# rednote-hilab/dots.ocr

Hardware: AMD Instinct MI355X
Metric: pages/sec, dots.ocr 1.7B bf16, A4@200dpi page batch (preprocess + ViT + prefill + 1024-token greedy decode + detokenise) (higher is better)
Workload: dtype bf16; 1 GPU; a4: 8 pages/GPU of 1654x2339 px -> 19824 patches, 5200 prompt tokens/page, max_new_tokens=1024, EOS disabled; pages_per_gpu=8, parallelism=dp1, decode_rows_in_flight=64

## Files before the change

### dots_ocr_amd/csrc/attn_prefill.hip

```cpp
#include <algorithm>
#include <cstdlib>
#include <utility>

#include "common.h"
#include "kernels.h"

namespace {

constexpr int KT_BYTES = 64 * 256;
constexpr int VT_BYTES = 128 * 128;
constexpr int BUF_BYTES = KT_BYTES + VT_BYTES;
constexpr float RESCALE_THR = 6.0f;

template <bool CAUSAL, int NW, int MODE>
__global__ __launch_bounds__(NW * 64, 2) void flash_attn_kernel(
    const bf16_t* __restrict__ Q, const bf16_t* __restrict__ K, const bf16_t* __restrict__ VT,
    bf16_t* __restrict__ O, const QBlock* __restrict__ blocks, int n_items, int64_t T, int64_t Tpad, int Hq, int group,
    float scale_log2e) {
    constexpr bool PINGPONG = MODE == 1;
    static_assert(!PINGPONG || NW == 8, "ping-pong pairs wave w with wave w + 4 on the same SIMD");
    extern __shared__ __attribute__((aligned(16))) char smem[];

    const QBlock qb = blocks[xcd_remap(blockIdx.x, n_items)];
    const int h = qb.head;
// ... 502 lines not shown
        tile_body(j + 1, sB, sA);
    }

#ifdef F64_PROF
    if (blockIdx.x == 1000 && tid == 0)
        printf("F64_PROF tiles %d: gaps0-7 %llu, gaps8-63 %llu cycles per tile (s_memtime units)\n", n_tiles, prof[1] / n_tiles, prof[3] / n_tiles);
#endif
#pragma unroll
    for (int bk = 0; bk < 2; ++bk) {
        const float l_tot = l_run[bk] + __shfl_xor(l_run[bk], 32, 64);
        const float inv = 1.0f / l_tot;
        const int qrow = qb.q0 + w * 64 + bk * 32 + l31;
        if (qrow < n) {
            bf16_t* op = O + ((size_t)(qb.tok0 + qrow) * Hq + h) * 128;
#pragma unroll
            for (int dt = 0; dt < 4; ++dt)
#pragma unroll
                for (int rq = 0; rq < 4; ++rq) {
                    u32x2 pk = {pack_bf2(o[bk][dt][4 * rq] * inv, o[bk][dt][4 * rq + 1] * inv),
                                pack_bf2(o[bk][dt][4 * rq + 2] * inv, o[bk][dt][4 * rq + 3] * inv)};
                    *reinterpret_cast<u32x2*>(op + dt * 32 + 8 * rq + 4 * hi) = pk;
                }
        }
    }
}
#undef F64_QK_OPS
#undef F64_PV_OPS

}

XcdPlan make_xcd_plan(const QBlock* b, int n_blocks) {
    XcdPlan p;
    bool uniform = true;
    for (int i = 1; i < n_blocks && uniform; ++i) uniform = b[i].n == b[0].n;
    if (uniform || n_blocks < 8) {
        const int q = n_blocks / 8, r = n_blocks % 8;
        for (int x = 0, pos = 0; x < 8; ++x) { p.base[x] = pos; p.cnt[x] = q + (x < r ? 1 : 0); pos += p.cnt[x]; }
        return p;
    }
    auto cost = [&](int i) { return (int64_t)(((b[i].n + 63) / 64 + 1) & ~1); };
    int64_t total = 0;
    for (int i = 0; i < n_blocks; ++i) total += cost(i);
    int pos = 0;
    int64_t done = 0;
    for (int x = 0; x < 8; ++x) {
        const int64_t target = total * (x + 1) / 8;
        p.base[x] = pos;
        while (pos < n_blocks && (x == 7 || done + cost(pos) / 2 < target)) done += cost(pos++);
        p.cnt[x] = pos - p.base[x];
    }
    return p;
}

hipError_t launch_flash_attn(hipStream_t s, const bf16_t* q, const bf16_t* k, const bf16_t* vt, bf16_t* out,
                             const QBlock* blocks, int n_blocks, int64_t T, int64_t Tpad, int Hq, int Hkv,
                             int causal, float scale, const XcdPlan* plan) {
    if (n_blocks <= 0) return hipSuccess;
    if (Hq % Hkv != 0) return hipErrorInvalidValue;
    const float c = scale * 1.44269504088896340736f;
    dim3 grid(n_blocks);
    static const int mode = getenv("DOTS_OCR_ATTN_MODE") ? atoi(getenv("DOTS_OCR_ATTN_MODE")) : 2;
    auto go = [&](auto kern, int threads, int lds) -> hipError_t {
        if (lds > 64 * 1024) {
            hipError_t e = hipFuncSetAttribute(reinterpret_cast<const void*>(kern), hipFuncAttributeMaxDynamicSharedMemorySize, lds);
            if (e != hipSuccess) return e;
        }
        hipLaunchKernelGGL(kern, grid, dim3(threads), lds, s, q, k, vt, out, blocks, n_blocks, T, Tpad, Hq, Hq / Hkv, c);
        return hipGetLastError();
    };
    if (flash_rows_per_block() == 256) {
        static const bool causal64 = !(getenv("DOTS_OCR_PREFILL_F64") && atoi(getenv("DOTS_OCR_PREFILL_F64")) == 0);
        if (mode == 2 && (!causal || causal64)) {
            static uint32_t attr_done[2] = {0, 0};
            int dev = 0;
            hipError_t e = hipGetDevice(&dev);
            if (e != hipSuccess) return e;
            const uint32_t bit = 1u << (dev & 31);
            if (!(__atomic_load_n(&attr_done[causal ? 1 : 0], __ATOMIC_ACQUIRE) & bit)) {
                e = causal ? hipFuncSetAttribute(reinterpret_cast<const void*>(flash_attn64_kernel<true>), hipFuncAttributeMaxDynamicSharedMemorySize, RING_BYTES)
                           : hipFuncSetAttribute(reinterpret_cast<const void*>(flash_attn64_kernel<false>), hipFuncAttributeMaxDynamicSharedMemorySize, RING_BYTES);
                if (e != hipSuccess) return e;
                __atomic_fetch_or(&attr_done[causal ? 1 : 0], bit, __ATOMIC_RELEASE);
            }
            XcdPlan pl;
            if (plan) pl = *plan;
            else {
                const int qn = n_blocks / 8, rn = n_blocks % 8;
                for (int x = 0, pos = 0; x < 8; ++x) { pl.base[x] = pos; pl.cnt[x] = qn + (x < rn ? 1 : 0); pos += pl.cnt[x]; }
            }
            int mx = 0;
            for (int x = 0; x < 8; ++x) mx = std::max(mx, (int)pl.cnt[x]);
            if (causal) hipLaunchKernelGGL(flash_attn64_kernel<true>, dim3(8 * mx), dim3(256), RING_BYTES, s, q, k, vt, out, blocks, n_blocks, T, Tpad, Hq, Hq / Hkv, c, pl);
            else hipLaunchKernelGGL(flash_attn64_kernel<false>, dim3(8 * mx), dim3(256), RING_BYTES, s, q, k, vt, out, blocks, n_blocks, T, Tpad, Hq, Hq / Hkv, c, pl);
            return hipGetLastError();
        }
        if (mode >= 1) return causal ? go(flash_attn_kernel<true, 8, 1>, 512, 3 * BUF_BYTES) : go(flash_attn_kernel<false, 8, 1>, 512, 3 * BUF_BYTES);
        return causal ? go(flash_attn_kernel<true, 8, 0>, 512, 2 * BUF_BYTES) : go(flash_attn_kernel<false, 8, 0>, 512, 2 * BUF_BYTES);
    }
    return causal ? go(flash_attn_kernel<true, 4, 0>, 256, 2 * BUF_BYTES) : go(flash_attn_kernel<false, 4, 0>, 256, 2 * BUF_BYTES);
}

int flash_rows_per_block() {
    static const int rows = getenv("DOTS_OCR_ATTN_ROWS128") ? 128 : 256;
    return rows;
}
```

### dots_ocr_amd/csrc/elementwise.hip

```cpp
#include "common.h"
#include "kernels.h"

namespace {

constexpr int MAX_CHUNKS = 8;

template <bool LAYERNORM, int NCH>
__global__ __launch_bounds__(256) void norm_kernel(const bf16_t* __restrict__ x, const bf16_t* __restrict__ w,
                                                   const bf16_t* __restrict__ b, bf16_t* __restrict__ y,
                                                   int64_t rows, int dim, float eps) {
    const int l = threadIdx.x & 63;
    const int64_t row = (int64_t)blockIdx.x * 4 + (threadIdx.x >> 6);
    if (row >= rows) return;
    const bf16_t* xr = x + row * dim;
    constexpr int NC = NCH > 0 ? NCH : MAX_CHUNKS;
    u32x4 v[NC];
    float s = 0.f, s2 = 0.f;
    if constexpr (NCH > 0) {
#pragma unroll
        for (int c = 0; c < NC; ++c) v[c] = *reinterpret_cast<const u32x4*>(xr + c * 512 + l * 8);
    }
#pragma unroll
    for (int c = 0; c < NC; ++c) {
        const int off = c * 512 + l * 8;
// ... 104 lines not shown
            const int item = it * 256 + tid;
            const int tok = item >> 3, c = item & 7;
            if (tok >= tl.n) continue;
            const int64_t t = tl.tok0 + tok;
            const float2* tab = cs + t * 64 + c * 8;
            float2 cc[8];
#pragma unroll
            for (int e = 0; e < 8; ++e) cc[e] = tab[e];
            for (int hh = slot * ROPE_HPB; hh < h_end; ++hh) {
                bf16_t* dst = hh < Hq ? q + (size_t)hh * T * 128 : k + (size_t)(hh - Hq) * T * 128;
                const bf16_t* src = qkv + t * ld + hh * 128 + c * 8;
                u32x4 xl = *reinterpret_cast<const u32x4*>(src);
                u32x4 xh = *reinterpret_cast<const u32x4*>(src + 64);
                u32x4 ol, oh;
#pragma unroll
                for (int e = 0; e < 4; ++e) {
                    float2 c0 = cc[2 * e], c1 = cc[2 * e + 1];
                    float a0 = lo_bf(xl[e]), a1 = hi_bf(xl[e]), b0 = lo_bf(xh[e]), b1 = hi_bf(xh[e]);
                    ol[e] = pack_bf2(__builtin_fmaf(a0, c0.x, -(b0 * c0.y)), __builtin_fmaf(a1, c1.x, -(b1 * c1.y)));
                    oh[e] = pack_bf2(__builtin_fmaf(a0, c0.y, b0 * c0.x), __builtin_fmaf(b1, c1.x, a1 * c1.y));
                }
                bf16_t* d = dst + t * 128 + c * 8;
                *reinterpret_cast<u32x4*>(d) = ol;
                *reinterpret_cast<u32x4*>(d + 64) = oh;
            }
        }
    } else {
        const int h = slot - n_groups;
#pragma unroll
        for (int it = 0; it < 4; ++it) {
            const int item = it * 256 + tid;
            const int tok = item >> 4, c = item & 15;
            u32x4 v = {0, 0, 0, 0};
            if (tok < tl.n) v = *reinterpret_cast<const u32x4*>(qkv + (size_t)(tl.tok0 + tok) * ld + (Hq + Hkv + h) * 128 + c * 8);
            const int p = (tok & ~15) | (tok & 3) | (((tok >> 3) & 1) << 2) | (((tok >> 2) & 1) << 3);
            *reinterpret_cast<u32x4*>(&lds[p * 136 + c * 8]) = v;
        }
        __syncthreads();
#pragma unroll
        for (int it = 0; it < 4; ++it) {
            const int item = it * 256 + tid;
            const int d = item >> 3, pc = item & 7;
            u32x4 o;
#pragma unroll
            for (int e = 0; e < 4; ++e) {
                uint32_t a = lds[(pc * 8 + 2 * e) * 136 + d], b = lds[(pc * 8 + 2 * e + 1) * 136 + d];
                o[e] = a | (b << 16);
            }
            *reinterpret_cast<u32x4*>(vt + ((size_t)h * 128 + d) * Tpad + tl.pad0 + pc * 8) = o;
        }
    }
}

__global__ __launch_bounds__(256) void embed_gather_kernel(const int32_t* __restrict__ src, const bf16_t* __restrict__ embed,
                                                           const bf16_t* __restrict__ vision, bf16_t* __restrict__ x,
                                                           int64_t T, int dim) {
    const int l = threadIdx.x & 63;
    const int64_t t = (int64_t)blockIdx.x * 4 + (threadIdx.x >> 6);
    if (t >= T) return;
    const int sidx = src[t];
    const bf16_t* s = sidx >= 0 ? embed + (size_t)sidx * dim : vision + (size_t)(-sidx - 1) * dim;
    for (int off = l * 8; off < dim; off += 512)
        *reinterpret_cast<u32x4*>(x + t * dim + off) = *reinterpret_cast<const u32x4*>(s + off);
}

__global__ __launch_bounds__(256) void gather_rows_kernel(const bf16_t* __restrict__ x, const int32_t* __restrict__ rows,
                                                          const int32_t* __restrict__ dst, bf16_t* __restrict__ y, int n, int dim) {
    const int l = threadIdx.x & 63;
    const int r = blockIdx.x * 4 + (threadIdx.x >> 6);
    if (r >= n) return;
    const bf16_t* s = x + (size_t)rows[r] * dim;
    bf16_t* d = y + (size_t)(dst ? dst[r] : r) * dim;
    for (int off = l * 8; off < dim; off += 512) *reinterpret_cast<u32x4*>(d + off) = *reinterpret_cast<const u32x4*>(s + off);
}

}

hipError_t launch_rmsnorm(hipStream_t s, const bf16_t* x, const bf16_t* w, bf16_t* y, int64_t rows, int dim, float eps) {
    if (rows <= 0) return hipSuccess;
    if (dim % 8 != 0 || dim > MAX_CHUNKS * 512) return hipErrorInvalidValue;
    const dim3 grid((unsigned)((rows + 3) / 4));
    const bf16_t* nob = nullptr;
    if (dim == 1536) hipLaunchKernelGGL((norm_kernel<false, 3>), grid, dim3(256), 0, s, x, w, nob, y, rows, dim, eps);
    else if (dim == 1024) hipLaunchKernelGGL((norm_kernel<false, 2>), grid, dim3(256), 0, s, x, w, nob, y, rows, dim, eps);
    else if (dim == 512) hipLaunchKernelGGL((norm_kernel<false, 1>), grid, dim3(256), 0, s, x, w, nob, y, rows, dim, eps);
    else hipLaunchKernelGGL((norm_kernel<false, 0>), grid, dim3(256), 0, s, x, w, nob, y, rows, dim, eps);
    return hipGetLastError();
}

hipError_t launch_layernorm(hipStream_t s, const bf16_t* x, const bf16_t* w, const bf16_t* b, bf16_t* y,
                            int64_t rows, int dim, float eps) {
    if (rows <= 0) return hipSuccess;
    if (dim % 8 != 0 || dim > MAX_CHUNKS * 512) return hipErrorInvalidValue;
    const dim3 grid((unsigned)((rows + 3) / 4));
    if (dim == 1536) hipLaunchKernelGGL((norm_kernel<true, 3>), grid, dim3(256), 0, s, x, w, b, y, rows, dim, eps);
    else hipLaunchKernelGGL((norm_kernel<true, 0>), grid, dim3(256), 0, s, x, w, b, y, rows, dim, eps);
    return hipGetLastError();
}

hipError_t launch_patch_prep(hipStream_t s, const float* x, bf16_t* y, int64_t rows, int in_dim, int out_dim) {
    if (rows <= 0) return hipSuccess;
    if (in_dim % 4 != 0 || out_dim % 4 != 0 || out_dim < in_dim) return hipErrorInvalidValue;
    const int64_t n = rows * (out_dim / 4);
    hipLaunchKernelGGL(patch_prep_kernel, dim3((unsigned)((n + 255) / 256)), dim3(256), 0, s, x, y, rows, in_dim, out_dim);
    return hipGetLastError();
}

hipError_t launch_rope_table(hipStream_t s, const int32_t* pos, const float* inv_freq, float2* cs, int64_t T, int two_d) {
    if (T <= 0) return hipSuccess;
    hipLaunchKernelGGL(rope_table_kernel, dim3((unsigned)((T * 64 + 255) / 256)), dim3(256), 0, s, pos, inv_freq, cs, T, two_d);
    return hipGetLastError();
}

hipError_t launch_qkv_rope_split(hipStream_t s, const bf16_t* qkv, const float2* cs, const Tile64* tiles, int n_tiles,
                                 bf16_t* q, bf16_t* k, bf16_t* vt, int64_t T, int64_t Tpad, int Hq, int Hkv, bool v_only) {
    if (n_tiles <= 0) return hipSuccess;
    const int n_groups = (Hq + Hkv + ROPE_HPB - 1) / ROPE_HPB;
    if (v_only) hipLaunchKernelGGL(qkv_rope_split_kernel, dim3(n_tiles, Hkv), dim3(256), 0, s, qkv, cs, tiles, q, k, vt, T, Tpad, Hq, Hkv, n_groups);
    else hipLaunchKernelGGL(qkv_rope_split_kernel, dim3(n_tiles, n_groups + Hkv), dim3(256), 0, s, qkv, cs, tiles, q, k, vt, T, Tpad, Hq, Hkv, 0);
    return hipGetLastError();
}

hipError_t launch_embed_gather(hipStream_t s, const int32_t* src, const bf16_t* embed, const bf16_t* vision, bf16_t* x,
                               int64_t T, int dim) {
    if (T <= 0) return hipSuccess;
    hipLaunchKernelGGL(embed_gather_kernel, dim3((unsigned)((T + 3) / 4)), dim3(256), 0, s, src, embed, vision, x, T, dim);
    return hipGetLastError();
}

hipError_t launch_gather_rows(hipStream_t s, const bf16_t* x, const int32_t* rows, const int32_t* dst, bf16_t* y, int n, int dim) {
    if (n <= 0) return hipSuccess;
    hipLaunchKernelGGL(gather_rows_kernel, dim3((n + 3) / 4), dim3(256), 0, s, x, rows, dst, y, n, dim);
    return hipGetLastError();
}
```

### dots_ocr_amd/csrc/engine.h

```cpp
#pragma once
#include <hip/hip_runtime.h>
#include <hip/hip_fp16.h>

#include <algorithm>
#include <cmath>
#include <cstdarg>
#include <cstddef>
#include <cstdio>
#include <cstdlib>
#include <cstring>
#include <string>
#include <type_traits>
#include <unordered_map>
#include <vector>

#include "common.h"
#include "decode_layout.h"
#include "dots_ocr_hip.h"
#include "kernels.h"
#include "row_stage.h"

struct Tensor {
    bf16_t* p = nullptr;
    std::vector<int64_t> shape;
// ... 12 lines not shown
    uint8_t *qkv_8, *o_8, *w13_8, *down_8;
};

struct DotsEngine {
    DotsConfig cfg{};
    int device = 0;
    hipStream_t stream = nullptr;
    std::string err;
    std::vector<void*> allocs;
    bool finalized = false;

    std::unordered_map<std::string, Tensor> raw;

    bf16_t *patch_w = nullptr, *patch_b = nullptr, *patch_norm = nullptr;
    int patch_k = 0, patch_kpad = 0;
    std::vector<VLayer> vl;
    bf16_t *v_post_norm = nullptr, *m_ln_w = nullptr, *m_ln_b = nullptr, *m0_w = nullptr, *m0_b = nullptr, *m2_w = nullptr, *m2_b = nullptr;
    bf16_t *embed = nullptr, *final_norm = nullptr, *lm_head = nullptr;
    void* lm_head_d = nullptr;
    float *m0_s = nullptr, *m2_s = nullptr, *lm_head_s = nullptr;
    uint8_t *m0_8 = nullptr, *m2_8 = nullptr;
    uint8_t* act_q = nullptr;
    float* act_s = nullptr;
    uint8_t* act_q_v = nullptr;
    float* act_s_v = nullptr;
    hipStream_t s_vit = nullptr, s_dec = nullptr;
    int dec_cus = 128;
    hipEvent_t ev_vis_ready = nullptr, ev_xs = nullptr;
    bf16_t* vis_pref = nullptr;
    int64_t vis_pref_rows = 0;
    bool pref_pending = false;
    bool pref_deferred = false;
    const float* pref_pix = nullptr;
    int64_t pref_patches = 0;
    std::vector<int64_t> pref_grid;
    hipStream_t vs = nullptr;
    hipStream_t s_vit_full = nullptr;
    hipEvent_t ev_tw0 = nullptr, ev_tw_sw = nullptr, ev_dec_end = nullptr;
    int tail_fixed = 0;
    int tail_now = 0;
    int tail_head_blocks = 0;
    uint64_t tw_seq = 0, dec_end_seq = 0, dec_end_at_tw = 0;
    std::vector<LLayer> ll;
    float *v_inv_freq = nullptr, *lm_inv_freq = nullptr;

    int64_t P = 0, Ppad = 0;
    bf16_t *v_xa = nullptr, *v_x = nullptr, *v_xn = nullptr, *v_qkv = nullptr, *v_q = nullptr, *v_k = nullptr, *v_vt = nullptr,
           *v_att = nullptr, *v_act = nullptr, *v_mh = nullptr, *vis = nullptr;
    float* v_pix = nullptr;
    float2* v_cs = nullptr;
    int32_t* v_pos = nullptr;
    Tile64* v_tiles = nullptr;
    QBlock* v_qblocks = nullptr;
    int64_t vis_rows = 0;
    std::vector<int32_t> h_pos;
    std::vector<Tile64> h_tiles;
    std::vector<QBlock> h_qblocks;

    int64_t TP = 0, TPpad = 0;
    bf16_t *p_x = nullptr, *p_xn = nullptr, *p_qkv = nullptr, *p_q = nullptr, *p_k = nullptr, *p_vt = nullptr, *p_att = nullptr, *p_act = nullptr;
    float2* p_cs = nullptr;
    int32_t *p_pos = nullptr, *p_src = nullptr, *p_last = nullptr;
    Tile64* p_tiles = nullptr;
    QBlock* p_qblocks = nullptr;
    std::vector<int32_t> hp_pos, hp_src, hp_last, hp_table;
    std::vector<Tile64> hp_tiles;
    std::vector<QBlock> hp_qblocks;

    int max_pages = 0;
    int n_pool_pages = 0;
    int kv_capped = 0;
    std::vector<int32_t> free_pages;
    std::vector<int32_t> page_refs;
    std::vector<int> fresh_slots;
    int32_t* fk_dev = nullptr;
    std::vector<std::vector<int32_t>> slot_pages;
    bf16_t* pool = nullptr;
    size_t pool_layer_elems = 0;
    bool kv8 = false;
    float* kv_scales = nullptr;
    int32_t *block_table = nullptr, *ctx_len = nullptr, *cur_tokens = nullptr, *out_ids = nullptr, *out_lens = nullptr,
            *finished = nullptr, *eos_ids = nullptr, *am_idx = nullptr;
    float* am_val = nullptr;
    int n_eos = 0;
    float temperature = 0.f, top_p = 1.f;
    uint64_t seed = 0;
    RowStage stage;
    RowParams* d_rowp = nullptr;
    int32_t* d_row_own = nullptr;
    uint32_t* d_row_thr = nullptr;
    int32_t* pen_cnt = nullptr;
    uint32_t* pen_seen = nullptr;
    float* pen_logits = nullptr;
    RowRules* d_rules = nullptr;
    float* rule_img = nullptr;
    int32_t *rule_stage = nullptr, *rule_stage_host = nullptr;
    hipEvent_t rule_ev = nullptr;
    int32_t h_eos[16] = {0};
    int32_t* tok_off = nullptr;
    uint8_t* tok_bytes = nullptr;
    struct Guide { uint16_t* table = nullptr; uint8_t* accepting = nullptr; int n_states = 0, start = 0, rows = 0; };
    std::vector<Guide> guides;
    RowGuide* d_guides = nullptr;
    uint32_t* guide_mask = nullptr;
    int row_guide[DOTS_MAX_BATCH] = {0};
    RowNgram* d_ngram = nullptr;
    uint32_t* ngram_mask = nullptr;
    struct Stop { uint16_t* table = nullptr; uint16_t* match_len = nullptr; uint8_t* match_id = nullptr; int n_states = 0, rows = 0; };
    std::vector<Stop> stops;
// ... 79 lines not shown

static_assert(sizeof(RowParams) == sizeof(DotsSamplingParams) && offsetof(RowParams, seed) == offsetof(DotsSamplingParams, seed) &&
                  offsetof(RowParams, presence_penalty) == offsetof(DotsSamplingParams, presence_penalty),
              "RowParams (kernels.h) must mirror DotsSamplingParams");

#define CK(expr)                                                                                         \
    do {                                                                                                 \
        hipError_t e_ = (expr);                                                                          \
        if (e_ != hipSuccess) return e->fail(DOTS_E_HIP, "%s failed: %s (%s:%d)", #expr, hipGetErrorString(e_), __FILE__, __LINE__); \
    } while (0)

#define RET(x) do { int r_ = (x); if (r_ != DOTS_OK) return r_; } while (0)

struct Scratch {
    DotsEngine* e;
    std::vector<void*> ptrs;
    explicit Scratch(DotsEngine* e_) : e(e_) {}
    template <typename T>
    hipError_t get(T** p, size_t n) {
        hipError_t r = e->alloc(p, n);
        if (r == hipSuccess) ptrs.push_back(*p);
        return r;
    }
    ~Scratch() {
        hipStreamSynchronize(e->stream);
        for (void* p : ptrs) e->release(p);
    }
};

namespace engine {

inline int64_t round_up(int64_t a, int64_t b) { return (a + b - 1) / b * b; }

int alloc_workspaces(DotsEngine* e);
hipError_t upload_table_row(DotsEngine* e, int slot);
void release_pages(DotsEngine* e, int slot);
bool reserve_pages(DotsEngine* e, int slot, int tokens);
int admit_tokens(const DotsEngine* e, int prompt, int max_new);
StepState step_state(const DotsEngine* e, int advance, const int32_t* sel);
bool spec_draws(const DotsEngine* e);
SpecState spec_state(const DotsEngine* e);
hipError_t launch_row_stage(hipStream_t s, const float* logits, int V, int ld, int B, const RowSel& rs, float* am_val, int32_t* am_idx,
                            const StepState& st, const int32_t* ban_finished);
int select_tokens(DotsEngine* e, int advance);
int clear_row_feature(DotsEngine* e, int row, RowFeature f);
int hold_row_stop(DotsEngine* e, int row, int id, int min_tokens);
int check_row_params(DotsEngine* e, const DotsSamplingParams& p, RowParams* out);
int check_logit_rules(DotsEngine* e, const DotsLogitRules& r, int V, const int32_t* eos, int n_eos, RowRules* out);
int check_ngram_rule(DotsEngine* e, const DotsNgramRule& r, int V, int max_len, RowNgram* out);
int clear_lp_row(DotsEngine* e, int row);
int set_row_lp(DotsEngine* e, int row, int top_n);
void build_worklists(const std::vector<int>& lens, int Hq, std::vector<Tile64>& tiles, std::vector<QBlock>& qblocks, int64_t* Tpad_used,
                     const int* seq_ids = nullptr);
void drop_step_graphs(DotsEngine* e);
int chain_streams(DotsEngine* e, hipStream_t from, hipStream_t to);
int pick_decode_stream(DotsEngine* e, hipStream_t* cur);
int prefill(DotsEngine* e, const int32_t* ids, const int32_t* lens, int B, const int32_t* slots = nullptr, const int32_t* max_new = nullptr);
int decode_step_launches(DotsEngine* e, int n_splits, int part = 0);
int splits_for_ctx(int max_ctx);
int step_graph(DotsEngine* e, int rows, int n_splits, int out_cap, hipGraphExec_t* exec, int part = 0);

}
```

### dots_ocr_amd/csrc/engine.hip

```cpp
#include "engine.h"

namespace engine {
namespace {
thread_local std::string g_create_error;

int dense_on(DotsEngine* e, hipStream_t st, uint8_t* aq, float* as, const bf16_t* A, const bf16_t* W, const uint8_t* W8, const float* wscale,
             const bf16_t* bias, const bf16_t* R, void* C, int64_t M, int N, int K, int ldc, int epi) {
    if (!W8) {
        CK(launch_gemm(st, A, W, bias, R, C, M, N, K, K, ldc, epi, wscale));
        return DOTS_OK;
    }
    CK(launch_quant_act_fp8(st, A, aq, as, M, K, K));
    CK(launch_gemm_fp8(st, aq, as, W8, wscale, bias, R, C, M, N, K, ldc, epi));
    return DOTS_OK;
}
int dense(DotsEngine* e, const bf16_t* A, const bf16_t* W, const uint8_t* W8, const float* wscale, const bf16_t* bias, const bf16_t* R, void* C,
          int64_t M, int N, int K, int ldc, int epi) {
    return dense_on(e, e->stream, e->act_q, e->act_s, A, W, W8, wscale, bias, R, C, M, N, K, ldc, epi);
}
int vdense(DotsEngine* e, const bf16_t* A, const bf16_t* W, const uint8_t* W8, const float* wscale, const bf16_t* bias, const bf16_t* R, void* C,
           int64_t M, int N, int K, int ldc, int epi) {
    return dense_on(e, e->vs, e->act_q_v, e->act_s_v, A, W, W8, wscale, bias, R, C, M, N, K, ldc, epi);
}

int qkv_rope_on(DotsEngine* e, hipStream_t st, uint8_t* aq, float* as, const bf16_t* A, const bf16_t* W, const uint8_t* W8, const float* wscale, const bf16_t* bias,
                bf16_t* qkv, const float2* cs, const Tile64* tiles, int n_tiles, bf16_t* q, bf16_t* k, bf16_t* vt, int64_t T, int64_t Tpad, int K, int Hq, int Hkv) {
    const int N = (Hq + 2 * Hkv) * 128;
    if (!W8 && !wscale) {
        const hipError_t r = launch_gemm_qk_rope(st, A, W, bias, qkv, T, N, K, K, N, cs, q, k, Hq, Hkv);
        if (r == hipSuccess) {
            CK(launch_qkv_rope_split(st, qkv, cs, tiles, n_tiles, q, k, vt, T, Tpad, Hq, Hkv, true));
            return DOTS_OK;
        }
        if (r != hipErrorNotSupported) CK(r);
    }
    RET(dense_on(e, st, aq, as, A, W, W8, wscale, bias, nullptr, qkv, T, N, K, N, EPI_NONE));
    CK(launch_qkv_rope_split(st, qkv, cs, tiles, n_tiles, q, k, vt, T, Tpad, Hq, Hkv));
    return DOTS_OK;
}

const float* layer_kv_scales(const DotsEngine* e, int layer) {
    return e->kv8 ? e->kv_scales + (size_t)layer * e->cfg.num_kv_heads * 2 : nullptr;
}

hipError_t attn_event(DotsEngine* e, int idx) {
    while ((int)e->attn_ev.size() <= idx) {
        hipEvent_t ev;
        hipError_t r = hipEventCreate(&ev);
        if (r != hipSuccess) return r;
        e->attn_ev.push_back(ev);
    }
    return hipEventRecord(e->attn_ev[idx], e->vs);
}

int check_vision_request(DotsEngine* e, int64_t N, const int64_t* grid, int n_img) {
    const DotsConfig& c = e->cfg;
    const int m = c.v_merge;
    if (N > e->P) return e->fail(DOTS_E_CAPACITY, "total_patches %lld > max_patches %lld", (long long)N, (long long)e->P);
    if (c.v_temporal_patch != 1) return e->fail(DOTS_E_INVALID, "temporal_patch_size != 1 is not supported");
    int64_t off = 0, n_seq = 0;
    for (int i = 0; i < n_img; ++i) {
        const int64_t t = grid[i * 3], h = grid[i * 3 + 1], w = grid[i * 3 + 2];
        if (t < 1 || h < 1 || w < 1 || h % m || w % m) return e->fail(DOTS_E_INVALID, "grid_thw[%d] not divisible by merge size", i);
        if (t * h * w > N - off) return e->fail(DOTS_E_INVALID, "grid_thw does not match total_patches");
        off += t * h * w;
        n_seq += t;
    }
    if (off != N) return e->fail(DOTS_E_INVALID, "grid_thw covers %lld patches, total_patches is %lld", (long long)off, (long long)N);
    if (n_seq > 256) return e->fail(DOTS_E_CAPACITY, "more than 256 images per call");
    return DOTS_OK;
}

int vit_forward(DotsEngine* e, const float* pix_dev, int64_t N, const int64_t* grid, int n_img, void* out_dev, bf16_t* vis_out, int64_t* rows_out) {
    const DotsConfig& c = e->cfg;
    hipStream_t s = e->vs;
    const int E = c.v_embed_dim, Hh = c.v_heads, m = c.v_merge;
    RET(check_vision_request(e, N, grid, n_img));
    e->h_pos.resize((size_t)N * 2);
    std::vector<int> lens;
    int64_t off = 0;
    double attn_flops = 0;
    for (int i = 0; i < n_img; ++i) {
        const int64_t t = grid[i * 3], h = grid[i * 3 + 1], w = grid[i * 3 + 2];
        if (h % m || w % m || t < 1) return e->fail(DOTS_E_INVALID, "grid_thw[%d] not divisible by merge size", i);
        if (off + t * h * w > N) return e->fail(DOTS_E_INVALID, "grid_thw does not match total_patches");
        for (int64_t tt = 0; tt < t; ++tt) {
            for (int64_t gh = 0; gh < h / m; ++gh)
                for (int64_t gw = 0; gw < w / m; ++gw)
                    for (int mh = 0; mh < m; ++mh)
                        for (int mw = 0; mw < m; ++mw) {
                            e->h_pos[off * 2] = (int32_t)(gh * m + mh);
                            e->h_pos[off * 2 + 1] = (int32_t)(gw * m + mw);
                            ++off;
                        }
            lens.push_back((int)(h * w));
            attn_flops += 4.0 * (double)(h * w) * (double)(h * w) * E;
        }
    }
    if (off != N) return e->fail(DOTS_E_INVALID, "grid_thw covers %lld patches, total_patches is %lld", (long long)off, (long long)N);
    if (lens.size() > 256) return e->fail(DOTS_E_CAPACITY, "more than 256 images per call");
    int64_t Tpad = 0;
    build_worklists(lens, Hh, e->h_tiles, e->h_qblocks, &Tpad);
    CK(hipMemcpyAsync(e->v_pos, e->h_pos.data(), e->h_pos.size() * 4, hipMemcpyHostToDevice, s));
    CK(hipMemcpyAsync(e->v_tiles, e->h_tiles.data(), e->h_tiles.size() * sizeof(Tile64), hipMemcpyHostToDevice, s));
    CK(hipMemcpyAsync(e->v_qblocks, e->h_qblocks.data(), e->h_qblocks.size() * sizeof(QBlock), hipMemcpyHostToDevice, s));

    CK(hipEventRecord(e->ev[0], s));
    CK(launch_patch_prep(s, pix_dev, e->v_xa, N, e->patch_k, e->patch_kpad));
    CK(launch_gemm(s, e->v_xa, e->patch_w, e->patch_b, nullptr, e->v_xn, N, E, e->patch_kpad, e->patch_kpad, E, EPI_NONE));
    CK(launch_rmsnorm(s, e->v_xn, e->patch_norm, e->v_x, N, E, c.v_rms_eps));
    CK(launch_rope_table(s, e->v_pos, e->v_inv_freq, e->v_cs, N, 1));
    const float scale = 1.0f / sqrtf(128.0f);
    e->attn_pairs = 0;
    const XcdPlan xcd_plan = make_xcd_plan(e->h_qblocks.data(), (int)e->h_qblocks.size());
    hipStream_t const s_first = s;
    const bool prefetched = e->s_vit && s == e->s_vit && e->s_vit_full;
    const int switch_at = prefetched ? c.v_layers - std::max(0, std::min(e->tail_now, c.v_layers - 1)) : -1;
    if (prefetched) CK(hipEventRecord(e->ev_tw0, s));
    for (int i = 0; i < c.v_layers; ++i) {
        const VLayer& L = e->vl[i];
        if (i == switch_at) {
            CK(hipEventRecord(e->ev_tw_sw, s));
            e->tail_head_blocks = i;
            RET(chain_streams(e, s, e->s_vit_full));
            e->vs = s = e->s_vit_full;
        }
        CK(launch_rmsnorm(s, e->v_x, L.norm1, e->v_xn, N, E, c.v_rms_eps));
        RET(qkv_rope_on(e, s, e->act_q_v, e->act_s_v, e->v_xn, L.qkv_w, L.qkv_8, L.qkv_s, L.qkv_b, e->v_qkv, e->v_cs, e->v_tiles, (int)e->h_tiles.size(), e->v_q, e->v_k, e->v_vt,
                        N, Tpad, E, Hh, Hh));
        CK(attn_event(e, 2 * i));
        CK(launch_flash_attn(s, e->v_q, e->v_k, e->v_vt, e->v_att, e->v_qblocks, (int)e->h_qblocks.size(), N, Tpad, Hh, Hh, 0, scale, &xcd_plan));
        CK(attn_event(e, 2 * i + 1));
        e->attn_pairs = i + 1;
        RET(vdense(e, e->v_att, L.proj_w, L.proj_8, L.proj_s, L.proj_b, e->v_x, e->v_x, N, E, E, E, EPI_RESIDUAL));
        CK(launch_rmsnorm(s, e->v_x, L.norm2, e->v_xn, N, E, c.v_rms_eps));
        RET(vdense(e, e->v_xn, L.w13, L.w13_8, L.w13_s, L.b13, nullptr, e->v_act, N, 2 * c.v_intermediate, E, c.v_intermediate, EPI_SWIGLU));
        RET(vdense(e, e->v_act, L.w2, L.w2_8, L.w2_s, L.b2, e->v_x, e->v_x, N, E, c.v_intermediate, E, EPI_RESIDUAL));
        if (e->dbg_hidden && (size_t)(i + 1) * N * E <= e->dbg_cap) {
            CK(hipMemcpyAsync(e->dbg_hidden + (size_t)i * N * E, e->v_x, (size_t)N * E * 2, hipMemcpyDeviceToDevice, s));
            e->dbg_vit_rows = N;
        }
    }
    if (prefetched && switch_at == c.v_layers) {
        CK(hipEventRecord(e->ev_tw_sw, s));
        e->tail_head_blocks = c.v_layers;
    }
    const bf16_t* xin = e->v_x;
    if (c.v_post_norm) {
        CK(launch_rmsnorm(s, e->v_x, e->v_post_norm, e->v_xn, N, E, c.v_rms_eps));
        xin = e->v_xn;
    }
    CK(launch_layernorm(s, xin, e->m_ln_w, e->m_ln_b, e->v_att, N, E, c.v_ln_eps));
    const int g = m * m, Mg = E * g;
    const int64_t R = N / g;
    RET(vdense(e, e->v_att, e->m0_w, e->m0_8, e->m0_s, e->m0_b, nullptr, e->v_mh, R, Mg, Mg, Mg, EPI_GELU));
    RET(vdense(e, e->v_mh, e->m2_w, e->m2_8, e->m2_s, e->m2_b, nullptr, vis_out, R, c.hidden_size, Mg, c.hidden_size, EPI_NONE));
    if (s != s_first) {
        RET(chain_streams(e, s, s_first));
        e->vs = s = s_first;
    }
    CK(hipEventRecord(e->ev[1], s));
    *rows_out = R;
    if (out_dev) CK(hipMemcpyAsync(out_dev, vis_out, (size_t)R * c.hidden_size * 2, hipMemcpyDeviceToDevice, s));

    e->stats.vit_patches = N;
    e->stats.vit_attn_flops = attn_flops * c.v_layers;
    e->stats.vit_flops = e->stats.vit_attn_flops +
                         (double)c.v_layers * 2.0 * N * (4.0 * E * E + 3.0 * E * c.v_intermediate) +
                         2.0 * N * e->patch_k * E + 2.0 * (double)R * ((double)Mg * Mg + (double)Mg * c.hidden_size);
    return DOTS_OK;
}

int ensure_overlap_streams(DotsEngine* e) {
    if (e->s_vit) return DOTS_OK;
    if (const char* v = getenv("DOTS_OCR_OVERLAP_DEC_CUS")) e->dec_cus = std::max(32, std::min(224, atoi(v) / 8 * 8));
    uint32_t wd[8] = {0}, wv[8] = {0};
    static const bool by_xcd = getenv("DOTS_OCR_OVERLAP_BY_XCD") != nullptr;
    for (int b = 0; b < 256; ++b) ((by_xcd ? (b % 8) < e->dec_cus / 32 : b < e->dec_cus) ? wd : wv)[b / 32] |= 1u << (b % 32);
    if (hipExtStreamCreateWithCUMask(&e->s_dec, 8, wd) != hipSuccess || hipExtStreamCreateWithCUMask(&e->s_vit, 8, wv) != hipSuccess) {
        (void)hipGetLastError();
        if (e->s_dec) { hipStreamDestroy(e->s_dec); e->s_dec = nullptr; }
        fprintf(stderr, "[dots_ocr_hip] CU-masked streams are not available on this device: vision prefetch runs without CU partitioning\n");
// ... 40 lines not shown
    e->tail_now = pick_tower_tail(e);
    e->dec_end_at_tw = e->dec_end_seq;
    ++e->tw_seq;
    RET(chain_streams(e, e->stream, e->s_vit));
    e->vs = e->s_vit;
    int r = vit_forward(e, e->pref_pix, e->pref_patches, e->pref_grid.data(), (int)(e->pref_grid.size() / 3), nullptr, e->vis_pref, &e->vis_pref_rows);
    e->vs = e->stream;
    if (e->s_vit_full) {
        const int rc = chain_streams(e, e->s_vit_full, e->s_vit);
        if (r == DOTS_OK) r = rc;
    }
    CK(hipEventRecord(e->ev_vis_ready, e->s_vit));
    if (r != DOTS_OK) e->pref_pending = false;
    return r;
}

DotsEngine::StepKey step_key(const DotsEngine* e, int rows, int n_splits, int out_cap, int part) {
    DotsEngine::StepKey k;
    k.rows = rows; k.splits = n_splits; k.out_cap = out_cap; k.n_eos = e->n_eos; k.part = part;
    k.rowp = e->stage.staged_rows() > 0;
    k.lp = e->n_lp > 0;
    k.rules = e->stage.rows(ROW_RULES) > 0;
    k.guided = e->stage.rows(ROW_GUIDE) > 0;
    k.ngram = e->stage.rows(ROW_NGRAM) > 0;
    k.spec = e->slot_mode ? e->spec_k : 0;
    k.draw = spec_draws(e);
    return k;
}

double decode_step_bytes(const DotsConfig& c) {
    const double H = c.hidden_size, Nq = c.num_heads * 128.0, Nkv = c.num_kv_heads * 128.0, I = c.intermediate_size;
    const double lin = H * (Nq + 2 * Nkv) + Nq * H + 3 * H * I, chans = (Nq + 2 * Nkv) + H + 2 * I + H;
    const double small = 2.0 * ((c.attention_bias ? Nq + 2 * Nkv : 0) + 2 * H);
    if (c.fp8_weights) return c.num_layers * (lin + 4.0 * chans + small) + 2.0 * H + (double)c.vocab_size * (H + 4.0);
    return c.num_layers * (2.0 * lin + small) + 2.0 * H + 2.0 * (double)c.vocab_size * H;
}
}

void build_worklists(const std::vector<int>& lens, int Hq, std::vector<Tile64>& tiles, std::vector<QBlock>& qblocks, int64_t* Tpad_used,
                     const int* seq_ids) {
    tiles.clear();
    qblocks.clear();
    int tok0 = 0, pad0 = 0;
    for (size_t s = 0; s < lens.size(); ++s) {
        const int n = lens[s];
        const int seq = seq_ids ? seq_ids[s] : (int)s;
        for (int t = 0; t * 64 < n; ++t) tiles.push_back(Tile64{tok0 + t * 64, std::min(64, n - t * 64), pad0 + t * 64, seq, t, 0});
        for (int h = 0; h < Hq; ++h)
            for (int q = 0; q < n; q += flash_rows_per_block()) qblocks.push_back(QBlock{q, n, tok0, pad0, h, 0});
        tok0 += n;
        pad0 += (int)round_up(n, 64);
    }
    *Tpad_used = pad0;
}

void drop_step_graphs(DotsEngine* e) {
    for (auto& g : e->step_graphs) {
        hipGraphExecDestroy(g.exec);
        hipGraphDestroy(g.graph);
    }
    e->step_graphs.clear();
}

int chain_streams(DotsEngine* e, hipStream_t from, hipStream_t to) {
    if (from == to) return DOTS_OK;
    CK(hipEventRecord(e->ev_xs, from));
    CK(hipStreamWaitEvent(to, e->ev_xs, 0));
    return DOTS_OK;
}

int pick_decode_stream(DotsEngine* e, hipStream_t* cur) {
    hipStream_t want = e->stream;
    if (e->s_vit && e->pref_pending && !e->pref_deferred && hipEventQuery(e->ev_vis_ready) == hipErrorNotReady) {
        (void)hipGetLastError();
        want = e->s_dec;
    }
    if (want != *cur) {
        RET(chain_streams(e, *cur, want));
        *cur = want;
    }
    return DOTS_OK;
}

int prefill(DotsEngine* e, const int32_t* ids, const int32_t* lens, int B, const int32_t* slots, const int32_t* max_new) {
    const DotsConfig& c = e->cfg;
    hipStream_t s = e->stream;
    const int H = c.hidden_size, Hq = c.num_heads, Hkv = c.num_kv_heads, Nq = Hq * 128, Nkv = Hkv * 128, NQKV = Nq + 2 * Nkv;
    if (B < 1 || B > c.max_batch) return e->fail(DOTS_E_CAPACITY, "batch %d exceeds max_batch %d", B, c.max_batch);
    int64_t T = 0;
    std::vector<int> L(B), S(B);
    int rows = B;
    for (int b = 0; b < B; ++b) {
        if (lens[b] < 1 || lens[b] >= c.max_seq_len) return e->fail(DOTS_E_CAPACITY, "prompt %d length %d not in [1, max_seq_len)", b, lens[b]);
        L[b] = lens[b];
        T += lens[b];
        S[b] = slots ? slots[b] : b;
        if (slots) {
            if (S[b] < 0 || S[b] >= c.max_batch) return e->fail(DOTS_E_INVALID, "slot %d out of range [0, %d)", S[b], c.max_batch);
            if (e->spec_k && S[b] >= c.max_batch / (e->spec_k + 1))
                return e->fail(DOTS_E_CAPACITY, "slot %d is not usable while speculating: with %d drafts a slot takes %d rows of a step, so only slots [0, max_batch / (k + 1)) = [0, %d) are",
                               S[b], e->spec_k, e->spec_k + 1, c.max_batch / (e->spec_k + 1));
            if (e->slot_mode && e->slot_active[S[b]]) return e->fail(DOTS_E_STATE, "slot %d is occupied", S[b]);
            for (int a = 0; a < b; ++a)
                if (S[a] == S[b]) return e->fail(DOTS_E_INVALID, "slot %d listed twice", S[b]);
            if (max_new[b] < 1 || lens[b] + max_new[b] > c.max_seq_len)
                return e->fail(DOTS_E_CAPACITY, "slot %d: prompt (%d) + max_new_tokens (%d) exceeds max_seq_len %d", S[b], lens[b], max_new[b], c.max_seq_len);
            rows = std::max(rows, S[b] + 1);
        }
    }
    if (T > e->TP) return e->fail(DOTS_E_CAPACITY, "packed prompt tokens %lld > max_prefill_tokens %lld", (long long)T, (long long)e->TP);
    e->fresh_slots.clear();
    e->hp_pos.resize(T); e->hp_src.resize(T); e->hp_last.assign(DOTS_MAX_BATCH, 0);
    int64_t t = 0, vis_used = 0;
    for (int b = 0; b < B; ++b) {
        for (int i = 0; i < L[b]; ++i, ++t) {
            e->hp_pos[t] = i;
            const int id = ids[t];
            if (id == c.image_token_id) e->hp_src[t] = -(int32_t)(++vis_used);
            else if (id < 0 || id >= c.vocab_size) return e->fail(DOTS_E_INVALID, "token id %d out of range", id);
            else e->hp_src[t] = id;
        }
        e->hp_last[b] = (int32_t)(t - 1);
    }
    if (vis_used != (vis_used ? e->vis_rows : 0))
        return e->fail(DOTS_E_STATE, "prompt has %lld image tokens but the vision tower produced %lld rows", (long long)vis_used, (long long)e->vis_rows);
    int64_t Tpad = 0;
    build_worklists(L, Hq, e->hp_tiles, e->hp_qblocks, &Tpad, S.data());
    CK(hipMemcpyAsync(e->p_pos, e->hp_pos.data(), T * 4, hipMemcpyHostToDevice, s));
    CK(hipMemcpyAsync(e->p_src, e->hp_src.data(), T * 4, hipMemcpyHostToDevice, s));
    CK(hipMemcpyAsync(e->p_last, e->hp_last.data(), DOTS_MAX_BATCH * 4, hipMemcpyHostToDevice, s));
    CK(hipMemcpyAsync(e->p_tiles, e->hp_tiles.data(), e->hp_tiles.size() * sizeof(Tile64), hipMemcpyHostToDevice, s));
    CK(hipMemcpyAsync(e->p_qblocks, e->hp_qblocks.data(), e->hp_qblocks.size() * sizeof(QBlock), hipMemcpyHostToDevice, s));
    if (!slots || !e->slot_mode)
        for (int b = 0; b < (int)e->slot_pages.size(); ++b) release_pages(e, b);
    const bool whole_table = !slots || !e->slot_mode;
    {
        int need = 0;
        for (int b = 0; b < B; ++b) need += ((slots ? admit_tokens(e, L[b], max_new[b]) : std::min(L[b] + e->out_cap, c.max_seq_len)) + 63) / 64;
        if (need > (int)e->free_pages.size()) {
            const int have = (int)e->free_pages.size();
            if (whole_table) CK(hipMemcpyAsync(e->block_table, e->hp_table.data(), e->hp_table.size() * 4, hipMemcpyHostToDevice, s));
            return e->fail(DOTS_E_CAPACITY, "KV pool exhausted: these sequences need %d pages of 64 tokens, %d of %d are free", need, have, e->n_pool_pages);
        }
        for (int b = 0; b < B; ++b) reserve_pages(e, S[b], slots ? admit_tokens(e, L[b], max_new[b]) : std::min(L[b] + e->out_cap, c.max_seq_len));
        if (whole_table) CK(hipMemcpyAsync(e->block_table, e->hp_table.data(), e->hp_table.size() * 4, hipMemcpyHostToDevice, s));
        else for (int b = 0; b < B; ++b) CK(upload_table_row(e, S[b]));
    }
    struct PageGuard {
        DotsEngine* e; const std::vector<int>& S; bool slots, armed = true;
        ~PageGuard() {
            if (!armed || !slots) return;
            for (int sl : S) { release_pages(e, sl); (void)upload_table_row(e, sl); }
        }
    } page_guard{e, S, slots != nullptr};
    if (!slots) {
        e->slot_mode = false;
        std::fill(e->slot_active, e->slot_active + DOTS_MAX_BATCH, 0);
        CK(hipMemcpyAsync(e->ctx_len, lens, B * 4, hipMemcpyHostToDevice, s));
        CK(hipMemsetAsync(e->out_lens, 0, c.max_batch * 4, s));
        CK(hipMemsetAsync(e->finished, 0, c.max_batch * 4, s));
    } else {
        if (!e->slot_mode) {
            std::fill(e->slot_active, e->slot_active + DOTS_MAX_BATCH, 0);
            CK(hipMemsetAsync(e->ctx_len, 0, c.max_batch * 4, s));
            e->slot_mode = true;
        }
        int32_t sel_new[DOTS_MAX_BATCH] = {0};
        for (int b = 0; b < B; ++b) {
            sel_new[S[b]] = 1;
            CK(hipMemcpyAsync(e->ctx_len + S[b], lens + b, 4, hipMemcpyHostToDevice, s));
            CK(hipMemcpyAsync(e->d_max_len + S[b], max_new + b, 4, hipMemcpyHostToDevice, s));
            CK(hipMemsetAsync(e->out_lens + S[b], 0, 4, s));
            CK(hipMemsetAsync(e->finished + S[b], 0, 4, s));
            if (e->sp_ndraft) {
                CK(hipMemsetAsync(e->sp_ndraft + S[b], 0, 4, s));
                CK(hipMemsetAsync(e->sp_stats + (size_t)S[b] * 3, 0, 3 * sizeof(unsigned long long), s));
            }
        }
        CK(hipMemcpyAsync(e->d_sel_new, sel_new, DOTS_MAX_BATCH * 4, hipMemcpyHostToDevice, s));
        CK(hipMemcpyAsync(e->p_dst, S.data(), B * 4, hipMemcpyHostToDevice, s));
    }

    for (int b = 0; b < B; ++b) RET(clear_lp_row(e, S[b]));
    CK(hipEventRecord(e->ev[2], s));
    CK(launch_embed_gather(s, e->p_src, e->embed, e->vis, e->p_x, T, H));
    CK(launch_rope_table(s, e->p_pos, e->lm_inv_freq, e->p_cs, T, 0));
    const float scale = 1.0f / sqrtf(128.0f);
    const int n_tiles = (int)e->hp_tiles.size();
    for (int i = 0; i < c.num_layers; ++i) {
        const LLayer& Lw = e->ll[i];
        bf16_t* pool_l = e->pool + e->pool_layer_elems * i;
        CK(launch_rmsnorm(s, e->p_x, Lw.ln1, e->p_xn, T, H, c.rms_norm_eps));
        RET(qkv_rope_on(e, s, e->act_q, e->act_s, e->p_xn, Lw.qkv_w, Lw.qkv_8, Lw.qkv_s, Lw.qkv_b, e->p_qkv, e->p_cs, e->p_tiles, n_tiles, e->p_q, e->p_k, e->p_vt, T, Tpad, H, Hq, Hkv));
        CK(launch_kv_to_pages(s, e->p_k, e->p_qkv, e->p_tiles, n_tiles, e->block_table, e->max_pages, pool_l, T, Hq, Hkv, layer_kv_scales(e, i)));
        CK(launch_flash_attn(s, e->p_q, e->p_k, e->p_vt, e->p_att, e->p_qblocks, (int)e->hp_qblocks.size(), T, Tpad, Hq, Hkv, 1, scale));
        RET(dense(e, e->p_att, Lw.o_w, Lw.o_8, Lw.o_s, nullptr, e->p_x, e->p_x, T, H, Nq, H, EPI_RESIDUAL));
        CK(launch_rmsnorm(s, e->p_x, Lw.ln2, e->p_xn, T, H, c.rms_norm_eps));
        RET(dense(e, e->p_xn, Lw.w13, Lw.w13_8, Lw.w13_s, nullptr, nullptr, e->p_act, T, 2 * c.intermediate_size, H, c.intermediate_size, EPI_SWIGLU));
        RET(dense(e, e->p_act, Lw.down_w, Lw.down_8, Lw.down_s, nullptr, e->p_x, e->p_x, T, H, c.intermediate_size, H, EPI_RESIDUAL));
        const size_t voff = (size_t)c.v_layers * e->dbg_vit_rows * c.v_embed_dim;
        if (e->dbg_hidden && voff + (size_t)(i + 1) * T * H <= e->dbg_cap) {
            CK(hipMemcpyAsync(e->dbg_hidden + voff + (size_t)i * T * H, e->p_x, (size_t)T * H * 2, hipMemcpyDeviceToDevice, s));
            e->dbg_lm_rows = T;
        }
    }
    if (e->pen_cnt) CK(launch_pen_prompt(s, e->p_src, e->p_last, slots ? e->p_dst : nullptr, B, c.image_token_id, c.vocab_size, e->pen_cnt, e->pen_seen));
    if (e->stage.rows(ROW_GUIDE) > 0) CK(launch_guide_reset_rows(s, e->d_guides, slots ? e->p_dst : nullptr, B));
    if (e->stage.rows(ROW_STOP) > 0) CK(launch_stop_reset_rows(s, e->d_stop, slots ? e->p_dst : nullptr, B));
    CK(launch_gather_rows(s, e->p_x, e->p_last, slots ? e->p_dst : nullptr, e->d_h, B, H));
    CK(launch_dec_lmhead(s, e->d_h, e->final_norm, e->lm_head_d, e->lm_head_s, e->d_logits, rows, H, c.vocab_size, c.rms_norm_eps));
    e->B_sel = rows;
    e->sel_now = e->d_sel_new;
    RET(select_tokens(e, 0));
    CK(hipEventRecord(e->ev[3], s));
    if (slots) {
        for (int b = 0; b < B; ++b) {
            e->slot_active[S[b]] = 1;
            e->slot_limit[S[b]] = L[b] + max_new[b];
            e->slot_prompt[S[b]] = L[b];
            e->slot_ctx_ub[S[b]] = L[b];
            e->slot_done[S[b]] = 0;
        }
        e->sel_dirty = true;
        e->B = 0;
        e->fresh_slots = S;
    } else {
        e->B = B;
        e->h_prompt_lens = L;
    }
    page_guard.armed = false;
    if (e->pref_deferred) RET(launch_prefetched_tower(e));
    e->steps_done = 0;
    e->vis_rows = 0;
    e->stats.prefill_tokens = T;
    double pf = 0;
    const double lin = (double)c.num_layers * ((double)H * NQKV + (double)Nq * H + 3.0 * H * c.intermediate_size);
    for (int b = 0; b < B; ++b) pf += 2.0 * lin * L[b] + (double)c.num_layers * 2.0 * L[b] * (double)L[b] * Nq + 2.0 * (double)c.vocab_size * H;
    e->stats.prefill_flops = pf;
    return DOTS_OK;
}

int decode_step_launches(DotsEngine* e, int n_splits, int part) {
    const DotsConfig& c = e->cfg;
    hipStream_t s = e->stream;
    const int H = c.hidden_size, Hq = c.num_heads, Hkv = c.num_kv_heads, Nq = Hq * 128, I = c.intermediate_size;
    const int rows = e->B, spec_k = e->slot_mode ? e->spec_k : 0;
    const int B = rows * (spec_k + 1);
    const float scale = 1.0f / sqrtf(128.0f);
// ... 355 lines not shown
        if (e->pp_tab) { hipStreamSynchronize(s); e->release(e->pp_tab); e->pp_tab = nullptr; }
        e->pp_tab_cap = tab_ints + tab_ints / 4;
        CK(e->alloc(&e->pp_tab, e->pp_tab_cap));
    }
    int32_t* tab = e->pp_tab;
    if (rw != w) {
        CK(grow(&e->pp_tmp, &e->pp_tmp_cap, tmp_bytes));
        CK(hipMemcpyAsync(tab, hcoef, (size_t)rw * hk * 4, hipMemcpyHostToDevice, s));
        CK(hipMemcpyAsync(tab + (size_t)rw * hk, hbounds, (size_t)rw * 2 * 4, hipMemcpyHostToDevice, s));
        CK(launch_resize_h(s, src, e->pp_tmp, tab, tab + (size_t)rw * hk, hk, h, w, rw));
        src = e->pp_tmp;
        tab += (size_t)rw * (hk + 2);
    }
    if (rh != h) {
        CK(grow(&e->pp_out, &e->pp_out_cap, out_bytes));
        CK(hipMemcpyAsync(tab, vcoef, (size_t)rh * vk * 4, hipMemcpyHostToDevice, s));
        CK(hipMemcpyAsync(tab + (size_t)rh * vk, vbounds, (size_t)rh * 2 * 4, hipMemcpyHostToDevice, s));
        CK(launch_resize_v(s, src, e->pp_out, tab, tab + (size_t)rh * vk, vk, rw, rh));
        src = e->pp_out;
    }
    CK(launch_normalize_patchify(s, src, out, rw, rh / P, rw / P, P, m, rescale, mean3, std3));
    CK(hipStreamSynchronize(s));
    return DOTS_OK;
}

int dots_set_decode_plan(DotsEngine* e, int plan) {
    if (!e) return DOTS_E_INVALID;
    if (plan < 0 || plan > 5 || (plan & 6) == 6)
        return e->fail(DOTS_E_INVALID, "decode plan must be 0 (by stream) or 1 (partition plan on every step), + 2 (streaming attention) or + 4 (per-split attention)");
    const int part = plan & 1, stream = (plan & 2) ? 1 : (plan & 4) ? 0 : -1;
    if (part != e->force_part || stream != e->attn_stream) {
        e->force_part = part;
        e->attn_stream = stream;
        drop_step_graphs(e);
    }
    return DOTS_OK;
}

int dots_tower_tail(DotsEngine* e, int set, int* now) {
    if (!e) return DOTS_E_INVALID;
    if (set < -2 || set > e->cfg.v_layers) return e->fail(DOTS_E_INVALID, "tower tail must be -2 (query), -1 (adaptive) or 0 .. v_layers");
    if (set >= -1) e->tail_fixed = set;
    if (now) *now = e->tail_now;
    return DOTS_OK;
}

int dots_set_gemm_plan(DotsEngine* e, int plan) {
    if (!e) return DOTS_E_INVALID;
    if (plan < 0 || plan > 1) return e->fail(DOTS_E_INVALID, "gemm plan must be 0 (8-wave ping-pong) or 1 (one wave per SIMD)");
    gemm_set_plan(plan);
    return DOTS_OK;
}

int dots_get_logits(DotsEngine* e, float* out) {
    if (!e || !out) return DOTS_E_INVALID;
    if (e->B < 1) return e->fail(DOTS_E_STATE, "no prefilled batch");
    CK(hipSetDevice(e->device));
    CK(hipMemcpyAsync(out, e->d_logits, (size_t)e->B * e->cfg.vocab_size * 4, hipMemcpyDeviceToHost, e->stream));
    CK(hipStreamSynchronize(e->stream));
    return DOTS_OK;
}

int dots_set_next_tokens(DotsEngine* e, const int32_t* tokens, int B) {
    if (!e || !tokens || B != e->B) return e ? e->fail(DOTS_E_INVALID, "bad set_next_tokens arguments") : DOTS_E_INVALID;
    CK(hipSetDevice(e->device));
    CK(hipMemcpyAsync(e->cur_tokens, tokens, B * 4, hipMemcpyHostToDevice, e->stream));
    CK(hipStreamSynchronize(e->stream));
    return DOTS_OK;
}

int dots_get_last_tokens(DotsEngine* e, int32_t* out) {
    if (!e || !out) return DOTS_E_INVALID;
    if (e->B < 1) return e->fail(DOTS_E_STATE, "no prefilled batch");
    CK(hipSetDevice(e->device));
    std::vector<int32_t> lens(DOTS_MAX_BATCH), ids((size_t)DOTS_MAX_BATCH * std::max(1, e->out_cap));
    CK(hipMemcpyAsync(lens.data(), e->out_lens, e->B * 4, hipMemcpyDeviceToHost, e->stream));
    CK(hipMemcpyAsync(ids.data(), e->out_ids, (size_t)e->B * e->out_cap * 4, hipMemcpyDeviceToHost, e->stream));
    CK(hipStreamSynchronize(e->stream));
    for (int b = 0; b < e->B; ++b) out[b] = lens[b] > 0 ? ids[(size_t)b * e->out_cap + lens[b] - 1] : -1;
    return DOTS_OK;
}

int dots_debug_capture_hidden(DotsEngine* e, int64_t capacity_elems) {
    if (!e || capacity_elems < 0) return DOTS_E_INVALID;
    CK(hipSetDevice(e->device));
    CK(hipStreamSynchronize(e->stream));
    if (e->dbg_hidden) { e->release(e->dbg_hidden); e->dbg_hidden = nullptr; }
    e->dbg_cap = 0; e->dbg_vit_rows = e->dbg_lm_rows = 0;
    if (capacity_elems > 0) {
        CK(e->alloc(&e->dbg_hidden, (size_t)capacity_elems));
        e->dbg_cap = (size_t)capacity_elems;
    }
    return DOTS_OK;
}

int dots_debug_read_hidden(DotsEngine* e, int which, int layer, void* out_host, int64_t* rows_out) {
    if (!e || !out_host || !rows_out || !e->dbg_hidden) return e ? e->fail(DOTS_E_STATE, "hidden-state capture is off") : DOTS_E_INVALID;
    CK(hipSetDevice(e->device));
    const DotsConfig& c = e->cfg;
    const int64_t rows = which == 0 ? e->dbg_vit_rows : e->dbg_lm_rows;
    const int dim = which == 0 ? c.v_embed_dim : c.hidden_size, n_layers = which == 0 ? c.v_layers : c.num_layers;
    if (rows <= 0 || layer < 0 || layer >= n_layers) return e->fail(DOTS_E_INVALID, "no captured hidden state for layer %d", layer);
    const size_t off = (which == 0 ? 0 : (size_t)c.v_layers * e->dbg_vit_rows * c.v_embed_dim) + (size_t)layer * rows * dim;
    if (off + (size_t)rows * dim > e->dbg_cap) return e->fail(DOTS_E_CAPACITY, "capture buffer too small for layer %d", layer);
    CK(hipMemcpyAsync(out_host, e->dbg_hidden + off, (size_t)rows * dim * 2, hipMemcpyDeviceToHost, e->stream));
    CK(hipStreamSynchronize(e->stream));
// ... 74 lines not shown
```

### dots_ocr_amd/csrc/gemm.hip

```cpp
#include <cstdlib>
#include <utility>

#include "common.h"
#include "kernels.h"

namespace {

constexpr int BM = 128, BN = 128, BK = 64;
constexpr int TILE_BYTES = 128 * 128;
#ifndef GEMM_GROUP_M
#define GEMM_GROUP_M 8
#endif
constexpr int GROUP_M = GEMM_GROUP_M;

DEVI float gelu_erf(float x) { return 0.5f * x * (1.0f + erff(x * 0.70710678118654752440f)); }
#ifdef GEMM_EXACT_SILU
DEVI float silu(float x) { return x / (1.0f + __expf(-x)); }
#else
DEVI float silu(float x) {
    const float d = 1.0f + __expf(fminf(-x, 80.f));
    const float r = __builtin_amdgcn_rcpf(d);
    const float q = x * r;
    return __builtin_fmaf(__builtin_fmaf(-q, d, x), r, q);
}
// ... 601 lines not shown
        }
    };
    load_t(0, tb[0]);
    W4_PUT(0, 0)
#pragma unroll
    for (int qb = 0; qb < 16; ++qb) {
        const int fm = qb >> 2;
        if (qb + 1 < 16) load_t(qb + 1, tb[(qb + 1) & 1]);
        if ((qb & 3) == 0 && fm + 1 < 4) {
            if (fm == 0) { W4_PUT(1, 1) } else if (fm == 1) { W4_PUT(2, 0) } else { W4_PUT(3, 1) }
        }
        __builtin_amdgcn_sched_barrier(0);
        const char* img = stage2 + (fm & 1) * 16384;
        f32x4 a[2][4];
#pragma unroll
        for (int it = 0; it < 2; ++it) {
            const int row = (qb & 3) * 8 + it * 4 + rrow;
            const int sw = swz(row);
            const char* rp = img + row * 512;
            const int s0 = gcol >> 2;
            a[it][0] = *reinterpret_cast<const f32x4*>(rp + ((s0 ^ sw) << 4));
            a[it][1] = *reinterpret_cast<const f32x4*>(rp + (((s0 + 1) ^ sw) << 4));
            a[it][2] = *reinterpret_cast<const f32x4*>(rp + ((s0 ^ 16 ^ sw) << 4));
            a[it][3] = *reinterpret_cast<const f32x4*>(rp + (((s0 + 1) ^ 16 ^ sw) << 4));
        }
        __builtin_amdgcn_sched_barrier(0);
#pragma unroll
        for (int it = 0; it < 2; ++it) {
            const int m = mw0 + qb * 8 + it * 4 + rrow;
            float o[8] = {a[it][0][0], a[it][0][1], a[it][0][2], a[it][0][3], a[it][1][0], a[it][1][1], a[it][1][2], a[it][1][3]};
            float u[8] = {a[it][2][0], a[it][2][1], a[it][2][2], a[it][2][3], a[it][3][0], a[it][3][1], a[it][3][2], a[it][3][3]};
            if (has_cols) {
#pragma unroll
                for (int e = 0; e < 8; ++e) { o[e] = o[e] * cc.sc0[e] + cc.bi0[e]; u[e] = u[e] * cc.sc1[e] + cc.bi1[e]; }
            }
            uint32_t pk[4];
#pragma unroll
            for (int e = 0; e < 4; ++e) {
                const uint32_t ow = pack_bf2(o[2 * e], o[2 * e + 1]), uw = pack_bf2(u[2 * e], u[2 * e + 1]);
                const float x0 = lo_bf(ow), x1 = hi_bf(ow), y0 = lo_bf(uw), y1 = hi_bf(uw);
                const f32x4 t4 = tb[qb & 1][it][e];
                const float f0 = lo_half ? x0 : y0, g0 = lo_half ? t4[0] : t4[1], m0 = lo_half ? y0 : x0, n0_ = lo_half ? t4[1] : t4[0];
                const float p0 = m0 * n0_, p1 = y1 * t4[3];
                const float r0 = __builtin_fmaf(f0, g0, lo_half ? -p0 : p0), r1 = __builtin_fmaf(x1, t4[2], lo_half ? -p1 : p1);
                pk[e] = pack_bf2(r0, r1);
            }
            if (FULL || m < M) *reinterpret_cast<u32x4*>(dst + (size_t)m * 128 + gcol) = u32x4{pk[0], pk[1], pk[2], pk[3]};
        }
        __builtin_amdgcn_sched_barrier(0);
    }
#undef W4_PUT
}

template <int... I, class F> DEVI void gemm_static_for_impl(std::integer_sequence<int, I...>, F&& f) { (f(std::integral_constant<int, I>{}), ...); }
template <int N, class F> DEVI void gemm_static_for(F&& f) { gemm_static_for_impl(std::make_integer_sequence<int, N>{}, f); }

template <int EPI>
DEVI void gemm_bf16_w4_body(
    const bf16_t* __restrict__ A, const bf16_t* __restrict__ W, const bf16_t* __restrict__ bias,
    const float* __restrict__ colscale, const bf16_t* R, void* Cout, int M, int N, int K, int lda, int ldc, int m_tiles, int n_tiles, int group_m, const QkRope& rope) {
    extern __shared__ __attribute__((aligned(16))) char smem2[];
    (void)rope;

    const int tid = threadIdx.x;
    const int l = tid & 63;
    const int w = __builtin_amdgcn_readfirstlane(tid >> 6);
    const int hi = l >> 5, l31 = l & 31;

    int bid = xcd_remap(blockIdx.x, m_tiles * n_tiles);
    const int per_group = group_m * n_tiles;
    const int g = bid / per_group;
    const int first_m = g * group_m;
    const int gsz = min(m_tiles - first_m, group_m);
    const int in_grp = bid - g * per_group;
    const int tm = first_m + in_grp % gsz;
    const int tn = in_grp / gsz;
    const int m0 = tm * BM2, n0 = tn * BN2;

    const int prow = 8 * w + (l >> 3);
    const int chunk = ((l & 7) ^ ((4 * w + (l >> 4)) & 7)) << 4;
    const int w_src = prow * (K * 2) + chunk;
    int x_src[8];
#pragma unroll
    for (int i = 0; i < 8; ++i) x_src[i] = (min(m0 + prow + 32 * i, M - 1) - m0) * (lda * 2) + chunk;
    const __amdgpu_buffer_rsrc_t rw = __builtin_amdgcn_make_buffer_rsrc((void*)(W + (size_t)n0 * K), 0, 0x7ffffff0, 0x00020000);
    const __amdgpu_buffer_rsrc_t rx = __builtin_amdgcn_make_buffer_rsrc((void*)(A + (size_t)m0 * lda), 0, 0x7ffffff0, 0x00020000);
    const int w_step = 32 * K * 2;
    auto dma_w = [&](int t, int slot, int i) {
        __builtin_amdgcn_raw_ptr_buffer_load_lds(rw, (__attribute__((address_space(3))) void*)(smem2 + slot * W4_UNIT + (w + 4 * i) * 1024), 16, w_src,
                                                 t * 128 + i * w_step, 0, 0);
    };
    auto dma_x = [&](int t, int slot, int i) {
        __builtin_amdgcn_raw_ptr_buffer_load_lds(rx, (__attribute__((address_space(3))) void*)(smem2 + slot * W4_UNIT + (w + 4 * i) * 1024), 16, x_src[i],
                                                 t * 128, 0, 0);
    };

    const int wn = w >> 1, wm = w & 1;
    const int rsw = (l31 >> 1) & 7;
    const int lane_sw = ((hi ^ (rsw & 1)) << 4) | ((rsw >> 1) << 5);
    const int lds0 = (int)(uintptr_t)(__attribute__((address_space(3))) char*)smem2;
    const int a_lane = lds0 + (wn * 128 + l31) * 128 + lane_sw;
    const int b_lane = lds0 + (wm * 128 + l31) * 128 + lane_sw;
    auto frag = [&](int base, int ks, int f) {
        return *reinterpret_cast<const __attribute__((address_space(3))) bf16x8*>((uintptr_t)(uint32_t)((base ^ (ks << 5)) + f * 4096));
    };

// ... 56 lines not shown
                    if constexpr (idx < 4) fa[cur ^ 1][f] = frag(aw, ks + 1, f);
                    else fb[cur ^ 1][f] = frag(ax, ks + 1, f);
                } else {
                    if constexpr (idx < 4) fa[cur ^ 1][f] = frag(awn, 0, f);
                    else fb[cur ^ 1][f] = frag(axn, 0, f);
                }
            }
#ifndef W4_NO_DMA
            if constexpr (MODE == 0) {
                if constexpr (gp == 8 || gp == 11 || gp == 14 || gp == 24 || gp == 27 || gp == 30 || gp == 40 || gp == 43) {
                    constexpr int i = gp < 16 ? (gp - 8) / 3 : gp < 32 ? 3 + (gp - 24) / 3 : 6 + (gp - 40) / 3;
                    dma_w(t + 2, s4, i);
                }
                if constexpr (gp >= 56) dma_x(t + 2, u0, gp - 56);
            }
#endif
            asm volatile("v_mfma_f32_32x32x16_bf16 %[d], %[a], %[b], %[d]" : [d] "+a"(acc[fn][fm]) : [a] "v"(fa[cur][fn]), [b] "v"(fb[cur][fm]));
        });
    };
    int u0 = 0;
    for (int t = 0; t < nt - 2; ++t) {
        tile_body(std::integral_constant<int, 0>{}, t, u0);
        u0 = u0 + 2 >= W4_RING ? u0 + 2 - W4_RING : u0 + 2;
    }
    tile_body(std::integral_constant<int, 1>{}, nt - 2, u0);
    u0 = u0 + 2 >= W4_RING ? u0 + 2 - W4_RING : u0 + 2;
    tile_body(std::integral_constant<int, 2>{}, nt - 1, u0);

#ifdef W4_PROF
    const unsigned long long pt2 = __builtin_amdgcn_s_memtime(), pw2 = wall_clock64();
#endif
    __syncthreads();
#ifdef W4_NO_STORE
#pragma unroll
    for (int i = 0; i < 4; ++i)
#pragma unroll
        for (int j = 0; j < 4; ++j) asm volatile("" ::"a"(acc[i][j]));
    return;
#endif
#ifdef W4_OLD_EPILOGUE
    if constexpr (EPI == EPI_F32 || EPI == EPI_SWIGLU) {
        gemm_epilogue<EPI, 4, 4>(acc, bias, colscale, R, Cout, M, ldc, n0 + wn * 128, m0 + wm * 128, l31, hi);
    } else {
        gemm_epilogue_lds<EPI, 4>(acc, bias, colscale, R, reinterpret_cast<bf16_t*>(Cout), M, ldc, n0 + wn * 128, m0 + wm * 128, l, smem2 + w * 16384);
    }
#else
    if constexpr (EPI == EPI_QKROPE) {
        const int head = (n0 + wn * 128) >> 7;
        const bool full = m0 + wm * 128 + 128 <= M, has_cols = bias != nullptr || colscale != nullptr;
        if (head < rope.n_rope_heads) {
            bf16_t* dst = head < rope.Hq ? rope.q + (size_t)head * rope.T * 128 : rope.k + (size_t)(head - rope.Hq) * rope.T * 128;
            if (full) w4_epilogue_qkrope<true>(acc, cols, has_cols, rope.cs, dst, M, m0 + wm * 128, l, smem2 + w * 32768);
            else w4_epilogue_qkrope<false>(acc, cols, has_cols, rope.cs, dst, M, m0 + wm * 128, l, smem2 + w * 32768);
        } else if (full) {
            w4_epilogue_lds<EPI_NONE, true>(acc, cols, has_cols, R, reinterpret_cast<bf16_t*>(Cout), M, ldc, n0 + wn * 128, m0 + wm * 128, l, smem2 + w * 32768);
        } else {
            w4_epilogue_lds<EPI_NONE, false>(acc, cols, has_cols, R, reinterpret_cast<bf16_t*>(Cout), M, ldc, n0 + wn * 128, m0 + wm * 128, l, smem2 + w * 32768);
        }
    } else if constexpr (EPI == EPI_F32) {
        gemm_epilogue<EPI, 4, 4>(acc, bias, colscale, R, Cout, M, ldc, n0 + wn * 128, m0 + wm * 128, l31, hi);
    } else if (m0 + wm * 128 + 128 <= M) {
        w4_epilogue_lds<EPI, true>(acc, cols, bias != nullptr || colscale != nullptr, R, reinterpret_cast<bf16_t*>(Cout), M, ldc, n0 + wn * 128, m0 + wm * 128, l, smem2 + w * 32768);
    } else {
        w4_epilogue_lds<EPI, false>(acc, cols, bias != nullptr || colscale != nullptr, R, reinterpret_cast<bf16_t*>(Cout), M, ldc, n0 + wn * 128, m0 + wm * 128, l, smem2 + w * 32768);
    }
#endif
#ifdef W4_PROF
    const unsigned long long pt2b = __builtin_amdgcn_s_memtime();
    asm volatile("s_waitcnt vmcnt(0)" ::: "memory");
    const unsigned long long pt3 = __builtin_amdgcn_s_memtime(), pw3 = wall_clock64();
    if ((blockIdx.x == 1000 || blockIdx.x == 2001 || blockIdx.x == 3002) && tid == 0)
        printf("W4_PROF epi %d N %d K %d blk %d: prologue %llu cyc / %.2f us, main loop %llu cyc / %.2f us (%.0f cyc per K tile), epilogue + drain %llu cyc / %.2f us; issue %llu drain %llu\n", EPI, N, K,
               (int)blockIdx.x, pt1 - pt0, (pw1 - pw0) * 0.01, pt2 - pt1, (pw2 - pw1) * 0.01, (double)(pt2 - pt1) / nt, pt3 - pt2, (pw3 - pw2) * 0.01, pt2b - pt2, pt3 - pt2b);
#endif
}

template <int EPI>
__global__ __launch_bounds__(256) void gemm_bf16_w4_kernel(
    const bf16_t* __restrict__ A, const bf16_t* __restrict__ W, const bf16_t* __restrict__ bias,
    const float* __restrict__ colscale, const bf16_t* R, void* Cout, int M, int N, int K, int lda, int ldc, int m_tiles, int n_tiles, int group_m) {
    gemm_bf16_w4_body<EPI>(A, W, bias, colscale, R, Cout, M, N, K, lda, ldc, m_tiles, n_tiles, group_m, QkRope{});
}
__global__ __launch_bounds__(256) void gemm_bf16_w4_qkrope_kernel(
    const bf16_t* __restrict__ A, const bf16_t* __restrict__ W, const bf16_t* __restrict__ bias,
    const float* __restrict__ colscale, void* Cout, int M, int N, int K, int lda, int ldc, int m_tiles, int n_tiles, int group_m, QkRope rope) {
    gemm_bf16_w4_body<EPI_QKROPE>(A, W, bias, colscale, nullptr, Cout, M, N, K, lda, ldc, m_tiles, n_tiles, group_m, rope);
}

typedef __attribute__((ext_vector_type(8))) int i32x8;

template <int EPI>
__global__ __launch_bounds__(512, 2) void gemm_fp8_256pp_kernel(
    const uint8_t* __restrict__ A, const float* __restrict__ rowscale, const uint8_t* __restrict__ W, const float* __restrict__ colscale,
    const bf16_t* __restrict__ bias, const bf16_t* R, void* Cout, int M, int N, int K, int ldc, int m_tiles, int n_tiles, int group_m) {
    extern __shared__ __attribute__((aligned(16))) char smem2[];
    constexpr int SUBK8 = 64;

    const int tid = threadIdx.x;
    const int l = tid & 63;
    const int w = __builtin_amdgcn_readfirstlane(tid >> 6);
    const int hi = l >> 5, l31 = l & 31;
    const int grp = w >> 2;

    int bid = xcd_remap(blockIdx.x, m_tiles * n_tiles);
    const int per_group = group_m * n_tiles;
    const int g = bid / per_group;
// ... 135 lines not shown
        if (!(__atomic_load_n(&configured_w4, __ATOMIC_ACQUIRE) & bit)) {
            e = hipFuncSetAttribute(reinterpret_cast<const void*>(&gemm_bf16_w4_kernel<E>), hipFuncAttributeMaxDynamicSharedMemorySize, W4_RING * W4_UNIT);
            if (e != hipSuccess) return e;
            __atomic_fetch_or(&configured_w4, bit, __ATOMIC_RELEASE);
        }
        hipLaunchKernelGGL(gemm_bf16_w4_kernel<E>, dim3(m_tiles * n_tiles), dim3(256), W4_RING * W4_UNIT, s, A, W, bias, colscale, R, C, M, N, K,
                           lda, ldc, m_tiles, n_tiles, raster_group_m(K * 2));
        return hipGetLastError();
    }
    static uint32_t configured_pp = 0;
    if (!(__atomic_load_n(&configured_pp, __ATOMIC_ACQUIRE) & bit)) {
        e = hipFuncSetAttribute(reinterpret_cast<const void*>(&gemm_bf16_256pp_kernel<E>), hipFuncAttributeMaxDynamicSharedMemorySize,
                                PP_STAGES * SUB_STAGE);
        if (e != hipSuccess) return e;
        __atomic_fetch_or(&configured_pp, bit, __ATOMIC_RELEASE);
    }
    hipLaunchKernelGGL(gemm_bf16_256pp_kernel<E>, dim3(m_tiles * n_tiles), dim3(512), PP_STAGES * SUB_STAGE, s, A, W, bias, colscale, R, C, M, N, K,
                       lda, ldc, m_tiles, n_tiles, raster_group_m(K * 2));
    return hipGetLastError();
}

hipError_t launch_gemm(hipStream_t s, const bf16_t* A, const bf16_t* W, const bf16_t* bias, const bf16_t* R,
                       void* C, int64_t M, int N, int K, int lda, int ldc, int epi, const float* colscale) {
    if (M <= 0) return hipSuccess;
    if (N % BN != 0 || K % BK != 0 || (lda % 8) != 0 || (ldc % 4) != 0) return hipErrorInvalidValue;
    static const bool force_small = getenv("DOTS_OCR_GEMM_128") != nullptr;
    if (N % BN2 == 0 && !force_small) {
        switch (epi) {
            case EPI_NONE: return launch_256<EPI_NONE>(s, A, W, bias, colscale, R, C, (int)M, N, K, lda, ldc);
            case EPI_RESIDUAL: return launch_256<EPI_RESIDUAL>(s, A, W, bias, colscale, R, C, (int)M, N, K, lda, ldc);
            case EPI_SWIGLU: return launch_256<EPI_SWIGLU>(s, A, W, bias, colscale, R, C, (int)M, N, K, lda, ldc);
            case EPI_GELU: return launch_256<EPI_GELU>(s, A, W, bias, colscale, R, C, (int)M, N, K, lda, ldc);
            case EPI_F32: return launch_256<EPI_F32>(s, A, W, bias, colscale, R, C, (int)M, N, K, lda, ldc);
            default: return hipErrorInvalidValue;
        }
    }
    const int m_tiles = (int)((M + BM - 1) / BM), n_tiles = N / BN;
    dim3 grid(m_tiles * n_tiles), block(256);
#define LAUNCH(E)                                                                                       \
    hipLaunchKernelGGL(gemm_bf16_kernel<E>, grid, block, 0, s, A, W, bias, colscale, R, C, (int)M, N, K, lda, ldc, \
                       m_tiles, n_tiles)
    switch (epi) {
        case EPI_NONE: LAUNCH(EPI_NONE); break;
        case EPI_RESIDUAL: LAUNCH(EPI_RESIDUAL); break;
        case EPI_SWIGLU: LAUNCH(EPI_SWIGLU); break;
        case EPI_GELU: LAUNCH(EPI_GELU); break;
        case EPI_F32: LAUNCH(EPI_F32); break;
        default: return hipErrorInvalidValue;
    }
#undef LAUNCH
    return hipGetLastError();
}

hipError_t launch_gemm_qk_rope(hipStream_t s, const bf16_t* A, const bf16_t* W, const bf16_t* bias, bf16_t* qkv, int64_t M, int N, int K, int lda, int ldc,
                               const float2* cs, bf16_t* q, bf16_t* k, int Hq, int Hkv) {
    static const bool off = getenv("DOTS_OCR_QK_FUSE") && atoi(getenv("DOTS_OCR_QK_FUSE")) == 0;
    static const bool lockstep = getenv("DOTS_OCR_GEMM_LOCKSTEP") != nullptr, force_small = getenv("DOTS_OCR_GEMM_128") != nullptr;
    if (off || lockstep || force_small || gemm_get_plan() != 1 || N != (Hq + 2 * Hkv) * 128 || N % BN2 != 0 || K % BK != 0 || K / BK < 3 || lda % 8 != 0 || ldc % 8 != 0 ||
        !cs || !q || !k || M > 0x7fffffff)
        return hipErrorNotSupported;
    if (M <= 0) return hipSuccess;
    static uint32_t configured = 0;
    int dev = 0;
    hipError_t e = hipGetDevice(&dev);
    if (e != hipSuccess) return e;
    const uint32_t bit = 1u << (dev & 31);
    if (!(__atomic_load_n(&configured, __ATOMIC_ACQUIRE) & bit)) {
        e = hipFuncSetAttribute(reinterpret_cast<const void*>(&gemm_bf16_w4_qkrope_kernel), hipFuncAttributeMaxDynamicSharedMemorySize, W4_RING * W4_UNIT);
        if (e != hipSuccess) return e;
        __atomic_fetch_or(&configured, bit, __ATOMIC_RELEASE);
    }
    const int m_tiles = (int)((M + BM2 - 1) / BM2), n_tiles = N / BN2;
    const QkRope rope{cs, q, k, (long long)M, Hq, Hq + Hkv};
    hipLaunchKernelGGL(gemm_bf16_w4_qkrope_kernel, dim3(m_tiles * n_tiles), dim3(256), W4_RING * W4_UNIT, s, A, W, bias, (const float*)nullptr, (void*)qkv, (int)M, N, K,
                       lda, ldc, m_tiles, n_tiles, raster_group_m(K * 2), rope);
    return hipGetLastError();
}

bool gemm_fp8_supports(int N, int K) { return N % BN2 == 0 && K % 64 == 0; }

template <int E>
static hipError_t launch_fp8_t(hipStream_t s, const uint8_t* Aq, const float* rowscale, const uint8_t* Wq, const float* colscale, const bf16_t* bias,
                               const bf16_t* R, void* C, int M, int N, int K, int ldc) {
    static uint32_t configured = 0;
    int dev = 0;
    hipError_t e = hipGetDevice(&dev);
    if (e != hipSuccess) return e;
    const uint32_t bit = 1u << (dev & 31);
    if (!(__atomic_load_n(&configured, __ATOMIC_ACQUIRE) & bit)) {
        e = hipFuncSetAttribute(reinterpret_cast<const void*>(&gemm_fp8_256pp_kernel<E>), hipFuncAttributeMaxDynamicSharedMemorySize, PP_STAGES * SUB_STAGE);
        if (e != hipSuccess) return e;
        __atomic_fetch_or(&configured, bit, __ATOMIC_RELEASE);
    }
    const int m_tiles = (M + BM2 - 1) / BM2, n_tiles = N / BN2;
    hipLaunchKernelGGL(gemm_fp8_256pp_kernel<E>, dim3(m_tiles * n_tiles), dim3(512), PP_STAGES * SUB_STAGE, s, Aq, rowscale, Wq, colscale, bias, R, C, M, N, K,
                       ldc, m_tiles, n_tiles, raster_group_m(K));
    return hipGetLastError();
}

hipError_t launch_gemm_fp8(hipStream_t s, const uint8_t* Aq, const float* rowscale, const uint8_t* Wq, const float* colscale, const bf16_t* bias,
                           const bf16_t* R, void* C, int64_t M, int N, int K, int ldc, int epi) {
    if (M <= 0) return hipSuccess;
    if (!gemm_fp8_supports(N, K) || ldc % 8 != 0 || !rowscale || !colscale) return hipErrorInvalidValue;
    switch (epi) {
        case EPI_NONE: return launch_fp8_t<EPI_NONE>(s, Aq, rowscale, Wq, colscale, bias, R, C, (int)M, N, K, ldc);
        case EPI_RESIDUAL: return launch_fp8_t<EPI_RESIDUAL>(s, Aq, rowscale, Wq, colscale, bias, R, C, (int)M, N, K, ldc);
        case EPI_SWIGLU: return launch_fp8_t<EPI_SWIGLU>(s, Aq, rowscale, Wq, colscale, bias, R, C, (int)M, N, K, ldc);
        case EPI_GELU: return launch_fp8_t<EPI_GELU>(s, Aq, rowscale, Wq, colscale, bias, R, C, (int)M, N, K, ldc);
        default: return hipErrorInvalidValue;
    }
}
```

### dots_ocr_amd/csrc/kernels.h

```cpp
#pragma once
#include <hip/hip_runtime.h>
#include <stdint.h>

typedef uint16_t bf16_t;

#define DOTS_MAX_BATCH 64

enum { EPI_NONE = 0, EPI_RESIDUAL = 1, EPI_SWIGLU = 2, EPI_GELU = 3, EPI_F32 = 4, EPI_QKROPE = 5  };

hipError_t launch_gemm(hipStream_t s, const bf16_t* A, const bf16_t* W, const bf16_t* bias, const bf16_t* R,
                       void* C, int64_t M, int N, int K, int lda, int ldc, int epi, const float* colscale = nullptr);
int gemm_get_plan();
void gemm_set_plan(int plan);

hipError_t launch_rmsnorm(hipStream_t s, const bf16_t* x, const bf16_t* w, bf16_t* y, int64_t rows, int dim, float eps);
hipError_t launch_layernorm(hipStream_t s, const bf16_t* x, const bf16_t* w, const bf16_t* b, bf16_t* y,
                            int64_t rows, int dim, float eps);
hipError_t launch_patch_prep(hipStream_t s, const float* x, bf16_t* y, int64_t rows, int in_dim, int out_dim);
hipError_t launch_rope_table(hipStream_t s, const int32_t* pos, const float* inv_freq, float2* cs, int64_t T, int two_d);
struct Tile64 { int32_t tok0, n, pad0, seq, page, _pad; };
hipError_t launch_qkv_rope_split(hipStream_t s, const bf16_t* qkv, const float2* cs, const Tile64* tiles, int n_tiles,
                                 bf16_t* q, bf16_t* k, bf16_t* vt, int64_t T, int64_t Tpad, int Hq, int Hkv, bool v_only = false);
struct QkRope { const float2* cs; bf16_t* q; bf16_t* k; long long T; int Hq; int n_rope_heads; };
hipError_t launch_gemm_qk_rope(hipStream_t s, const bf16_t* A, const bf16_t* W, const bf16_t* bias, bf16_t* qkv, int64_t M, int N, int K, int lda, int ldc,
                               const float2* cs, bf16_t* q, bf16_t* k, int Hq, int Hkv);
hipError_t launch_embed_gather(hipStream_t s, const int32_t* src, const bf16_t* embed, const bf16_t* vision, bf16_t* x,
                               int64_t T, int dim);
hipError_t launch_gather_rows(hipStream_t s, const bf16_t* x, const int32_t* rows, const int32_t* dst, bf16_t* y, int n, int dim);

struct QBlock { int32_t q0, n, tok0, pad0, head, _pad; };
int flash_rows_per_block();
struct XcdPlan { int32_t base[8], cnt[8]; };
XcdPlan make_xcd_plan(const QBlock* blocks_host, int n_blocks);
hipError_t launch_flash_attn(hipStream_t s, const bf16_t* q, const bf16_t* k, const bf16_t* vt, bf16_t* out,
                             const QBlock* blocks, int n_blocks, int64_t T, int64_t Tpad, int Hq, int Hkv,
                             int causal, float scale, const XcdPlan* plan = nullptr);

hipError_t launch_kv_to_pages(hipStream_t s, const bf16_t* k, const bf16_t* qkv, const Tile64* tiles, int n_tiles,
                              const int32_t* block_table, int max_pages, void* pool_layer, int64_t T, int Hq, int Hkv,
                              const float* kv_scales = nullptr);
hipError_t launch_kv_fork_pages(hipStream_t s, void* pool, size_t layer_bytes, size_t page_bytes, int layers, int src_page, const int32_t* dst_pages,
                                int n);
hipError_t launch_dec_embed(hipStream_t s, const int32_t* tokens, const bf16_t* embed, bf16_t* h, int B, int dim);
hipError_t launch_dec_qkv(hipStream_t s, const bf16_t* h, const bf16_t* ln_w, const void* Wd, const float* wscale, const bf16_t* bias,
                          const float* inv_freq, const int32_t* ctx_len, const int32_t* block_table, int max_pages,
                          void* pool_layer, bf16_t* q_out, int B, int H, int Hq, int Hkv, float eps, int part_cus = 0, bf16_t* xn = nullptr,
                          const float* pend = nullptr, const float* pend_scale = nullptr, const float* kv_scales = nullptr);
hipError_t launch_dec_proj(hipStream_t s, const bf16_t* X, const void* Wd, const float* wscale, bf16_t* h, int B, int N, int K, int part_cus = 0,
                           float* part = nullptr, bool* pending = nullptr);
hipError_t launch_dec_gateup(hipStream_t s, const bf16_t* h, const bf16_t* ln_w, const void* W13d, const float* wscale, bf16_t* act,
                             int B, int H, int I, float eps, int part_cus = 0, bf16_t* xn = nullptr, const float* pend = nullptr, const float* pend_scale = nullptr);
hipError_t launch_dec_lmhead(hipStream_t s, const bf16_t* h, const bf16_t* ln_w, const void* Wd, const float* wscale, float* logits,
                             int B, int H, int V, float eps, int part_cus = 0, bf16_t* xn = nullptr, const float* pend = nullptr, const float* pend_scale = nullptr);
bool dec_stream64_supports(int B, int H);
hipError_t launch_dec_norm_ximg(hipStream_t s, const bf16_t* h, const bf16_t* ln_w, bf16_t* xn, int B, int H, float eps, const float* part = nullptr, const float* pscale = nullptr);
hipError_t launch_dec_gateup64(hipStream_t s, const bf16_t* h, const bf16_t* ln_w, const void* W13d, const float* wscale, bf16_t* act, bf16_t* xn,
                               int B, int H, int I, float eps, int cus, const float* pend = nullptr, const float* pend_scale = nullptr);
hipError_t launch_dec_lmhead64(hipStream_t s, const bf16_t* h, const bf16_t* ln_w, const void* Wd, const float* wscale, float* logits, bf16_t* xn,
                               int B, int H, int V, float eps, int cus, const float* pend = nullptr, const float* pend_scale = nullptr);
constexpr int DEC_KSPLIT_PARTS = 4;
bool dec_proj_ksplit_supports(int B, int N, int K);
hipError_t launch_dec_proj_ksplit(hipStream_t s, const bf16_t* X, const void* Wd, bool fp8, float* part, int B, int N, int K, int cus);
int decode_attn_waves();
int decode_attn_splits(int max_seq_len);
hipError_t launch_decode_attn(hipStream_t s, const bf16_t* q, const void* pool_layer, const int32_t* ctx_len,
                              const int32_t* block_table, int max_pages, float* part_o, float* part_ml,
                              int B, int Hq, int Hkv, int n_splits, float scale, int part_cus = 0, int stream_mode = -1,
                              const float* kv_scales = nullptr);
int decode_attn_stream_wgs(int B, int Hkv, int n_splits, int max_pages, int part_cus, int stream_mode = -1, bool kv8 = false);
hipError_t launch_decode_attn_combine(hipStream_t s, const float* part_o, const float* part_ml, const int32_t* ctx_len, bf16_t* out,
                                      int B, int Hq, int Hkv, int n_splits);
struct StepState {
    int32_t *cur_tokens, *ctx_len, *out_ids, *out_lens, *finished;
    const int32_t *eos_ids, *sel, *max_len;
    int n_eos, out_stride, cap, advance_ctx;
};
hipError_t launch_argmax_step(hipStream_t s, const float* logits, int V, int ld, int B, float* pval, int32_t* pidx, const StepState& st);
hipError_t launch_sample_step(hipStream_t s, const float* logits, int V, int ld, int B, float temperature, float top_p, uint64_t seed,
                              const StepState& st, const int32_t* own = nullptr);
struct RowParams { float temperature, top_p; int32_t top_k; float repetition_penalty, frequency_penalty, presence_penalty; uint64_t seed; };
#ifndef DOTS_MAX_STOP_IDS
#define DOTS_MAX_STOP_IDS 16
#endif
enum { RULE_ON = 1, RULE_IMG = 2, RULE_IGNORE_EOS = 4 };
struct RowRules { int32_t flags, min_tokens, n_stop, stop[DOTS_MAX_STOP_IDS]; };
constexpr uint16_t GUIDE_DEAD = 0xFFFF;
// ... 128 lines not shown
```

### dots_ocr_amd/csrc/ops.hip

```cpp
#include "engine.h"

using namespace engine;

namespace {
int op_weight(DotsEngine* e, Scratch& sc, const bf16_t* w, int64_t rows, int K, int Hq, int Hkv, bool qkv, int fp8, void** wd, float** scale) {
    *scale = nullptr;
    if (fp8) {
        bf16_t* q = nullptr;
        uint8_t* d = nullptr;
        CK(sc.get(&q, (size_t)rows * K));
        CK(sc.get(scale, (size_t)rows));
        CK(sc.get(&d, (size_t)((rows + 15) / 16 * 16) * K));
        CK(hipMemcpyAsync(q, w, (size_t)rows * K * 2, hipMemcpyDeviceToDevice, e->stream));
        CK(launch_quant_rows_fp8(e->stream, q, *scale, rows, K));
        CK(launch_pack_frag_fp8(e->stream, q, d, rows, K, qkv ? (Hq + Hkv) * 128 : 0));
        *wd = d;
    } else {
        bf16_t* d = nullptr;
        CK(sc.get(&d, (size_t)((rows + 15) / 16 * 16) * K));
        if (qkv) CK(launch_pack_frag_qkv(e->stream, w, d, Hq, Hkv, K));
        else CK(launch_pack_frag(e->stream, w, d, rows, K));
        *wd = d;
    }
    return DOTS_OK;
// ... 266 lines not shown
    CK(sc.get(&a8, (size_t)M * K));
    CK(sc.get(&as, (size_t)M));
    CK(hipMemcpyAsync(wq, W, (size_t)N * K * 2, hipMemcpyDeviceToDevice, e->stream));
    CK(launch_quant_rows_fp8(e->stream, wq, ws, N, K));
    CK(launch_bf16q_to_fp8(e->stream, wq, w8, (int64_t)N * K));
    CK(launch_quant_act_fp8(e->stream, (const bf16_t*)A, a8, as, M, K, K));
    const int ldc = epilogue == EPI_SWIGLU ? N / 2 : N;
    CK(launch_gemm_fp8(e->stream, a8, as, w8, ws, (const bf16_t*)bias, (const bf16_t*)residual, C, M, N, K, ldc, epilogue));
    CK(hipStreamSynchronize(e->stream));
    return DOTS_OK;
}

int dots_op_quant_fp8(DotsEngine* e, void* w_inout, float* scale_out, int64_t N, int K) {
    if (!e || !w_inout || !scale_out) return e ? e->fail(DOTS_E_INVALID, "null argument") : DOTS_E_INVALID;
    CK(hipSetDevice(e->device));
    CK(launch_quant_rows_fp8(e->stream, (bf16_t*)w_inout, scale_out, N, K));
    CK(hipStreamSynchronize(e->stream));
    return DOTS_OK;
}

static int upload_lists(DotsEngine* e, const int32_t* cu, int n_seq, int Hq, std::vector<Tile64>& tiles, std::vector<QBlock>& qb,
                        Tile64** d_tiles, QBlock** d_qb, int64_t* Tpad) {
    std::vector<int> lens(n_seq);
    for (int i = 0; i < n_seq; ++i) lens[i] = cu[i + 1] - cu[i];
    build_worklists(lens, Hq, tiles, qb, Tpad);
    CK(e->alloc(d_tiles, tiles.size() + 1));
    CK(e->alloc(d_qb, qb.size() + 1));
    CK(hipMemcpyAsync(*d_tiles, tiles.data(), tiles.size() * sizeof(Tile64), hipMemcpyHostToDevice, e->stream));
    CK(hipMemcpyAsync(*d_qb, qb.data(), qb.size() * sizeof(QBlock), hipMemcpyHostToDevice, e->stream));
    CK(hipStreamSynchronize(e->stream));
    return DOTS_OK;
}

int dots_op_flash_attn(DotsEngine* e, const void* q, const void* k, const void* vt, void* out, const int32_t* cu, int n_seq,
                       int Hq, int Hkv, int causal, float scale) {
    if (!e || !cu || n_seq < 1) return DOTS_E_INVALID;
    CK(hipSetDevice(e->device));
    std::vector<Tile64> tiles;
    std::vector<QBlock> qb;
    Tile64* dt = nullptr;
    QBlock* dq = nullptr;
    int64_t Tpad = 0;
    RET(upload_lists(e, cu, n_seq, Hq, tiles, qb, &dt, &dq, &Tpad));
    const int64_t T = cu[n_seq];
    const XcdPlan xcd_plan = make_xcd_plan(qb.data(), (int)qb.size());
    hipError_t r = launch_flash_attn(e->stream, (const bf16_t*)q, (const bf16_t*)k, (const bf16_t*)vt, (bf16_t*)out, dq, (int)qb.size(), T, Tpad, Hq, Hkv, causal, scale, &xcd_plan);
    hipStreamSynchronize(e->stream);
    e->release(dt);
    e->release(dq);
    CK(r);
    return DOTS_OK;
}

int dots_plan_flash_xcd(const int32_t* lens, int n_seq, int Hq, int32_t* base8, int32_t* cnt8, int64_t* cost8) {
    if (!lens || n_seq < 1 || Hq < 1 || !base8 || !cnt8 || !cost8) return DOTS_E_INVALID;
    std::vector<int> L(lens, lens + n_seq);
    for (int n : L)
        if (n < 1) return DOTS_E_INVALID;
    std::vector<Tile64> tiles;
    std::vector<QBlock> qb;
    int64_t Tpad = 0;
    build_worklists(L, Hq, tiles, qb, &Tpad);
    const XcdPlan p = make_xcd_plan(qb.data(), (int)qb.size());
    for (int x = 0; x < 8; ++x) {
        base8[x] = p.base[x];
        cnt8[x] = p.cnt[x];
        cost8[x] = 0;
        for (int i = p.base[x]; i < p.base[x] + p.cnt[x]; ++i) cost8[x] += ((qb[i].n + 63) / 64 + 1) & ~1;
    }
    return (int)qb.size();
}

int dots_op_qkv_rope_split(DotsEngine* e, const void* qkv, void* q, void* k, void* vt, const int32_t* cu, int n_seq,
                           const int32_t* pos_host, int Hq, int Hkv, int rope2d, float theta) {
    if (!e || !cu || n_seq < 1 || !pos_host) return DOTS_E_INVALID;
    CK(hipSetDevice(e->device));
    std::vector<Tile64> tiles;
    std::vector<QBlock> qb;
    Tile64* dt = nullptr;
    QBlock* dq = nullptr;
    int64_t Tpad = 0;
    RET(upload_lists(e, cu, n_seq, Hq, tiles, qb, &dt, &dq, &Tpad));
    const int64_t T = cu[n_seq];
    int32_t* dpos = nullptr;
    float2* cs = nullptr;
    float* freq = nullptr;
    const int nf = rope2d ? 32 : 64;
    std::vector<float> f(nf);
    for (int i = 0; i < nf; ++i) f[i] = 1.0f / powf(theta, (float)(2 * i) / (rope2d ? 64.0f : 128.0f));
    CK(e->alloc(&dpos, (size_t)T * (rope2d ? 2 : 1)));
    CK(e->alloc(&cs, (size_t)T * 64));
    CK(e->alloc(&freq, (size_t)nf));
    CK(hipMemcpyAsync(dpos, pos_host, (size_t)T * (rope2d ? 2 : 1) * 4, hipMemcpyHostToDevice, e->stream));
    CK(hipMemcpyAsync(freq, f.data(), nf * 4, hipMemcpyHostToDevice, e->stream));
    CK(launch_rope_table(e->stream, dpos, freq, cs, T, rope2d));
    hipError_t r = launch_qkv_rope_split(e->stream, (const bf16_t*)qkv, cs, dt, (int)tiles.size(), (bf16_t*)q, (bf16_t*)k, (bf16_t*)vt, T, Tpad, Hq, Hkv);
    hipStreamSynchronize(e->stream);
    e->release(dt); e->release(dq); e->release(dpos); e->release(cs); e->release(freq);
    CK(r);
    return DOTS_OK;
}

int dots_op_qkv_proj_rope(DotsEngine* e, const void* x, const void* w, const void* bias, void* qkv_ws, void* q, void* k, void* vt, const int32_t* cu, int n_seq,
                          const int32_t* pos_host, int K, int Hq, int Hkv, int rope2d, float theta, int fused) {
    if (!e || !x || !w || !qkv_ws || !q || !k || !vt || !cu || n_seq < 1 || !pos_host) return DOTS_E_INVALID;
    CK(hipSetDevice(e->device));
    std::vector<Tile64> tiles;
    std::vector<QBlock> qb;
    Tile64* dt = nullptr;
    QBlock* dq = nullptr;
    int64_t Tpad = 0;
    RET(upload_lists(e, cu, n_seq, Hq, tiles, qb, &dt, &dq, &Tpad));
    const int64_t T = cu[n_seq];
    const int N = (Hq + 2 * Hkv) * 128;
    int32_t* dpos = nullptr;
    float2* cs = nullptr;
    float* freq = nullptr;
    const int nf = rope2d ? 32 : 64;
    std::vector<float> f(nf);
    for (int i = 0; i < nf; ++i) f[i] = 1.0f / powf(theta, (float)(2 * i) / (rope2d ? 64.0f : 128.0f));
    CK(e->alloc(&dpos, (size_t)T * (rope2d ? 2 : 1)));
    CK(e->alloc(&cs, (size_t)T * 64));
    CK(e->alloc(&freq, (size_t)nf));
    CK(hipMemcpyAsync(dpos, pos_host, (size_t)T * (rope2d ? 2 : 1) * 4, hipMemcpyHostToDevice, e->stream));
    CK(hipMemcpyAsync(freq, f.data(), nf * 4, hipMemcpyHostToDevice, e->stream));
    CK(launch_rope_table(e->stream, dpos, freq, cs, T, rope2d));
    hipError_t r;
    if (fused) {
        r = launch_gemm_qk_rope(e->stream, (const bf16_t*)x, (const bf16_t*)w, (const bf16_t*)bias, (bf16_t*)qkv_ws, T, N, K, K, N, cs, (bf16_t*)q, (bf16_t*)k, Hq, Hkv);
        if (r == hipSuccess) r = launch_qkv_rope_split(e->stream, (const bf16_t*)qkv_ws, cs, dt, (int)tiles.size(), (bf16_t*)q, (bf16_t*)k, (bf16_t*)vt, T, Tpad, Hq, Hkv, true);
    } else {
        r = launch_gemm(e->stream, (const bf16_t*)x, (const bf16_t*)w, (const bf16_t*)bias, nullptr, qkv_ws, T, N, K, K, N, EPI_NONE);
        if (r == hipSuccess) r = launch_qkv_rope_split(e->stream, (const bf16_t*)qkv_ws, cs, dt, (int)tiles.size(), (bf16_t*)q, (bf16_t*)k, (bf16_t*)vt, T, Tpad, Hq, Hkv);
    }
    hipStreamSynchronize(e->stream);
    e->release(dt); e->release(dq); e->release(dpos); e->release(cs); e->release(freq);
    if (r == hipErrorNotSupported) { (void)hipGetLastError(); return e->fail(DOTS_E_INVALID, "no fused qkv + rope kernel for this shape / GEMM plan"); }
    CK(r);
    return DOTS_OK;
}


int dots_op_dec_qkv(DotsEngine* e, const void* h, const void* ln_w, const void* wqkv, const void* bias, const int32_t* ctx_len_dev,
                    const int32_t* block_table_dev, int max_pages, void* pool_layer, void* q_out, int B, int H, int Hq, int Hkv, float eps,
                    float rope_theta, int fp8) {
    return op_dec_qkv(e, h, ln_w, wqkv, bias, ctx_len_dev, block_table_dev, max_pages, pool_layer, q_out, B, H, Hq, Hkv, eps, rope_theta, fp8, nullptr);
}

int dots_op_dec_qkv_kv8(DotsEngine* e, const void* h, const void* ln_w, const void* wqkv, const void* bias, const int32_t* ctx_len_dev,
                        const int32_t* block_table_dev, int max_pages, void* pool_layer, void* q_out, int B, int H, int Hq, int Hkv, float eps,
                        float rope_theta, int fp8, const float* kv_scales_dev) {
    if (!kv_scales_dev) return e ? e->fail(DOTS_E_INVALID, "null kv_scales") : DOTS_E_INVALID;
    return op_dec_qkv(e, h, ln_w, wqkv, bias, ctx_len_dev, block_table_dev, max_pages, pool_layer, q_out, B, H, Hq, Hkv, eps, rope_theta, fp8, kv_scales_dev);
}

int dots_op_decode_attn(DotsEngine* e, const void* q, const void* pool_layer, const int32_t* ctx_len_dev, const int32_t* block_table_dev,
                        int max_pages, void* out, int B, int Hq, int Hkv, int max_seq_len) {
    return op_decode_attn(e, q, pool_layer, ctx_len_dev, block_table_dev, max_pages, out, B, Hq, Hkv, max_seq_len, nullptr);
}

int dots_op_decode_attn_kv8(DotsEngine* e, const void* q, const void* pool_layer, const int32_t* ctx_len_dev, const int32_t* block_table_dev,
                            int max_pages, void* out, int B, int Hq, int Hkv, int max_seq_len, const float* kv_scales_dev) {
    if (!kv_scales_dev) return e ? e->fail(DOTS_E_INVALID, "null kv_scales") : DOTS_E_INVALID;
    return op_decode_attn(e, q, pool_layer, ctx_len_dev, block_table_dev, max_pages, out, B, Hq, Hkv, max_seq_len, kv_scales_dev);
}

int dots_op_dec_proj(DotsEngine* e, const void* x, const void* w, void* h_inout, int B, int N, int K, int fp8) {
    if (!e || !x || !w || !h_inout || B < 1 || B > DOTS_MAX_BATCH) return e ? e->fail(DOTS_E_INVALID, "bad dec_proj arguments") : DOTS_E_INVALID;
    CK(hipSetDevice(e->device));
    Scratch sc(e);
    bf16_t* xi = nullptr;
    void* wd = nullptr;
    float* wscale = nullptr;
    CK(sc.get(&xi, (size_t)(B + 15) / 16 * 16 * K));
    CK(launch_pack_x(e->stream, (const bf16_t*)x, xi, B, K));
    RET(op_weight(e, sc, (const bf16_t*)w, N, K, 0, 0, false, fp8, &wd, &wscale));
    bool pend = false;
    float* part = nullptr;
    CK(sc.get(&part, (size_t)DEC_KSPLIT_PARTS * DOTS_MAX_BATCH * N));
    CK(launch_dec_proj(e->stream, xi, wd, wscale, (bf16_t*)h_inout, B, N, K, e->force_part ? e->dec_cus : 0, part, &pend));
    if (pend) CK(launch_dec_norm_ximg(e->stream, (const bf16_t*)h_inout, nullptr, nullptr, B, N, 0.f, part, wscale));
    CK(hipStreamSynchronize(e->stream));
    return DOTS_OK;
}
// ... 118 lines not shown
```

### dots_ocr_amd/csrc/weights.hip

```cpp
#include "engine.h"

namespace {
__global__ void pack_w13_kernel(const bf16_t* __restrict__ gate, const bf16_t* __restrict__ up, bf16_t* __restrict__ out, int I, int K) {
    const int64_t idx = (int64_t)blockIdx.x * 256 + threadIdx.x;
    const int cpr = K / 8;
    if (idx >= (int64_t)2 * I * cpr) return;
    const int r = (int)(idx / cpr), c = (int)(idx % cpr);
    const int G = r >> 6, wi = r & 63;
    const bf16_t* src = (wi < 32 ? gate + (size_t)(G * 32 + wi) * K : up + (size_t)(G * 32 + wi - 32) * K) + c * 8;
    *reinterpret_cast<u32x4*>(out + (size_t)r * K + c * 8) = *reinterpret_cast<const u32x4*>(src);
}

__global__ void pack_b13_kernel(const bf16_t* __restrict__ gate, const bf16_t* __restrict__ up, bf16_t* __restrict__ out, int I) {
    const int r = blockIdx.x * 256 + threadIdx.x;
    if (r >= 2 * I) return;
    const int G = r >> 6, wi = r & 63;
    out[r] = wi < 32 ? gate[G * 32 + wi] : up[G * 32 + wi - 32];
}

__global__ void convert_kernel(const void* __restrict__ src, int dtype, bf16_t* __restrict__ dst, int64_t n) {
    const int64_t i = (int64_t)blockIdx.x * 256 + threadIdx.x;
    if (i >= n) return;
    if (dtype == DOTS_DTYPE_F32) dst[i] = f2bf(reinterpret_cast<const float*>(src)[i]);
    else if (dtype == DOTS_DTYPE_F16) dst[i] = f2bf(__half2float(reinterpret_cast<const __half*>(src)[i]));
// ... 196 lines not shown
        RET(decode_copy(e, L.o_w, &L.o_wd, H, Nq, 0));
        RET(decode_copy(e, L.w13, &L.w13_wd, 2 * I, H, 0));
        RET(decode_copy(e, L.down_w, &L.down_wd, H, I, 0));
        CK(hipStreamSynchronize(s));
        for (const char* n : {"self_attn.q_proj.weight", "self_attn.k_proj.weight", "self_attn.v_proj.weight",
                              "mlp.gate_proj.weight", "mlp.up_proj.weight"})
            drop(e, p + n);
    }
    {
        std::vector<float> vf(32), lf(64);
        for (int i = 0; i < 32; ++i) vf[i] = 1.0f / powf(10000.0f, (float)(2 * i) / 64.0f);
        for (int i = 0; i < 64; ++i) lf[i] = 1.0f / powf(c.rope_theta, (float)(2 * i) / 128.0f);
        CK(e->alloc(&e->v_inv_freq, 32));
        CK(e->alloc(&e->lm_inv_freq, 64));
        CK(hipMemcpyAsync(e->v_inv_freq, vf.data(), 32 * 4, hipMemcpyHostToDevice, s));
        CK(hipMemcpyAsync(e->lm_inv_freq, lf.data(), 64 * 4, hipMemcpyHostToDevice, s));
        CK(hipStreamSynchronize(s));
    }
    e->finalized = true;
    return DOTS_OK;
}
}

int alloc_workspaces(DotsEngine* e) {
    const DotsConfig& c = e->cfg;
    const int E = c.v_embed_dim, H = c.hidden_size, Nq = c.num_heads * 128, Nkv = c.num_kv_heads * 128;
    const int Mg = E * c.v_merge * c.v_merge;
    e->P = c.max_patches;
    e->Ppad = e->P + 64 * 256;
    const int kpad = (int)round_up(c.v_channels * c.v_patch * c.v_patch, 64);
    if (c.fp8_weights) {
        const size_t v_max = (size_t)e->P * std::max(E, c.v_intermediate);
        const size_t p_max = (size_t)c.max_prefill_tokens * std::max(H, std::max(Nq, c.intermediate_size));
        CK(e->alloc(&e->act_q, p_max));
        CK(e->alloc(&e->act_s, (size_t)c.max_prefill_tokens));
        CK(e->alloc(&e->act_q_v, v_max));
        CK(e->alloc(&e->act_s_v, (size_t)e->P));
    }
    CK(e->alloc(&e->v_xa, (size_t)e->P * kpad));
    CK(e->alloc(&e->v_x, (size_t)e->P * E));
    CK(e->alloc(&e->v_xn, (size_t)e->P * E));
    CK(e->alloc(&e->v_qkv, (size_t)e->P * 3 * E));
    CK(e->alloc(&e->v_q, (size_t)e->P * E));
    CK(e->alloc(&e->v_k, (size_t)(e->P + 64) * E));
    CK(e->alloc(&e->v_vt, (size_t)e->Ppad * E));
    CK(e->alloc(&e->v_att, (size_t)e->P * E));
    CK(e->alloc(&e->v_act, (size_t)e->P * c.v_intermediate));
    CK(e->alloc(&e->v_mh, (size_t)(e->P / 4 + 1) * Mg));
    CK(e->alloc(&e->vis, (size_t)(e->P / 4 + 1) * H));
    CK(e->alloc(&e->vis_pref, (size_t)(e->P / 4 + 1) * H));
    CK(e->alloc(&e->v_cs, (size_t)e->P * 64));
    CK(e->alloc(&e->v_pos, (size_t)e->P * 2));
    CK(e->alloc(&e->v_tiles, (size_t)(e->P / 64 + 256)));
    CK(e->alloc(&e->v_qblocks, (size_t)(e->P / 128 + 256) * c.v_heads));

    e->TP = c.max_prefill_tokens;
    e->TPpad = e->TP + 64 * c.max_batch;
    CK(e->alloc(&e->p_x, (size_t)e->TP * H));
    CK(e->alloc(&e->p_xn, (size_t)e->TP * H));
    CK(e->alloc(&e->p_qkv, (size_t)e->TP * (Nq + 2 * Nkv)));
    CK(e->alloc(&e->p_q, (size_t)e->TP * Nq));
    CK(e->alloc(&e->p_k, (size_t)(e->TP + 64) * Nkv));
    CK(e->alloc(&e->p_vt, (size_t)e->TPpad * Nkv));
    CK(e->alloc(&e->p_att, (size_t)e->TP * Nq));
    CK(e->alloc(&e->p_act, (size_t)e->TP * c.intermediate_size));
    CK(e->alloc(&e->p_cs, (size_t)e->TP * 64));
    CK(e->alloc(&e->p_pos, (size_t)e->TP));
    CK(e->alloc(&e->p_src, (size_t)e->TP));
    CK(e->alloc(&e->p_last, (size_t)DOTS_MAX_BATCH));
    CK(e->alloc(&e->p_tiles, (size_t)(e->TP / 64 + c.max_batch + 1)));
    CK(e->alloc(&e->p_qblocks, (size_t)(e->TP / 128 + c.max_batch + 1) * c.num_heads));

    e->max_pages = (c.max_seq_len + 63) / 64;
    const int64_t pool_tokens = c.kv_pool_tokens > 0 ? c.kv_pool_tokens : (int64_t)c.max_batch * e->max_pages * 64;
    e->n_pool_pages = (int)((pool_tokens + 63) / 64);
    e->kv8 = c.kv_cache_dtype == 1;
    e->pool_layer_elems = (size_t)(e->n_pool_pages + 1) * c.num_kv_heads * 2 * 8192 / (e->kv8 ? 2 : 1);
    CK(e->alloc(&e->pool, e->pool_layer_elems * c.num_layers));
    const std::vector<float> kv_ones((size_t)c.num_layers * c.num_kv_heads * 2, 1.0f);
    CK(e->alloc(&e->kv_scales, kv_ones.size()));
    CK(hipMemcpyAsync(e->kv_scales, kv_ones.data(), kv_ones.size() * 4, hipMemcpyHostToDevice, e->stream));
    const int mb = (c.max_batch + 15) / 16 * 16;
    CK(e->alloc(&e->block_table, (size_t)mb * e->max_pages));
    CK(e->alloc(&e->ctx_len, (size_t)mb));
    CK(e->alloc(&e->cur_tokens, (size_t)mb));
    CK(e->alloc(&e->out_ids, (size_t)mb * c.max_seq_len));
    CK(e->alloc(&e->out_lens, (size_t)mb));
    CK(e->alloc(&e->finished, (size_t)mb));
    CK(e->alloc(&e->eos_ids, (size_t)16));
    CK(e->alloc(&e->d_sel, (size_t)DOTS_MAX_BATCH));
    CK(e->alloc(&e->d_sel_new, (size_t)DOTS_MAX_BATCH));
    CK(e->alloc(&e->d_max_len, (size_t)DOTS_MAX_BATCH));
    CK(e->alloc(&e->p_dst, (size_t)DOTS_MAX_BATCH));
    CK(e->alloc(&e->fk_dev, (size_t)3 * DOTS_MAX_BATCH));
    CK(e->alloc(&e->am_idx, (size_t)mb * 64));
    CK(e->alloc(&e->am_val, (size_t)mb * 64));
    CK(e->alloc(&e->d_h, (size_t)mb * H));
    CK(e->alloc(&e->d_q, (size_t)mb * Nq));
    CK(e->alloc(&e->d_att, (size_t)mb * Nq));
    CK(e->alloc(&e->d_act, (size_t)mb * c.intermediate_size));
    CK(e->alloc(&e->d_xn, (size_t)DOTS_MAX_BATCH * H));
    CK(e->alloc(&e->d_part_h, (size_t)DEC_KSPLIT_PARTS * DOTS_MAX_BATCH * H));
    CK(e->alloc(&e->d_logits, (size_t)mb * c.vocab_size));
    CK(e->alloc(&e->d_part_o, (size_t)mb * c.num_heads * 64 * 128));
    CK(e->alloc(&e->d_part_ml, (size_t)mb * c.num_heads * 64 * 2));
    if (const char* fm = getenv("DOTS_OCR_DECODE_PLAN")) {
// ... 57 lines not shown
```

### dots_ocr_amd/engine.py

```python
from __future__ import annotations

import ctypes as C
import math
import os
from collections import OrderedDict
from dataclasses import dataclass
from typing import Dict, Optional, Sequence

import numpy as np

from . import _lib
from .config import DotsConfig

EPI_NONE, EPI_RESIDUAL, EPI_SWIGLU, EPI_GELU, EPI_F32 = range(5)
DTYPE_BF16, DTYPE_F32, DTYPE_F16 = 0, 1, 2


class CDotsConfig(C.Structure):
    _fields_ = [
        ("hidden_size", C.c_int32), ("num_layers", C.c_int32), ("num_heads", C.c_int32), ("num_kv_heads", C.c_int32),
        ("head_dim", C.c_int32), ("intermediate_size", C.c_int32), ("vocab_size", C.c_int32),
        ("rope_theta", C.c_float), ("rms_norm_eps", C.c_float),
        ("attention_bias", C.c_int32), ("image_token_id", C.c_int32),
        ("v_embed_dim", C.c_int32), ("v_layers", C.c_int32), ("v_heads", C.c_int32), ("v_intermediate", C.c_int32),
# ... 219 lines not shown
    def to_c(self) -> CDotsNgramRule:
        c = CDotsNgramRule(self.size, self.window, len(self.whitelist))
        for j, t in enumerate(self.whitelist):
            c.whitelist[j] = t
        return c


def banned_ngram_ids(out, n: int, window: int = 0, whitelist=()) -> set:
    out = [int(t) for t in out]
    L, n, window = len(out), int(n), int(window)
    if n < 1 or L < n - 1:
        return set()
    prefix = out[L - n + 1:] if n > 1 else []
    white = set(int(t) for t in whitelist)
    banned = set()
    for i in range(max(0, L - window) if window > 0 else 0, L - n + 1):
        if out[i:i + n - 1] == prefix and out[i + n - 1] not in white:
            banned.add(out[i + n - 1])
    return banned


class DotsEngineError(RuntimeError):
    pass


_SIGNATURES_SET = False


def _prototypes(lib):
    global _SIGNATURES_SET
    if _SIGNATURES_SET:
        return
    vp, i32, i64, f32 = C.c_void_p, C.c_int32, C.c_int64, C.c_float
    P = C.POINTER
    sig = {
        "dots_create": (i32, [P(CDotsConfig), i32, P(vp)]),
        "dots_destroy": (None, [vp]),
        "dots_last_error": (C.c_char_p, [vp]),
        "dots_stream": (vp, [vp]),
        "dots_load_weight": (i32, [vp, C.c_char_p, vp, i32, P(i64), i32]),
        "dots_finalize_weights": (i32, [vp]),
        "dots_vit_forward": (i32, [vp, vp, i32, i64, P(i64), i32, vp]),
        "dots_vit_prefetch": (i32, [vp, vp, i32, i64, P(i64), i32, i32]),
        "dots_vit_take_prefetched": (i32, [vp]),
        "dots_vit_prefetch_ready": (i32, [vp, P(i32)]),
        "dots_prefill": (i32, [vp, P(i32), P(i32), i32]),
        "dots_decode_step": (i32, [vp]),
        "dots_generate": (i32, [vp, P(i32), P(i32), i32, vp, i32, i64, P(i64), i32, i32, P(i32), i32, P(i32), P(i32)]),
        "dots_preprocess_image": (i32, [vp, vp, i32, i32, i32, i32, i32, P(i32), P(i32), i32, P(i32), P(i32), i32, P(f32), P(f32), f32, vp]),
        "dots_set_sampling": (i32, [vp, f32, f32, C.c_uint64]),
        "dots_set_row_sampling": (i32, [vp, i32, P(CDotsSamplingParams)]),
        "dots_set_decode_plan": (i32, [vp, i32]),
        "dots_set_gemm_plan": (i32, [vp, i32]),
        "dots_tower_tail": (i32, [vp, i32, P(i32)]),
        "dots_slot_capacity": (i32, [vp, i32, P(i32), P(i32)]),
        "dots_slots_reset": (i32, [vp]),
        "dots_set_eos": (i32, [vp, P(i32), i32]),
        "dots_slots_prefill": (i32, [vp, P(i32), i32, P(i32), P(i32), P(i32)]),
        "dots_slots_decode": (i32, [vp, i32]),
        "dots_slots_fork": (i32, [vp, i32, P(i32), i32]),
        "dots_slots_poll": (i32, [vp, P(i32), P(i32)]),
        "dots_slot_read": (i32, [vp, i32, P(i32), i32, P(i32)]),
        "dots_slot_release": (i32, [vp, i32]),
        "dots_kv_pool_info": (i32, [vp, P(i32), P(i32)]),
        "dots_set_kv_scales": (i32, [vp, P(f32)]),
        "dots_get_logits": (i32, [vp, P(f32)]),
        "dots_set_next_tokens": (i32, [vp, P(i32), i32]),
        "dots_get_last_tokens": (i32, [vp, P(i32)]),
        "dots_get_stats": (i32, [vp, P(CDotsStats)]),
        "dots_synchronize": (i32, [vp]),
        "dots_debug_capture_hidden": (i32, [vp, i64]),
        "dots_debug_read_hidden": (i32, [vp, i32, i32, vp, P(i64)]),
        "dots_debug_read_kv": (i32, [vp, i32, i32, i32, i32, i32, vp]),
        "dots_dev_alloc": (i32, [vp, i64, P(vp)]),
        "dots_dev_free": (i32, [vp, vp]),
        "dots_memcpy_h2d": (i32, [vp, vp, vp, i64]),
        "dots_memcpy_d2h": (i32, [vp, vp, vp, i64]),
        "dots_op_rmsnorm": (i32, [vp, vp, vp, vp, i64, i32, f32]),
        "dots_op_layernorm": (i32, [vp, vp, vp, vp, vp, i64, i32, f32]),
        "dots_op_gemm": (i32, [vp, vp, vp, vp, vp, vp, i64, i32, i32, i32, vp]),
        "dots_op_quant_fp8": (i32, [vp, vp, vp, i64, i32]),
        "dots_op_gemm_fp8": (i32, [vp, vp, vp, vp, vp, vp, i64, i32, i32, i32]),
        "dots_op_flash_attn": (i32, [vp, vp, vp, vp, vp, P(i32), i32, i32, i32, i32, f32]),
        "dots_plan_flash_xcd": (i32, [P(i32), i32, i32, P(i32), P(i32), P(i64)]),
        "dots_op_qkv_rope_split": (i32, [vp, vp, vp, vp, vp, P(i32), i32, P(i32), i32, i32, i32, f32]),
        "dots_op_qkv_proj_rope": (i32, [vp, vp, vp, vp, vp, vp, vp, vp, P(i32), i32, P(i32), i32, i32, i32, i32, f32, i32]),
        "dots_op_dec_qkv": (i32, [vp, vp, vp, vp, vp, vp, vp, i32, vp, vp, i32, i32, i32, i32, f32, f32, i32]),
        "dots_op_decode_attn": (i32, [vp, vp, vp, vp, vp, i32, vp, i32, i32, i32, i32]),
        "dots_op_dec_qkv_kv8": (i32, [vp, vp, vp, vp, vp, vp, vp, i32, vp, vp, i32, i32, i32, i32, f32, f32, i32, vp]),
        "dots_op_decode_attn_kv8": (i32, [vp, vp, vp, vp, vp, i32, vp, i32, i32, i32, i32, vp]),
        "dots_op_dec_proj": (i32, [vp, vp, vp, vp, i32, i32, i32, i32]),
        "dots_op_dec_gateup": (i32, [vp, vp, vp, vp, vp, vp, i32, i32, i32, f32, i32]),
        "dots_op_dec_lmhead": (i32, [vp, vp, vp, vp, vp, i32, i32, i32, f32, i32]),
        "dots_op_select_tokens": (i32, [vp, vp, i32, i32, P(CDotsSamplingParams), vp, vp, i32, vp, vp]),
        "dots_bench_select_tokens": (i32, [vp, vp, i32, i32, P(CDotsSamplingParams), vp, vp, i32, vp, i32, i32, P(f32)]),
        "dots_set_row_logit_rules": (i32, [vp, i32, P(CDotsLogitRules)]),
        "dots_op_select_tokens_rules": (i32, [vp, vp, i32, i32, P(CDotsSamplingParams), P(CDotsLogitRules), P(i32), vp, vp, i32, vp, vp]),
        "dots_bench_select_tokens_rules": (i32, [vp, vp, i32, i32, P(CDotsSamplingParams), P(CDotsLogitRules), P(i32), vp, vp, i32, vp, i32, P(f32)]),
        "dots_set_token_bytes": (i32, [vp, P(i32), vp]),
        "dots_guide_create": (i32, [vp, vp, i32, vp, i32, P(i32)]),
        "dots_guide_destroy": (i32, [vp, i32]),
        "dots_set_row_guide": (i32, [vp, i32, i32]),
        "dots_row_guide_state": (i32, [vp, i32, P(i32)]),
        "dots_op_select_tokens_guided": (i32, [vp, vp, i32, i32, P(CDotsSamplingParams), P(CDotsLogitRules), P(i32), P(i32), P(i32), vp, vp, i32, vp, vp,
                                               P(i32)]),
        "dots_bench_select_tokens_guided": (i32, [vp, vp, i32, i32, P(CDotsSamplingParams), P(CDotsLogitRules), P(i32), P(i32), P(i32), vp, vp, i32, vp,
                                                  i32, P(f32)]),
        "dots_set_row_ngram": (i32, [vp, i32, P(CDotsNgramRule)]),
        "dots_op_select_tokens_ngram": (i32, [vp, vp, i32, i32, P(CDotsSamplingParams), P(CDotsLogitRules), P(CDotsNgramRule), vp, vp, i32, vp, vp]),
        "dots_bench_select_tokens_ngram": (i32, [vp, vp, i32, i32, P(CDotsSamplingParams), P(CDotsLogitRules), P(CDotsNgramRule), vp, vp, i32, vp, i32,
                                                 P(f32)]),
        "dots_stop_create": (i32, [vp, vp, i32, vp, vp, P(i32)]),
        "dots_stop_destroy": (i32, [vp, i32]),
        "dots_set_row_stop": (i32, [vp, i32, i32, i32]),
        "dots_row_stop_hit": (i32, [vp, i32, P(i32)]),
        "dots_set_speculation": (i32, [vp, i32, i32, i32]),
        "dots_set_speculation_rows": (i32, [vp, i32]),
        "dots_set_row_drafts": (i32, [vp, i32, P(i32), i32]),
        "dots_spec_stats": (i32, [vp, i32, P(i64), P(i64), P(i64)]),
        "dots_op_ngram_draft": (i32, [vp, vp, vp, i32, i32, i32, i32, i32, vp, vp]),
        "dots_set_row_logprobs": (i32, [vp, i32, i32]),
        "dots_row_logprobs": (i32, [vp, i32, i32, i32, P(f32), P(i32), P(f32), P(i32)]),
        "dots_op_logprobs": (i32, [vp, vp, i32, i32, i32, P(i32), vp, vp, vp, vp]),
        "dots_bench_logprobs": (i32, [vp, vp, i32, i32, i32, P(i32), i32, i32, P(f32)]),
        "dots_probe_mfma": (i32, [i32, vp, vp, vp, vp]),
        "dots_probe_grid_barrier": (i32, [i32, i32, i32, i32, i32, P(f32), P(i32)]),
        "dots_probe_cu_mask": (i32, [P(C.c_uint32), i32, i32, i32, i32, P(C.c_uint32)]),
    }
    for name, (res, args) in sig.items():
        fn = getattr(lib, name)
        fn.restype = res
        fn.argtypes = args
    _SIGNATURES_SET = True


EXPORTED_SYMBOLS = [
    "dots_create", "dots_destroy", "dots_last_error", "dots_stream", "dots_load_weight", "dots_finalize_weights",
    "dots_vit_forward", "dots_vit_prefetch", "dots_vit_take_prefetched", "dots_vit_prefetch_ready", "dots_preprocess_image", "dots_prefill", "dots_decode_step", "dots_generate", "dots_set_sampling", "dots_set_decode_plan", "dots_set_gemm_plan", "dots_tower_tail", "dots_get_logits",
    "dots_set_eos", "dots_slots_prefill", "dots_slots_decode", "dots_slots_poll", "dots_slot_read", "dots_slot_release", "dots_kv_pool_info", "dots_slot_capacity", "dots_slots_reset",
    "dots_set_next_tokens", "dots_get_last_tokens", "dots_get_stats", "dots_synchronize", "dots_debug_capture_hidden",
    "dots_debug_read_hidden", "dots_dev_alloc",
    "dots_dev_free", "dots_memcpy_h2d", "dots_memcpy_d2h", "dots_op_rmsnorm", "dots_op_layernorm", "dots_op_gemm", "dots_op_quant_fp8", "dots_op_gemm_fp8",
    "dots_op_flash_attn", "dots_plan_flash_xcd", "dots_op_qkv_rope_split", "dots_op_qkv_proj_rope", "dots_op_dec_qkv", "dots_op_decode_attn", "dots_op_dec_proj", "dots_op_dec_gateup",
    "dots_op_dec_lmhead", "dots_probe_mfma", "dots_probe_grid_barrier", "dots_probe_cu_mask",
    "dots_set_kv_scales", "dots_debug_read_kv", "dots_op_dec_qkv_kv8", "dots_op_decode_attn_kv8",
    "dots_set_row_sampling", "dots_op_select_tokens", "dots_bench_select_tokens",
    "dots_set_row_logprobs", "dots_row_logprobs", "dots_op_logprobs", "dots_bench_logprobs",
    "dots_set_row_logit_rules", "dots_op_select_tokens_rules", "dots_bench_select_tokens_rules",
    "dots_set_token_bytes", "dots_guide_create", "dots_guide_destroy", "dots_set_row_guide", "dots_row_guide_state",
    "dots_op_select_tokens_guided", "dots_bench_select_tokens_guided",
    "dots_set_row_ngram", "dots_op_select_tokens_ngram", "dots_bench_select_tokens_ngram",
    "dots_set_speculation", "dots_set_speculation_rows", "dots_set_row_drafts", "dots_spec_stats", "dots_op_ngram_draft",
    "dots_slots_fork",
    "dots_stop_create", "dots_stop_destroy", "dots_set_row_stop", "dots_row_stop_hit",
]

MAX_SPEC_DRAFTS = 15
MAX_NGRAM_SIZE = 64


def ngram_draft(history: Sequence[int], k: int, min_n: int = 2, max_n: int = 4) -> list:
    out = [int(t) for t in history]
    L = len(out)
    if k < 1 or min_n < 1 or max_n < min_n:
        raise ValueError("ngram_draft needs k >= 1 and 1 <= min_n <= max_n")
    for n in range(max_n, min_n - 1, -1):
        if n + 1 > L:
            continue
        key = out[L - n:]
        hits = [i for i in range(L - n) if out[i:i + n] == key]
        if not hits:
            continue
        full = [i for i in hits if i + n + k <= L]
        i = max(full) if full else min(hits)
        return out[i + n:min(i + n + k, L)]
    return []


def spec_usable_slots(max_batch: int, k: int) -> int:
    return int(max_batch) // (int(k) + 1)


SPEC_ROWS = {"sampled": 1, "stop": 2}


def spec_rows_flags(value) -> int:
    if value is None:
        return 0
    names = (value,) if isinstance(value, str) else tuple(value)
    flags = 0
    for n in names:
        if n == "all":
            flags |= sum(SPEC_ROWS.values())
        elif n == "greedy" and len(names) == 1:
            pass
        elif isinstance(n, str) and n in SPEC_ROWS:
            flags |= SPEC_ROWS[n]
        else:
            raise ValueError(f"speculative_rows takes \"all\", \"greedy\" or names out of {sorted(SPEC_ROWS)}, got {value!r}")
    return flags


MAX_TOP_LOGPROBS = 20

KV_CACHE_DTYPES = {"bf16": 0, "fp8": 1}


def resolve_kv_cache_dtype(kv_cache_dtype: Optional[str]) -> str:
    if kv_cache_dtype is None:
        kv_cache_dtype = os.environ.get("DOTS_OCR_KV_CACHE_DTYPE", "") or "bf16"
    if kv_cache_dtype not in KV_CACHE_DTYPES:
        raise ValueError(f"kv_cache_dtype must be one of {sorted(KV_CACHE_DTYPES)}, got {kv_cache_dtype!r}")
    return kv_cache_dtype


def c_config(cfg: DotsConfig, max_batch: int, max_seq_len: int, max_patches: int, max_prefill_tokens: int, kv_pool_tokens: int = 0,
             fp8_weights: bool = False, kv_cache_dtype: str = "bf16") -> CDotsConfig:
    v = cfg.vision
    return CDotsConfig(
        hidden_size=cfg.hidden_size, num_layers=cfg.num_hidden_layers, num_heads=cfg.num_attention_heads,
        num_kv_heads=cfg.num_key_value_heads, head_dim=cfg.head_dim, intermediate_size=cfg.intermediate_size,
        vocab_size=cfg.vocab_size, rope_theta=cfg.rope_theta, rms_norm_eps=cfg.rms_norm_eps,
        attention_bias=int(cfg.attention_bias), image_token_id=cfg.image_token_id,
        v_embed_dim=v.embed_dim, v_layers=v.num_hidden_layers, v_heads=v.num_attention_heads,
        v_intermediate=v.intermediate_size, v_patch=v.patch_size, v_merge=v.spatial_merge_size,
        v_channels=v.num_channels, v_temporal_patch=v.temporal_patch_size, v_rms_eps=v.rms_norm_eps,
        v_ln_eps=v.merger_ln_eps, v_use_bias=int(v.use_bias), v_post_norm=int(v.post_norm),
        max_batch=max_batch, max_seq_len=max_seq_len, max_patches=max_patches,
        max_prefill_tokens=max_prefill_tokens, kv_pool_tokens=kv_pool_tokens, fp8_weights=int(bool(fp8_weights)),
        kv_cache_dtype=KV_CACHE_DTYPES[kv_cache_dtype])


def plan_flash_xcd(lens: Sequence[int], heads: int):
    lib = _lib.load()
    _prototypes(lib)
    L = np.ascontiguousarray(lens, dtype=np.int32)
    base, cnt, cost = np.zeros(8, np.int32), np.zeros(8, np.int32), np.zeros(8, np.int64)
    n = lib.dots_plan_flash_xcd(_i32p(L), int(L.shape[0]), int(heads), _i32p(base), _i32p(cnt), _i64p(cost))
    if n < 0:
        raise DotsEngineError(f"dots_plan_flash_xcd failed ({n})")
    return base, cnt, cost, int(n)


def _i32p(a: np.ndarray):
    return a.ctypes.data_as(C.POINTER(C.c_int32))


def _i64p(a: np.ndarray):
    return a.ctypes.data_as(C.POINTER(C.c_int64))


class Engine:

    def __init__(self, cfg: DotsConfig, device: int = 0, max_batch: int = 8, max_seq_len: int = 8192,
                 max_patches: int = 8 * 19824 + 64, max_prefill_tokens: Optional[int] = None, kv_pool_tokens: int = 0,
                 fp8_weights: bool = False, kv_cache_dtype: Optional[str] = None):
        self.kv_cache_dtype = resolve_kv_cache_dtype(kv_cache_dtype)
        self.lib = _lib.load()
        _prototypes(self.lib)
        self.cfg = cfg
        self.device = device
        self.max_batch = max_batch
        self.max_seq_len = max_seq_len
        self.max_patches = max_patches
        if max_prefill_tokens is None:
            max_prefill_tokens = max_batch * max_seq_len
        self.max_prefill_tokens = max_prefill_tokens
        self.kv_pool_tokens = kv_pool_tokens
        self.fp8_weights = bool(fp8_weights)
        self._cc = c_config(cfg, max_batch, max_seq_len, max_patches, max_prefill_tokens, kv_pool_tokens, fp8_weights, self.kv_cache_dtype)
        h = C.c_void_p()
        rc = self.lib.dots_create(C.byref(self._cc), device, C.byref(h))
        if rc != 0:
            raise DotsEngineError(f"dots_create failed ({rc}): {self.lib.dots_last_error(None).decode()}")
        self.h = h
        self.token_bytes = None
        self._stops = OrderedDict()

    def _ck(self, rc: int, what: str):
        if rc != 0:
            raise DotsEngineError(f"{what} failed ({rc}): {self.lib.dots_last_error(self.h).decode()}")

    def close(self):
        if getattr(self, "h", None):
            self.lib.dots_destroy(self.h)
            self.h = None

    def __del__(self):
        try:
            self.close()
        except Exception:
            pass

    @property
# ... 336 lines not shown
        hist = np.zeros((B, stride), np.int32)
        for b, h in enumerate(histories):
            hist[b, :len(h)] = np.asarray(h, np.int32)
        lens = np.asarray([len(h) for h in histories], np.int32)
        d_hist, d_lens = self.to_device(hist), self.to_device(lens)
        d_out, d_n = self.to_device(np.full((B, int(k)), -1, np.int32)), self.to_device(np.full((B,), -1, np.int32))
        try:
            self._ck(self.lib.dots_op_ngram_draft(self.h, C.c_void_p(d_hist), C.c_void_p(d_lens), stride, B, int(k), int(min_n), int(max_n),
                                                  C.c_void_p(d_out), C.c_void_p(d_n)), "dots_op_ngram_draft")
            out, n = self.to_host(d_out, (B, int(k)), np.int32), self.to_host(d_n, (B,), np.int32)
        finally:
            for ptr in (d_hist, d_lens, d_out, d_n):
                self.dev_free(ptr)
        return [out[b, :int(n[b])].tolist() for b in range(B)]

    def set_row_logprobs(self, row: int, top_n: Optional[int]):
        n = -1 if top_n is None else int(top_n)
        if top_n is not None and not 0 <= n <= MAX_TOP_LOGPROBS:
            raise ValueError(f"top_n must be None or in [0, {MAX_TOP_LOGPROBS}], got {top_n!r}")
        self._ck(self.lib.dots_set_row_logprobs(self.h, int(row), n), "dots_set_row_logprobs")

    def row_logprobs(self, row: int, n: int, pos0: int = 0):
        n = max(0, int(n))
        K = MAX_TOP_LOGPROBS
        tok = np.empty((max(1, n),), np.float32)
        ids = np.empty((max(1, n), K), np.int32)
        top = np.empty((max(1, n), K), np.float32)
        m = C.c_int32(0)
        fp = lambda a: a.ctypes.data_as(C.POINTER(C.c_float))
        self._ck(self.lib.dots_row_logprobs(self.h, int(row), int(pos0), n, fp(tok), _i32p(ids), fp(top), C.byref(m)), "dots_row_logprobs")
        k = int(m.value)
        return tok[:k].copy(), ids[:k].copy(), top[:k].copy()

    def op_logprobs(self, logits, B: int, V: int, ld: int, top_n: Sequence[int], chosen, tok_lp, top_ids, top_lp):
        tn = np.ascontiguousarray(top_n, dtype=np.int32)
        if tn.shape != (B,):
            raise ValueError("one top_n per row")
        self._ck(self.lib.dots_op_logprobs(self.h, logits, int(B), int(V), int(ld), _i32p(tn), chosen, tok_lp, top_ids, top_lp),
                 "dots_op_logprobs")

    def bench_logprobs(self, logits, B: int, V: int, ld: int, top_n: Sequence[int], which: int = 0, iters: int = 200) -> float:
        tn = np.ascontiguousarray(top_n, dtype=np.int32)
        ms = C.c_float()
        self._ck(self.lib.dots_bench_logprobs(self.h, logits, int(B), int(V), int(ld), _i32p(tn), int(which), int(iters), C.byref(ms)),
                 "dots_bench_logprobs")
        return float(ms.value)

    def set_decode_plan(self, plan: int):
        self._ck(self.lib.dots_set_decode_plan(self.h, int(plan)), "dots_set_decode_plan")

    def set_gemm_plan(self, plan: int):
        self._ck(self.lib.dots_set_gemm_plan(self.h, int(plan)), "dots_set_gemm_plan")

    def tower_tail(self, set: int = -2) -> int:
        now = C.c_int32(0)
        self._ck(self.lib.dots_tower_tail(self.h, int(set), C.byref(now)), "dots_tower_tail")
        return int(now.value)

    def decode_step(self):
        self._ck(self.lib.dots_decode_step(self.h), "dots_decode_step")

    def set_eos(self, eos_ids: Sequence[int]):
        eos = np.ascontiguousarray(list(eos_ids), dtype=np.int32)
        self._ck(self.lib.dots_set_eos(self.h, _i32p(eos) if len(eos) else None, len(eos)), "dots_set_eos")

    def slots_prefill(self, slots: Sequence[int], input_ids: np.ndarray, prompt_lens: Sequence[int], max_new_tokens: Sequence[int]):
        sl = np.ascontiguousarray(slots, dtype=np.int32)
        ids = np.ascontiguousarray(input_ids, dtype=np.int32)
        lens = np.ascontiguousarray(prompt_lens, dtype=np.int32)
        cap = np.ascontiguousarray(max_new_tokens, dtype=np.int32)
        assert sl.shape == lens.shape == cap.shape and ids.shape[0] == int(lens.sum())
        self._ck(self.lib.dots_slots_prefill(self.h, _i32p(sl), sl.shape[0], _i32p(ids), _i32p(lens), _i32p(cap)), "dots_slots_prefill")

    def slots_fork(self, src: int, dst_slots: Sequence[int]):
        dst = np.ascontiguousarray(dst_slots, dtype=np.int32)
        assert dst.ndim == 1
        self._ck(self.lib.dots_slots_fork(self.h, int(src), _i32p(dst) if dst.shape[0] else None, dst.shape[0]), "dots_slots_fork")

    def slots_reset(self):
        self._ck(self.lib.dots_slots_reset(self.h), "dots_slots_reset")

    def slots_decode(self, n_steps: int):
        self._ck(self.lib.dots_slots_decode(self.h, int(n_steps)), "dots_slots_decode")

    def slots_poll(self):
        fin = np.empty((self.max_batch,), dtype=np.int32)
        lens = np.empty((self.max_batch,), dtype=np.int32)
        self._ck(self.lib.dots_slots_poll(self.h, _i32p(fin), _i32p(lens)), "dots_slots_poll")
        return fin, lens

    def slot_read(self, slot: int, capacity: int) -> np.ndarray:
        out = np.empty((max(1, capacity),), dtype=np.int32)
        n = C.c_int32(0)
        self._ck(self.lib.dots_slot_read(self.h, int(slot), _i32p(out), int(capacity), C.byref(n)), "dots_slot_read")
        return out[:min(int(n.value), capacity)].copy()

    def slot_release(self, slot: int):
        self._ck(self.lib.dots_slot_release(self.h, int(slot)), "dots_slot_release")

    def slot_capacity(self, slot: int):
        pg, lim = C.c_int32(0), C.c_int32(0)
        self._ck(self.lib.dots_slot_capacity(self.h, int(slot), C.byref(pg), C.byref(lim)), "dots_slot_capacity")
        return pg.value, lim.value

    def kv_pool_info(self):
        tot, free = C.c_int32(0), C.c_int32(0)
# ... 43 lines not shown
            n = int((grid[:, 0] * grid[:, 1] * grid[:, 2]).sum())
            if pixel_on_device:
                ptr = C.c_void_p(int(pixel_values))
            else:
                pv = np.ascontiguousarray(pixel_values, dtype=np.float32)
                assert pv.shape[0] == n
                ptr = pv.ctypes.data_as(C.c_void_p)
            gp, n_img = _i64p(grid), grid.shape[0]
        else:
            ptr, n, gp, n_img = None, 0, None, 0
        self._ck(self.lib.dots_generate(self.h, _i32p(ids), _i32p(lens), B, ptr, int(pixel_on_device), n, gp, n_img,
                                        max_new_tokens, _i32p(eos) if len(eos) else None, len(eos),
                                        _i32p(out_ids), _i32p(out_lens)), "dots_generate")
        self._B = B
        return out_ids, out_lens

    def capture_hidden(self, capacity_elems: int):
        self._ck(self.lib.dots_debug_capture_hidden(self.h, int(capacity_elems)), "dots_debug_capture_hidden")

    def read_hidden(self, which: str, layer: int) -> np.ndarray:
        dim = self.cfg.vision.embed_dim if which == "vit" else self.cfg.hidden_size
        cap = (self.max_patches if which == "vit" else self.max_prefill_tokens) * dim
        buf = np.empty(cap, dtype=np.uint16)
        rows = C.c_int64(0)
        self._ck(self.lib.dots_debug_read_hidden(self.h, 0 if which == "vit" else 1, int(layer), buf.ctypes.data_as(C.c_void_p), C.byref(rows)),
                 "dots_debug_read_hidden")
        return buf[: rows.value * dim].reshape(rows.value, dim).copy()

    def stats(self) -> dict:
        st = CDotsStats()
        self._ck(self.lib.dots_get_stats(self.h, C.byref(st)), "dots_get_stats")
        return {k: getattr(st, k) for k, _ in CDotsStats._fields_}

    def op_rmsnorm(self, x, w, y, rows, dim, eps):
        self._ck(self.lib.dots_op_rmsnorm(self.h, x, w, y, rows, dim, eps), "dots_op_rmsnorm")

    def op_layernorm(self, x, w, b, y, rows, dim, eps):
        self._ck(self.lib.dots_op_layernorm(self.h, x, w, b, y, rows, dim, eps), "dots_op_layernorm")

    def op_gemm(self, A, W, bias, residual, Cout, M, N, K, epilogue=EPI_NONE, colscale=None):
        self._ck(self.lib.dots_op_gemm(self.h, A, W, bias or None, residual or None, Cout, M, N, K, epilogue, colscale or None), "dots_op_gemm")

    def op_gemm_fp8(self, A, W, bias, residual, Cout, M, N, K, epilogue=EPI_NONE):
        self._ck(self.lib.dots_op_gemm_fp8(self.h, A, W, bias or None, residual or None, Cout, M, N, K, epilogue), "dots_op_gemm_fp8")

    def op_quant_fp8(self, w_inout, scale_out, N, K):
        self._ck(self.lib.dots_op_quant_fp8(self.h, w_inout, scale_out, N, K), "dots_op_quant_fp8")

    def op_flash_attn(self, q, k, vt, out, cu_seqlens, Hq, Hkv, causal, scale):
        cu = np.ascontiguousarray(cu_seqlens, dtype=np.int32)
        self._ck(self.lib.dots_op_flash_attn(self.h, q, k, vt, out, _i32p(cu), cu.shape[0] - 1, Hq, Hkv, int(causal), scale),
                 "dots_op_flash_attn")

    def op_qkv_rope_split(self, qkv, q, k, vt, cu_seqlens, pos, Hq, Hkv, rope2d, theta):
        cu = np.ascontiguousarray(cu_seqlens, dtype=np.int32)
        pos = np.ascontiguousarray(pos, dtype=np.int32)
        self._ck(self.lib.dots_op_qkv_rope_split(self.h, qkv, q, k, vt, _i32p(cu), cu.shape[0] - 1, _i32p(pos), Hq, Hkv,
                                                 int(rope2d), theta), "dots_op_qkv_rope_split")

    def op_qkv_proj_rope(self, x, w, bias, qkv_ws, q, k, vt, cu_seqlens, pos, K, Hq, Hkv, rope2d, theta, fused):
        cu = np.ascontiguousarray(cu_seqlens, dtype=np.int32)
        pos = np.ascontiguousarray(pos, dtype=np.int32)
        self._ck(self.lib.dots_op_qkv_proj_rope(self.h, x, w, bias, qkv_ws, q, k, vt, _i32p(cu), cu.shape[0] - 1, _i32p(pos), K, Hq, Hkv,
                                                int(rope2d), theta, int(fused)), "dots_op_qkv_proj_rope")

    def op_dec_qkv(self, h, ln_w, wqkv, bias, ctx_len, block_table, max_pages, pool_layer, q_out, B, H, Hq, Hkv, eps, rope_theta, fp8=False):
        self._ck(self.lib.dots_op_dec_qkv(self.h, h, ln_w, wqkv, bias or None, ctx_len, block_table, max_pages, pool_layer, q_out,
                                          B, H, Hq, Hkv, eps, rope_theta, int(fp8)), "dots_op_dec_qkv")

    def op_decode_attn(self, q, pool_layer, ctx_len, block_table, max_pages, out, B, Hq, Hkv, max_seq_len):
        self._ck(self.lib.dots_op_decode_attn(self.h, q, pool_layer, ctx_len, block_table, max_pages, out, B, Hq, Hkv, max_seq_len),
                 "dots_op_decode_attn")

    def op_dec_qkv_kv8(self, h, ln_w, wqkv, bias, ctx_len, block_table, max_pages, pool_layer, q_out, B, H, Hq, Hkv, eps, rope_theta, kv_scales,
                       fp8=False):
        self._ck(self.lib.dots_op_dec_qkv_kv8(self.h, h, ln_w, wqkv, bias or None, ctx_len, block_table, max_pages, pool_layer, q_out,
                                              B, H, Hq, Hkv, eps, rope_theta, int(fp8), kv_scales), "dots_op_dec_qkv_kv8")

    def op_decode_attn_kv8(self, q, pool_layer, ctx_len, block_table, max_pages, out, B, Hq, Hkv, max_seq_len, kv_scales):
        self._ck(self.lib.dots_op_decode_attn_kv8(self.h, q, pool_layer, ctx_len, block_table, max_pages, out, B, Hq, Hkv, max_seq_len,
                                                  kv_scales), "dots_op_decode_attn_kv8")

    def op_dec_proj(self, x, w, h_inout, B, N, K, fp8=False):
        self._ck(self.lib.dots_op_dec_proj(self.h, x, w, h_inout, B, N, K, int(fp8)), "dots_op_dec_proj")

    def op_dec_gateup(self, h, ln_w, gate_w, up_w, act_out, B, H, I, eps, fp8=False):
        self._ck(self.lib.dots_op_dec_gateup(self.h, h, ln_w, gate_w, up_w, act_out, B, H, I, eps, int(fp8)), "dots_op_dec_gateup")

    def op_dec_lmhead(self, h, ln_w, w, logits_out, B, H, V, eps, fp8=False):
        self._ck(self.lib.dots_op_dec_lmhead(self.h, h, ln_w, w, logits_out, B, H, V, eps, int(fp8)), "dots_op_dec_lmhead")
```

### include/dots_ocr_hip.h

```cpp
#ifndef DOTS_OCR_HIP_H
#define DOTS_OCR_HIP_H

#include <stdint.h>

#ifdef __cplusplus
extern "C" {
#endif

#define DOTS_OK 0
#define DOTS_E_INVALID (-1)
#define DOTS_E_HIP (-2)
#define DOTS_E_STATE (-3)
#define DOTS_E_CAPACITY (-4)

#define DOTS_DTYPE_BF16 0
#define DOTS_DTYPE_F32 1
#define DOTS_DTYPE_F16 2

typedef struct DotsEngine DotsEngine;

typedef struct DotsConfig {
    int32_t hidden_size, num_layers, num_heads, num_kv_heads, head_dim, intermediate_size, vocab_size;
    float rope_theta, rms_norm_eps;
    int32_t attention_bias;
// ... 69 lines not shown
#define DOTS_MAX_STOP_IDS 16
typedef struct DotsLogitRules {
    const int32_t* bias_ids;
    const float* bias_values;
    int32_t n_bias;
    const int32_t* allowed_ids;
    int32_t n_allowed;
    int32_t min_tokens;
    int32_t stop_ids[DOTS_MAX_STOP_IDS];
    int32_t n_stop;
    int32_t ignore_eos;
} DotsLogitRules;
int dots_set_row_logit_rules(DotsEngine* e, int row, const DotsLogitRules* r);

#define DOTS_MAX_GUIDE_STATES 4096
int dots_set_token_bytes(DotsEngine* e, const int32_t* offsets_host, const uint8_t* bytes_host);
int dots_guide_create(DotsEngine* e, const uint16_t* table_host, int n_states, const uint8_t* accepting_host, int start, int32_t* id_out);
int dots_guide_destroy(DotsEngine* e, int32_t id);
int dots_set_row_guide(DotsEngine* e, int row, int32_t id);
int dots_row_guide_state(DotsEngine* e, int row, int32_t* state_out);

#define DOTS_MAX_NGRAM_SIZE 64
#define DOTS_MAX_NGRAM_WHITELIST 16
typedef struct DotsNgramRule {
    int32_t size;
    int32_t window;
    int32_t n_whitelist;
    int32_t whitelist[DOTS_MAX_NGRAM_WHITELIST];
} DotsNgramRule;
int dots_set_row_ngram(DotsEngine* e, int row, const DotsNgramRule* r);

#define DOTS_MAX_STOP_STRINGS 16
#define DOTS_MAX_STOP_BYTES 64
int dots_stop_create(DotsEngine* e, const uint16_t* table_host, int n_states, const uint16_t* match_len_host, const uint8_t* match_id_host,
                     int32_t* handle_out);
int dots_stop_destroy(DotsEngine* e, int32_t handle);
int dots_set_row_stop(DotsEngine* e, int row, int32_t handle, int min_tokens);
int dots_row_stop_hit(DotsEngine* e, int row, int32_t* out);

#define DOTS_MAX_SPEC_DRAFTS 15
#define DOTS_SPEC_ROWS_SAMPLED 1
#define DOTS_SPEC_ROWS_STOP 2
int dots_set_speculation(DotsEngine* e, int k, int min_n, int max_n);
int dots_set_speculation_rows(DotsEngine* e, int flags);
int dots_set_row_drafts(DotsEngine* e, int row, const int32_t* ids_host, int n);
int dots_spec_stats(DotsEngine* e, int row, int64_t* steps, int64_t* drafted, int64_t* accepted);

#define DOTS_MAX_TOP_LOGPROBS 20
int dots_set_row_logprobs(DotsEngine* e, int row, int top_n);
int dots_row_logprobs(DotsEngine* e, int row, int pos0, int n, float* tok_lp_host, int32_t* top_ids_host, float* top_lp_host, int32_t* n_out);
int dots_set_decode_plan(DotsEngine* e, int plan);
int dots_tower_tail(DotsEngine* e, int set, int* now);
int dots_set_gemm_plan(DotsEngine* e, int plan);

int dots_slots_reset(DotsEngine* e);
int dots_slots_fork(DotsEngine* e, int src_slot, const int32_t* dst_slots_host, int n);
int dots_set_eos(DotsEngine* e, const int32_t* eos_ids_host, int n_eos);
int dots_slots_prefill(DotsEngine* e, const int32_t* slots_host, int n, const int32_t* input_ids_host,
                       const int32_t* prompt_lens_host, const int32_t* max_new_tokens_host);
int dots_slots_decode(DotsEngine* e, int n_steps);
int dots_slots_poll(DotsEngine* e, int32_t* finished_host, int32_t* out_lens_host);
int dots_slot_read(DotsEngine* e, int slot, int32_t* out_ids_host, int capacity, int32_t* n_out);
int dots_slot_release(DotsEngine* e, int slot);
int dots_kv_pool_info(DotsEngine* e, int32_t* total_pages, int32_t* free_pages);
int dots_set_kv_scales(DotsEngine* e, const float* scales_host);
int dots_slot_capacity(DotsEngine* e, int slot, int32_t* pages_owned, int32_t* token_limit);

int dots_get_logits(DotsEngine* e, float* out_host);
int dots_set_next_tokens(DotsEngine* e, const int32_t* tokens_host, int B);
int dots_get_last_tokens(DotsEngine* e, int32_t* out_host);
int dots_get_stats(DotsEngine* e, DotsStats* out);
int dots_debug_capture_hidden(DotsEngine* e, int64_t capacity_elems);
int dots_debug_read_hidden(DotsEngine* e, int which, int layer, void* out_host, int64_t* rows_out);
int dots_debug_read_kv(DotsEngine* e, int layer, int seq_or_slot, int pos0, int n, int which, void* out_host);
int dots_synchronize(DotsEngine* e);

int dots_dev_alloc(DotsEngine* e, int64_t bytes, void** out_dev);
int dots_dev_free(DotsEngine* e, void* dev);
int dots_memcpy_h2d(DotsEngine* e, void* dst_dev, const void* src_host, int64_t bytes);
int dots_memcpy_d2h(DotsEngine* e, void* dst_host, const void* src_dev, int64_t bytes);

int dots_op_rmsnorm(DotsEngine* e, const void* x_dev, const void* w_dev, void* y_dev, int64_t rows, int dim, float eps);
int dots_op_layernorm(DotsEngine* e, const void* x_dev, const void* w_dev, const void* b_dev, void* y_dev,
                      int64_t rows, int dim, float eps);
int dots_op_gemm(DotsEngine* e, const void* A_dev, const void* W_dev, const void* bias_dev,
                 const void* residual_dev, void* C_dev, int64_t M, int N, int K, int epilogue, const float* colscale_dev);
int dots_op_quant_fp8(DotsEngine* e, void* w_inout_dev, float* scale_out_dev, int64_t N, int K);
int dots_op_gemm_fp8(DotsEngine* e, const void* A_dev, const void* W_dev, const void* bias_dev, const void* residual_dev, void* C_dev,
                     int64_t M, int N, int K, int epilogue);
int dots_op_flash_attn(DotsEngine* e, const void* q_dev, const void* k_dev, const void* vt_dev, void* out_dev,
                       const int32_t* cu_seqlens_host, int n_seq, int Hq, int Hkv, int causal, float scale);
int dots_plan_flash_xcd(const int32_t* lens, int n_seq, int Hq, int32_t* base8, int32_t* cnt8, int64_t* cost8);
int dots_op_qkv_rope_split(DotsEngine* e, const void* qkv_dev, void* q_dev, void* k_dev, void* vt_dev,
                           const int32_t* cu_seqlens_host, int n_seq, const int32_t* pos_host,
                           int Hq, int Hkv, int rope2d, float theta);
int dots_op_qkv_proj_rope(DotsEngine* e, const void* x_dev, const void* w_dev, const void* bias_dev, void* qkv_ws_dev, void* q_dev, void* k_dev, void* vt_dev,
                          const int32_t* cu_seqlens_host, int n_seq, const int32_t* pos_host, int K, int Hq, int Hkv, int rope2d, float theta, int fused);
int dots_op_dec_qkv(DotsEngine* e, const void* h_dev, const void* ln_w_dev, const void* wqkv_dev, const void* bias_dev,
                    const int32_t* ctx_len_dev, const int32_t* block_table_dev, int max_pages, void* pool_layer_dev, void* q_out_dev,
                    int B, int H, int Hq, int Hkv, float eps, float rope_theta, int fp8);
int dots_op_decode_attn(DotsEngine* e, const void* q_dev, const void* pool_layer_dev, const int32_t* ctx_len_dev,
                        const int32_t* block_table_dev, int max_pages, void* out_dev, int B, int Hq, int Hkv, int max_seq_len);
int dots_op_dec_qkv_kv8(DotsEngine* e, const void* h_dev, const void* ln_w_dev, const void* wqkv_dev, const void* bias_dev,
                        const int32_t* ctx_len_dev, const int32_t* block_table_dev, int max_pages, void* pool_layer_dev, void* q_out_dev,
                        int B, int H, int Hq, int Hkv, float eps, float rope_theta, int fp8, const float* kv_scales_dev);
int dots_op_decode_attn_kv8(DotsEngine* e, const void* q_dev, const void* pool_layer_dev, const int32_t* ctx_len_dev,
                            const int32_t* block_table_dev, int max_pages, void* out_dev, int B, int Hq, int Hkv, int max_seq_len,
                            const float* kv_scales_dev);
int dots_op_dec_proj(DotsEngine* e, const void* x_dev, const void* w_dev, void* h_inout_dev, int B, int N, int K, int fp8);
int dots_op_dec_gateup(DotsEngine* e, const void* h_dev, const void* ln_w_dev, const void* gate_w_dev, const void* up_w_dev, void* act_out_dev,
                       int B, int H, int I, float eps, int fp8);
int dots_op_dec_lmhead(DotsEngine* e, const void* h_dev, const void* ln_w_dev, const void* w_dev, void* logits_out_dev, int B, int H, int V,
                       float eps, int fp8);
int dots_op_select_tokens(DotsEngine* e, const float* logits_dev, int B, int V, const DotsSamplingParams* params_host, const int32_t* hist_dev,
                          const int32_t* hist_lens_dev, int hist_stride, const int32_t* n_prompt_dev, int32_t* out_tokens_dev);
int dots_bench_select_tokens(DotsEngine* e, const float* logits_dev, int B, int V, const DotsSamplingParams* params_host, const int32_t* hist_dev,
                             const int32_t* hist_lens_dev, int hist_stride, const int32_t* n_prompt_dev, int mode, int iters, float* ms_out);
int dots_op_select_tokens_rules(DotsEngine* e, const float* logits_dev, int B, int V, const DotsSamplingParams* params_host, const DotsLogitRules* rules_host,
                                const int32_t* n_gen_host, const int32_t* hist_dev, const int32_t* hist_lens_dev, int hist_stride,
                                const int32_t* n_prompt_dev, int32_t* out_tokens_dev);
int dots_bench_select_tokens_rules(DotsEngine* e, const float* logits_dev, int B, int V, const DotsSamplingParams* params_host, const DotsLogitRules* rules_host,
                                   const int32_t* n_gen_host, const int32_t* hist_dev, const int32_t* hist_lens_dev, int hist_stride,
                                   const int32_t* n_prompt_dev, int iters, float* ms_out);
int dots_op_select_tokens_guided(DotsEngine* e, const float* logits_dev, int B, int V, const DotsSamplingParams* params_host, const DotsLogitRules* rules_host,
                                 const int32_t* n_gen_host, const int32_t* guide_ids_host, const int32_t* states_host, const int32_t* hist_dev,
                                 const int32_t* hist_lens_dev, int hist_stride, const int32_t* n_prompt_dev, int32_t* out_tokens_dev, int32_t* states_out_host);
int dots_bench_select_tokens_guided(DotsEngine* e, const float* logits_dev, int B, int V, const DotsSamplingParams* params_host, const DotsLogitRules* rules_host,
                                    const int32_t* n_gen_host, const int32_t* guide_ids_host, const int32_t* states_host, const int32_t* hist_dev,
                                    const int32_t* hist_lens_dev, int hist_stride, const int32_t* n_prompt_dev, int iters, float* ms_out);
int dots_op_select_tokens_ngram(DotsEngine* e, const float* logits_dev, int B, int V, const DotsSamplingParams* params_host, const DotsLogitRules* rules_host,
                                const DotsNgramRule* ngram_host, const int32_t* hist_dev, const int32_t* hist_lens_dev, int hist_stride,
                                const int32_t* n_prompt_dev, int32_t* out_tokens_dev);
int dots_bench_select_tokens_ngram(DotsEngine* e, const float* logits_dev, int B, int V, const DotsSamplingParams* params_host, const DotsLogitRules* rules_host,
                                   const DotsNgramRule* ngram_host, const int32_t* hist_dev, const int32_t* hist_lens_dev, int hist_stride,
                                   const int32_t* n_prompt_dev, int iters, float* ms_out);
int dots_op_ngram_draft(DotsEngine* e, const int32_t* hist_dev, const int32_t* hist_lens_dev, int hist_stride, int B, int k, int min_n, int max_n,
                        int32_t* drafts_dev, int32_t* n_drafts_dev);
int dots_op_logprobs(DotsEngine* e, const float* logits_dev, int B, int V, int ld, const int32_t* top_n_host,
                     const int32_t* chosen_dev, float* tok_lp_dev, int32_t* top_ids_dev, float* top_lp_dev);
int dots_bench_logprobs(DotsEngine* e, const float* logits_dev, int B, int V, int ld, const int32_t* top_n_host, int which, int iters,
                        float* ms_out);

int dots_probe_mfma(int which, const void* A, const void* Bt, void* D, void* stream);
int dots_probe_grid_barrier(int n_wg, int threads, int n_barriers, int mode, int lds_bytes, float* ms_out, int32_t* stats_out);
int dots_probe_cu_mask(const uint32_t* mask, int words, int n_wg, int threads, int lds_bytes, uint32_t* ids_out_host);
// ... 6 lines not shown
```

Measured before the change: 6.072 pages/s.

## Write V^T directly from the vision QKV GEMM epilogue and add causal XCD plan

After: 6.092 pages/s, median of 6. Within noise of the previous version (+0.3%).

```diff
diff --git a/dots_ocr_amd/csrc/attn_prefill.hip b/dots_ocr_amd/csrc/attn_prefill.hip
--- a/dots_ocr_amd/csrc/attn_prefill.hip
+++ b/dots_ocr_amd/csrc/attn_prefill.hip
@@ -578,6 +578,27 @@
     return p;
 }
 
+int causal_block_cost(const QBlock& b) { return std::min((b.n + 63) / 64, (b.q0 + flash_rows_per_block() + 63) / 64); }
+XcdPlan make_causal_xcd_plan(QBlock* b, int n_blocks) {
+    XcdPlan p;
+    int64_t total = 0;
+    for (int i = 0; i < n_blocks; ++i) total += causal_block_cost(b[i]);
+    int pos = 0;
+    int64_t done = 0;
+    for (int x = 0; x < 8; ++x) {
+        const int64_t target = total * (x + 1) / 8;
+        p.base[x] = pos;
+        while (pos < n_blocks && (x == 7 || 2 * (done - target) + causal_block_cost(b[pos]) < 0)) done += causal_block_cost(b[pos++]);
+        p.cnt[x] = pos - p.base[x];
+        std::stable_sort(b + p.base[x], b + pos, [](const QBlock& u, const QBlock& v) { return causal_block_cost(u) > causal_block_cost(v); });
+    }
+    return p;
+}
+bool causal_xcd_plan_on() {
+    static const bool on = getenv("DOTS_OCR_CAUSAL_PLAN") && atoi(getenv("DOTS_OCR_CAUSAL_PLAN")) != 0;
+    return on;
+}
+
 hipError_t launch_flash_attn(hipStream_t s, const bf16_t* q, const bf16_t* k, const bf16_t* vt, bf16_t* out,
                              const QBlock* blocks, int n_blocks, int64_t T, int64_t Tpad, int Hq, int Hkv,
                              int causal, float scale, const XcdPlan* plan) {
diff --git a/dots_ocr_amd/csrc/elementwise.hip b/dots_ocr_amd/csrc/elementwise.hip
--- a/dots_ocr_amd/csrc/elementwise.hip
+++ b/dots_ocr_amd/csrc/elementwise.hip
@@ -180,6 +180,18 @@
     }
 }
 
+__global__ __launch_bounds__(256) void vt_zero_pad_kernel(const Tile64* __restrict__ tiles, bf16_t* __restrict__ vt, int64_t Tpad) {
+    const Tile64 tl = tiles[blockIdx.x];
+    if (tl.n >= 64) return;
+    const int h = blockIdx.y, tid = threadIdx.x;
+#pragma unroll
+    for (int it = 0; it < 4; ++it) {
+        const int item = it * 256 + tid;
+        const int d = item >> 3, pc = item & 7;
+        *reinterpret_cast<u32x4*>(vt + ((size_t)h * 128 + d) * Tpad + tl.pad0 + pc * 8) = u32x4{0, 0, 0, 0};
+    }
+}
+
 __global__ __launch_bounds__(256) void embed_gather_kernel(const int32_t* __restrict__ src, const bf16_t* __restrict__ embed,
                                                            const bf16_t* __restrict__ vision, bf16_t* __restrict__ x,
                                                            int64_t T, int dim) {
@@ -249,6 +261,12 @@
     return hipGetLastError();
 }
 
+hipError_t launch_vt_zero_pad(hipStream_t s, const Tile64* tiles, int n_tiles, bf16_t* vt, int64_t Tpad, int Hkv) {
+    if (n_tiles <= 0) return hipSuccess;
+    hipLaunchKernelGGL(vt_zero_pad_kernel, dim3(n_tiles, Hkv), dim3(256), 0, s, tiles, vt, Tpad);
+    return hipGetLastError();
+}
+
 hipError_t launch_embed_gather(hipStream_t s, const int32_t* src, const bf16_t* embed, const bf16_t* vision, bf16_t* x,
                                int64_t T, int dim) {
     if (T <= 0) return hipSuccess;
diff --git a/dots_ocr_amd/csrc/engine.h b/dots_ocr_amd/csrc/engine.h
--- a/dots_ocr_amd/csrc/engine.h
+++ b/dots_ocr_amd/csrc/engine.h
@@ -88,9 +88,11 @@
     int32_t* v_pos = nullptr;
     Tile64* v_tiles = nullptr;
     QBlock* v_qblocks = nullptr;
+    int32_t* v_vtcol = nullptr;
     int64_t vis_rows = 0;
     std::vector<int32_t> h_pos;
     std::vector<Tile64> h_tiles;
+    std::vector<int32_t> h_vtcol;
     std::vector<QBlock> h_qblocks;
 
     int64_t TP = 0, TPpad = 0;
@@ -276,6 +278,7 @@
 int set_row_lp(DotsEngine* e, int row, int top_n);
 void build_worklists(const std::vector<int>& lens, int Hq, std::vector<Tile64>& tiles, std::vector<QBlock>& qblocks, int64_t* Tpad_used,
                      const int* seq_ids = nullptr);
+void build_vt_cols(const std::vector<int>& lens, std::vector<int32_t>& cols);
 void drop_step_graphs(DotsEngine* e);
 int chain_streams(DotsEngine* e, hipStream_t from, hipStream_t to);
 int pick_decode_stream(DotsEngine* e, hipStream_t* cur);
diff --git a/dots_ocr_amd/csrc/engine.hip b/dots_ocr_amd/csrc/engine.hip
--- a/dots_ocr_amd/csrc/engine.hip
+++ b/dots_ocr_amd/csrc/engine.hip
@@ -24,9 +24,15 @@
 }
 
 int qkv_rope_on(DotsEngine* e, hipStream_t st, uint8_t* aq, float* as, const bf16_t* A, const bf16_t* W, const uint8_t* W8, const float* wscale, const bf16_t* bias,
-                bf16_t* qkv, const float2* cs, const Tile64* tiles, int n_tiles, bf16_t* q, bf16_t* k, bf16_t* vt, int64_t T, int64_t Tpad, int K, int Hq, int Hkv) {
+                bf16_t* qkv, const float2* cs, const Tile64* tiles, int n_tiles, bf16_t* q, bf16_t* k, bf16_t* vt, int64_t T, int64_t Tpad, int K, int Hq, int Hkv,
+                const int32_t* vt_col = nullptr) {
     const int N = (Hq + 2 * Hkv) * 128;
     if (!W8 && !wscale) {
+        if (vt_col) {
+            const hipError_t rv = launch_gemm_qk_rope(st, A, W, bias, qkv, T, N, K, K, N, cs, q, k, Hq, Hkv, vt, vt_col, Tpad);
+            if (rv == hipSuccess) return DOTS_OK;
+            if (rv != hipErrorNotSupported) CK(rv);
+        }
         const hipError_t r = launch_gemm_qk_rope(st, A, W, bias, qkv, T, N, K, K, N, cs, q, k, Hq, Hkv);
         if (r == hipSuccess) {
             CK(launch_qkv_rope_split(st, qkv, cs, tiles, n_tiles, q, k, vt, T, Tpad, Hq, Hkv, true));
@@ -101,6 +107,11 @@
     if (lens.size() > 256) return e->fail(DOTS_E_CAPACITY, "more than 256 images per call");
     int64_t Tpad = 0;
     build_worklists(lens, Hh, e->h_tiles, e->h_qblocks, &Tpad);
+    const bool vt_fused = gemm_get_vt_fuse() != 0;
+    if (vt_fused) {
+        build_vt_cols(lens, e->h_vtcol);
+        CK(hipMemcpyAsync(e->v_vtcol, e->h_vtcol.data(), e->h_vtcol.size() * 4, hipMemcpyHostToDevice, s));
+    }
     CK(hipMemcpyAsync(e->v_pos, e->h_pos.data(), e->h_pos.size() * 4, hipMemcpyHostToDevice, s));
     CK(hipMemcpyAsync(e->v_tiles, e->h_tiles.data(), e->h_tiles.size() * sizeof(Tile64), hipMemcpyHostToDevice, s));
     CK(hipMemcpyAsync(e->v_qblocks, e->h_qblocks.data(), e->h_qblocks.size() * sizeof(QBlock), hipMemcpyHostToDevice, s));
@@ -110,6 +121,7 @@
     CK(launch_gemm(s, e->v_xa, e->patch_w, e->patch_b, nullptr, e->v_xn, N, E, e->patch_kpad, e->patch_kpad, E, EPI_NONE));
     CK(launch_rmsnorm(s, e->v_xn, e->patch_norm, e->v_x, N, E, c.v_rms_eps));
     CK(launch_rope_table(s, e->v_pos, e->v_inv_freq, e->v_cs, N, 1));
+    if (vt_fused) CK(launch_vt_zero_pad(s, e->v_tiles, (int)e->h_tiles.size(), e->v_vt, Tpad, Hh));
     const float scale = 1.0f / sqrtf(128.0f);
     e->attn_pairs = 0;
     const XcdPlan xcd_plan = make_xcd_plan(e->h_qblocks.data(), (int)e->h_qblocks.size());
@@ -127,7 +139,7 @@
         }
         CK(launch_rmsnorm(s, e->v_x, L.norm1, e->v_xn, N, E, c.v_rms_eps));
         RET(qkv_rope_on(e, s, e->act_q_v, e->act_s_v, e->v_xn, L.qkv_w, L.qkv_8, L.qkv_s, L.qkv_b, e->v_qkv, e->v_cs, e->v_tiles, (int)e->h_tiles.size(), e->v_q, e->v_k, e->v_vt,
-                        N, Tpad, E, Hh, Hh));
+                        N, Tpad, E, Hh, Hh, vt_fused ? e->v_vtcol : nullptr));
         CK(attn_event(e, 2 * i));
         CK(launch_flash_attn(s, e->v_q, e->v_k, e->v_vt, e->v_att, e->v_qblocks, (int)e->h_qblocks.size(), N, Tpad, Hh, Hh, 0, scale, &xcd_plan));
         CK(attn_event(e, 2 * i + 1));
@@ -274,6 +286,15 @@
         pad0 += (int)round_up(n, 64);
     }
     *Tpad_used = pad0;
+}
+
+void build_vt_cols(const std::vector<int>& lens, std::vector<int32_t>& cols) {
+    cols.clear();
+    int pad0 = 0;
+    for (const int n : lens) {
+        for (int i = 0; i < n; ++i) cols.push_back(pad0 + ((i & ~15) | (i & 3) | (((i >> 3) & 1) << 2) | (((i >> 2) & 1) << 3)));
+        pad0 += (int)round_up(n, 64);
+    }
 }
 
 void drop_step_graphs(DotsEngine* e) {
@@ -348,6 +369,9 @@
         return e->fail(DOTS_E_STATE, "prompt has %lld image tokens but the vision tower produced %lld rows", (long long)vis_used, (long long)e->vis_rows);
     int64_t Tpad = 0;
     build_worklists(L, Hq, e->hp_tiles, e->hp_qblocks, &Tpad, S.data());
+    const bool causal_plan = causal_xcd_plan_on();
+    XcdPlan xcd_plan;
+    if (causal_plan) xcd_plan = make_causal_xcd_plan(e->hp_qblocks.data(), (int)e->hp_qblocks.size());
     CK(hipMemcpyAsync(e->p_pos, e->hp_pos.data(), T * 4, hipMemcpyHostToDevice, s));
     CK(hipMemcpyAsync(e->p_src, e->hp_src.data(), T * 4, hipMemcpyHostToDevice, s));
     CK(hipMemcpyAsync(e->p_last, e->hp_last.data(), DOTS_MAX_BATCH * 4, hipMemcpyHostToDevice, s));
@@ -415,7 +439,7 @@
         CK(launch_rmsnorm(s, e->p_x, Lw.ln1, e->p_xn, T, H, c.rms_norm_eps));
         RET(qkv_rope_on(e, s, e->act_q, e->act_s, e->p_xn, Lw.qkv_w, Lw.qkv_8, Lw.qkv_s, Lw.qkv_b, e->p_qkv, e->p_cs, e->p_tiles, n_tiles, e->p_q, e->p_k, e->p_vt, T, Tpad, H, Hq, Hkv));
         CK(launch_kv_to_pages(s, e->p_k, e->p_qkv, e->p_tiles, n_tiles, e->block_table, e->max_pages, pool_l, T, Hq, Hkv, layer_kv_scales(e, i)));
-        CK(launch_flash_attn(s, e->p_q, e->p_k, e->p_vt, e->p_att, e->p_qblocks, (int)e->hp_qblocks.size(), T, Tpad, Hq, Hkv, 1, scale));
+        CK(launch_flash_attn(s, e->p_q, e->p_k, e->p_vt, e->p_att, e->p_qblocks, (int)e->hp_qblocks.size(), T, Tpad, Hq, Hkv, 1, scale, causal_plan ? &xcd_plan : nullptr));
         RET(dense(e, e->p_att, Lw.o_w, Lw.o_8, Lw.o_s, nullptr, e->p_x, e->p_x, T, H, Nq, H, EPI_RESIDUAL));
         CK(launch_rmsnorm(s, e->p_x, Lw.ln2, e->p_xn, T, H, c.rms_norm_eps));
         RET(dense(e, e->p_xn, Lw.w13, Lw.w13_8, Lw.w13_s, nullptr, nullptr, e->p_act, T, 2 * c.intermediate_size, H, c.intermediate_size, EPI_SWIGLU));
@@ -877,6 +901,13 @@
     return DOTS_OK;
 }
 
+int dots_set_vt_fuse(DotsEngine* e, int on) {
+    if (!e) return DOTS_E_INVALID;
+    if (on < 0 || on > 1) return e->fail(DOTS_E_INVALID, "vt fuse must be 0 (GEMM + split kernel) or 1 (V^T from the GEMM)");
+    gemm_set_vt_fuse(on);
+    return DOTS_OK;
+}
+
 int dots_get_logits(DotsEngine* e, float* out) {
     if (!e || !out) return DOTS_E_INVALID;
     if (e->B < 1) return e->fail(DOTS_E_STATE, "no prefilled batch");
diff --git a/dots_ocr_amd/csrc/gemm.hip b/dots_ocr_amd/csrc/gemm.hip
--- a/dots_ocr_amd/csrc/gemm.hip
+++ b/dots_ocr_amd/csrc/gemm.hip
@@ -677,6 +677,48 @@
 #undef W4_PUT
 }
 
+template <bool FULL>
+DEVI void w4_epilogue_vt(const f32x16 (&acc)[4][4], const bf16_t* __restrict__ bias, int nw0, const int32_t* __restrict__ vt_col, bf16_t* __restrict__ vth,
+                         long long Tpad, int M, int mw0, int l) {
+    const int hi = l >> 5, l31 = l & 31;
+    int z = 0;
+    asm volatile("s_nop 15\n\ts_nop 3" : "+s"(z));
+    uint32_t col[4];
+#pragma unroll
+    for (int fm = 0; fm < 4; ++fm) {
+        const int m = FULL ? mw0 + fm * 32 + l31 : min(mw0 + fm * 32 + l31, M - 1);
+        col[fm] = (uint32_t)vt_col[m + z];
+    }
+    u32x2 bw[16];
+#pragma unroll
+    for (int g = 0; g < 16; ++g) {
+        bw[g] = u32x2{0x80008000u, 0x80008000u};
+        if (bias) bw[g] = *reinterpret_cast<const u32x2*>(bias + nw0 + 8 * g + 4 * hi + z);
+    }
+    const uint64_t row_bytes = (uint64_t)Tpad * 2;
+#pragma unroll
+    for (int fm = 0; fm < 4; ++fm) {
+        const uint32_t o0 = (col[fm] + (uint32_t)(4 * hi) * (uint32_t)Tpad) * 2, o1 = o0 + (uint32_t)row_bytes;
+        if (FULL || mw0 + fm * 32 + l31 < M) {
+            uint64_t row = (uint64_t)(uintptr_t)vth;
+#pragma unroll
+            for (int g = 0; g < 16; ++g) {
+#pragma unroll
+                for (int e = 0; e < 4; e += 2) {
+                    float x0, x1;
+                    asm volatile("v_accvgpr_read_b32 %0, %2\n\tv_accvgpr_read_b32 %1, %3" : "=v"(x0), "=v"(x1) : "a"(acc[g >> 2][fm][4 * (g & 3) + e]), "a"(acc[g >> 2][fm][4 * (g & 3) + e + 1]));
+                    const uint32_t pk = pack_bf2(x0 + lo_bf(bw[g][e >> 1]), x1 + hi_bf(bw[g][e >> 1]));
+                    asm volatile("global_store_short %0, %2, %3\n\tglobal_store_short_d16_hi %1, %2, %3" ::"v"(o0), "v"(o1), "v"(pk), "s"(row) : "memory");
+                    row += (e == 2 ? 6 : 2) * row_bytes;
+                    asm volatile("" : "+s"(row));
+                    __builtin_amdgcn_sched_barrier(0);
+                }
+            }
+        }
+        __builtin_amdgcn_sched_barrier(0);
+    }
+}
+
 template <int... I, class F> DEVI void gemm_static_for_impl(std::integer_sequence<int, I...>, F&& f) { (f(std::integral_constant<int, I>{}), ...); }
 template <int N, class F> DEVI void gemm_static_for(F&& f) { gemm_static_for_impl(std::make_integer_sequence<int, N>{}, f); }
 
@@ -839,6 +881,10 @@
             bf16_t* dst = head < rope.Hq ? rope.q + (size_t)head * rope.T * 128 : rope.k + (size_t)(head - rope.Hq) * rope.T * 128;
             if (full) w4_epilogue_qkrope<true>(acc, cols, has_cols, rope.cs, dst, M, m0 + wm * 128, l, smem2 + w * 32768);
             else w4_epilogue_qkrope<false>(acc, cols, has_cols, rope.cs, dst, M, m0 + wm * 128, l, smem2 + w * 32768);
+        } else if (rope.vt) {
+            bf16_t* vth = rope.vt + (size_t)(head - rope.n_rope_heads) * 128 * rope.Tpad;
+            if (full) w4_epilogue_vt<true>(acc, bias, n0 + wn * 128, rope.vt_col, vth, rope.Tpad, M, m0 + wm * 128, l);
+            else w4_epilogue_vt<false>(acc, bias, n0 + wn * 128, rope.vt_col, vth, rope.Tpad, M, m0 + wm * 128, l);
         } else if (full) {
             w4_epilogue_lds<EPI_NONE, true>(acc, cols, has_cols, R, reinterpret_cast<bf16_t*>(Cout), M, ldc, n0 + wn * 128, m0 + wm * 128, l, smem2 + w * 32768);
         } else {
@@ -1080,13 +1126,26 @@
     return hipGetLastError();
 }
 
+static int g_vt_fuse = -1;
+int gemm_get_vt_fuse() {
+    int p = __atomic_load_n(&g_vt_fuse, __ATOMIC_RELAXED);
+    if (p < 0) {
+        const char* ev = getenv("DOTS_OCR_VT_FUSE");
+        p = ev ? (atoi(ev) != 0) : 1;
+        __atomic_store_n(&g_vt_fuse, p, __ATOMIC_RELAXED);
+    }
+    return p;
+}
+void gemm_set_vt_fuse(int on) { __atomic_store_n(&g_vt_fuse, on != 0, __ATOMIC_RELAXED); }
+
 hipError_t launch_gemm_qk_rope(hipStream_t s, const bf16_t* A, const bf16_t* W, const bf16_t* bias, bf16_t* qkv, int64_t M, int N, int K, int lda, int ldc,
-                               const float2* cs, bf16_t* q, bf16_t* k, int Hq, int Hkv) {
+                               const float2* cs, bf16_t* q, bf16_t* k, int Hq, int Hkv, bf16_t* vt, const int32_t* vt_col, int64_t Tpad) {
     static const bool off = getenv("DOTS_OCR_QK_FUSE") && atoi(getenv("DOTS_OCR_QK_FUSE")) == 0;
     static const bool lockstep = getenv("DOTS_OCR_GEMM_LOCKSTEP") != nullptr, force_small = getenv("DOTS_OCR_GEMM_128") != nullptr;
     if (off || lockstep || force_small || gemm_get_plan() != 1 || N != (Hq + 2 * Hkv) * 128 || N % BN2 != 0 || K % BK != 0 || K / BK < 3 || lda % 8 != 0 || ldc % 8 != 0 ||
         !cs || !q || !k || M > 0x7fffffff)
         return hipErrorNotSupported;
+    if (vt && (!vt_col || !gemm_get_vt_fuse() || Tpad < M || Tpad > (int64_t)0x0fffffff)) return hipErrorNotSupported;
     if (M <= 0) return hipSuccess;
     static uint32_t configured = 0;
     int dev = 0;
@@ -1099,7 +1158,7 @@
         __atomic_fetch_or(&configured, bit, __ATOMIC_RELEASE);
     }
     const int m_tiles = (int)((M + BM2 - 1) / BM2), n_tiles = N / BN2;
-    const QkRope rope{cs, q, k, (long long)M, Hq, Hq + Hkv};
+    const QkRope rope{cs, q, k, (long long)M, Hq, Hq + Hkv, vt, vt_col, (long long)Tpad};
     hipLaunchKernelGGL(gemm_bf16_w4_qkrope_kernel, dim3(m_tiles * n_tiles), dim3(256), W4_RING * W4_UNIT, s, A, W, bias, (const float*)nullptr, (void*)qkv, (int)M, N, K,
                        lda, ldc, m_tiles, n_tiles, raster_group_m(K * 2), rope);
     return hipGetLastError();
diff --git a/dots_ocr_amd/csrc/kernels.h b/dots_ocr_amd/csrc/kernels.h
--- a/dots_ocr_amd/csrc/kernels.h
+++ b/dots_ocr_amd/csrc/kernels.h
@@ -21,9 +21,12 @@
 struct Tile64 { int32_t tok0, n, pad0, seq, page, _pad; };
 hipError_t launch_qkv_rope_split(hipStream_t s, const bf16_t* qkv, const float2* cs, const Tile64* tiles, int n_tiles,
                                  bf16_t* q, bf16_t* k, bf16_t* vt, int64_t T, int64_t Tpad, int Hq, int Hkv, bool v_only = false);
-struct QkRope { const float2* cs; bf16_t* q; bf16_t* k; long long T; int Hq; int n_rope_heads; };
+struct QkRope { const float2* cs; bf16_t* q; bf16_t* k; long long T; int Hq; int n_rope_heads; bf16_t* vt; const int32_t* vt_col; long long Tpad; };
 hipError_t launch_gemm_qk_rope(hipStream_t s, const bf16_t* A, const bf16_t* W, const bf16_t* bias, bf16_t* qkv, int64_t M, int N, int K, int lda, int ldc,
-                               const float2* cs, bf16_t* q, bf16_t* k, int Hq, int Hkv);
+                               const float2* cs, bf16_t* q, bf16_t* k, int Hq, int Hkv, bf16_t* vt = nullptr, const int32_t* vt_col = nullptr, int64_t Tpad = 0);
+int gemm_get_vt_fuse();
+void gemm_set_vt_fuse(int on);
+hipError_t launch_vt_zero_pad(hipStream_t s, const Tile64* tiles, int n_tiles, bf16_t* vt, int64_t Tpad, int Hkv);
 hipError_t launch_embed_gather(hipStream_t s, const int32_t* src, const bf16_t* embed, const bf16_t* vision, bf16_t* x,
                                int64_t T, int dim);
 hipError_t launch_gather_rows(hipStream_t s, const bf16_t* x, const int32_t* rows, const int32_t* dst, bf16_t* y, int n, int dim);
@@ -32,6 +35,9 @@
 int flash_rows_per_block();
 struct XcdPlan { int32_t base[8], cnt[8]; };
 XcdPlan make_xcd_plan(const QBlock* blocks_host, int n_blocks);
+int causal_block_cost(const QBlock& b);
+XcdPlan make_causal_xcd_plan(QBlock* blocks_host, int n_blocks);
+bool causal_xcd_plan_on();
 hipError_t launch_flash_attn(hipStream_t s, const bf16_t* q, const bf16_t* k, const bf16_t* vt, bf16_t* out,
                              const QBlock* blocks, int n_blocks, int64_t T, int64_t Tpad, int Hq, int Hkv,
                              int causal, float scale, const XcdPlan* plan = nullptr);
diff --git a/dots_ocr_amd/csrc/ops.hip b/dots_ocr_amd/csrc/ops.hip
--- a/dots_ocr_amd/csrc/ops.hip
+++ b/dots_ocr_amd/csrc/ops.hip
@@ -342,6 +342,54 @@
     return DOTS_OK;
 }
 
+int dots_op_flash_attn_causal(DotsEngine* e, const void* q, const void* k, const void* vt, void* out, const int32_t* cu, int n_seq,
+                              int Hq, int Hkv, float scale, int plan) {
+    if (!e || !cu || n_seq < 1) return DOTS_E_INVALID;
+    CK(hipSetDevice(e->device));
+    std::vector<int> lens(n_seq);
+    for (int i = 0; i < n_seq; ++i) lens[i] = cu[i + 1] - cu[i];
+    std::vector<Tile64> tiles;
+    std::vector<QBlock> qb;
+    int64_t Tpad = 0;
+    build_worklists(lens, Hq, tiles, qb, &Tpad);
+    XcdPlan xp;
+    if (plan) xp = make_causal_xcd_plan(qb.data(), (int)qb.size());
+    QBlock* dq = nullptr;
+    CK(e->alloc(&dq, qb.size() + 1));
+    hipError_t r = hipMemcpyAsync(dq, qb.data(), qb.size() * sizeof(QBlock), hipMemcpyHostToDevice, e->stream);
+    if (r == hipSuccess) r = hipStreamSynchronize(e->stream);
+    if (r == hipSuccess)
+        r = launch_flash_attn(e->stream, (const bf16_t*)q, (const bf16_t*)k, (const bf16_t*)vt, (bf16_t*)out, dq, (int)qb.size(), cu[n_seq], Tpad, Hq, Hkv, 1, scale,
+                              plan ? &xp : nullptr);
+    hipStreamSynchronize(e->stream);
+    e->release(dq);
+    CK(r);
+    return DOTS_OK;
+}
+
+int dots_plan_flash_causal_xcd(const int32_t* lens, int n_seq, int Hq, int32_t* base8, int32_t* cnt8, int32_t* item_seq, int32_t* item_head, int32_t* item_q0,
+                               int32_t* item_cost) {
+    if (!lens || n_seq < 1 || Hq < 1 || !base8 || !cnt8) return DOTS_E_INVALID;
+    std::vector<int> L(lens, lens + n_seq);
+    for (int n : L)
+        if (n < 1) return DOTS_E_INVALID;
+    std::vector<Tile64> tiles;
+    std::vector<QBlock> qb;
+    int64_t Tpad = 0;
+    build_worklists(L, Hq, tiles, qb, &Tpad);
+    const XcdPlan p = make_causal_xcd_plan(qb.data(), (int)qb.size());
+    for (int x = 0; x < 8; ++x) { base8[x] = p.base[x]; cnt8[x] = p.cnt[x]; }
+    std::vector<int> tok0(n_seq);
+    for (int i = 0, t = 0; i < n_seq; t += L[i++]) tok0[i] = t;
+    for (size_t i = 0; i < qb.size(); ++i) {
+        if (item_seq) item_seq[i] = (int32_t)(std::upper_bound(tok0.begin(), tok0.end(), qb[i].tok0) - tok0.begin() - 1);
+        if (item_head) item_head[i] = qb[i].head;
+        if (item_q0) item_q0[i] = qb[i].q0;
+        if (item_cost) item_cost[i] = causal_block_cost(qb[i]);
+    }
+    return (int)qb.size();
+}
+
 int dots_plan_flash_xcd(const int32_t* lens, int n_seq, int Hq, int32_t* base8, int32_t* cnt8, int64_t* cost8) {
     if (!lens || n_seq < 1 || Hq < 1 || !base8 || !cnt8 || !cost8) return DOTS_E_INVALID;
     std::vector<int> L(lens, lens + n_seq);
@@ -415,11 +463,28 @@
     CK(hipMemcpyAsync(dpos, pos_host, (size_t)T * (rope2d ? 2 : 1) * 4, hipMemcpyHostToDevice, e->stream));
     CK(hipMemcpyAsync(freq, f.data(), nf * 4, hipMemcpyHostToDevice, e->stream));
     CK(launch_rope_table(e->stream, dpos, freq, cs, T, rope2d));
-    hipError_t r;
-    if (fused) {
+    hipError_t r = hipErrorNotSupported;
+    if (fused == 2) {
+        std::vector<int> lens(n_seq);
+        for (int i = 0; i < n_seq; ++i) lens[i] = cu[i + 1] - cu[i];
+        std::vector<int32_t> cols;
+        build_vt_cols(lens, cols);
+        int32_t* dcols = nullptr;
+        CK(e->alloc(&dcols, cols.size() + 1));
+        r = hipMemcpyAsync(dcols, cols.data(), cols.size() * 4, hipMemcpyHostToDevice, e->stream);
+        if (r == hipSuccess) r = hipStreamSynchronize(e->stream);
+        if (r == hipSuccess) r = launch_vt_zero_pad(e->stream, dt, (int)tiles.size(), (bf16_t*)vt, Tpad, Hkv);
+        if (r == hipSuccess)
+            r = launch_gemm_qk_rope(e->stream, (const bf16_t*)x, (const bf16_t*)w, (const bf16_t*)bias, (bf16_t*)qkv_ws, T, N, K, K, N, cs, (bf16_t*)q, (bf16_t*)k, Hq, Hkv,
+                                    (bf16_t*)vt, dcols, Tpad);
+        hipStreamSynchronize(e->stream);
+        e->release(dcols);
+    }
+    if (fused && r == hipErrorNotSupported) {
+        (void)hipGetLastError();
         r = launch_gemm_qk_rope(e->stream, (const bf16_t*)x, (const bf16_t*)w, (const bf16_t*)bias, (bf16_t*)qkv_ws, T, N, K, K, N, cs, (bf16_t*)q, (bf16_t*)k, Hq, Hkv);
         if (r == hipSuccess) r = launch_qkv_rope_split(e->stream, (const bf16_t*)qkv_ws, cs, dt, (int)tiles.size(), (bf16_t*)q, (bf16_t*)k, (bf16_t*)vt, T, Tpad, Hq, Hkv, true);
-    } else {
+    } else if (!fused) {
         r = launch_gemm(e->stream, (const bf16_t*)x, (const bf16_t*)w, (const bf16_t*)bias, nullptr, qkv_ws, T, N, K, K, N, EPI_NONE);
         if (r == hipSuccess) r = launch_qkv_rope_split(e->stream, (const bf16_t*)qkv_ws, cs, dt, (int)tiles.size(), (bf16_t*)q, (bf16_t*)k, (bf16_t*)vt, T, Tpad, Hq, Hkv);
     }
diff --git a/dots_ocr_amd/csrc/weights.hip b/dots_ocr_amd/csrc/weights.hip
--- a/dots_ocr_amd/csrc/weights.hip
+++ b/dots_ocr_amd/csrc/weights.hip
@@ -272,6 +272,7 @@
     CK(e->alloc(&e->v_cs, (size_t)e->P * 64));
     CK(e->alloc(&e->v_pos, (size_t)e->P * 2));
     CK(e->alloc(&e->v_tiles, (size_t)(e->P / 64 + 256)));
+    CK(e->alloc(&e->v_vtcol, (size_t)e->P));
     CK(e->alloc(&e->v_qblocks, (size_t)(e->P / 128 + 256) * c.v_heads));
 
     e->TP = c.max_prefill_tokens;
diff --git a/dots_ocr_amd/engine.py b/dots_ocr_amd/engine.py
--- a/dots_ocr_amd/engine.py
+++ b/dots_ocr_amd/engine.py
@@ -295,6 +295,7 @@
         "dots_set_row_sampling": (i32, [vp, i32, P(CDotsSamplingParams)]),
         "dots_set_decode_plan": (i32, [vp, i32]),
         "dots_set_gemm_plan": (i32, [vp, i32]),
+        "dots_set_vt_fuse": (i32, [vp, i32]),
         "dots_tower_tail": (i32, [vp, i32, P(i32)]),
         "dots_slot_capacity": (i32, [vp, i32, P(i32), P(i32)]),
         "dots_slots_reset": (i32, [vp]),
@@ -326,6 +327,8 @@
         "dots_op_gemm_fp8": (i32, [vp, vp, vp, vp, vp, vp, i64, i32, i32, i32]),
         "dots_op_flash_attn": (i32, [vp, vp, vp, vp, vp, P(i32), i32, i32, i32, i32, f32]),
         "dots_plan_flash_xcd": (i32, [P(i32), i32, i32, P(i32), P(i32), P(i64)]),
+        "dots_op_flash_attn_causal": (i32, [vp, vp, vp, vp, vp, P(i32), i32, i32, i32, f32, i32]),
+        "dots_plan_flash_causal_xcd": (i32, [P(i32), i32, i32, P(i32), P(i32), P(i32), P(i32), P(i32), P(i32)]),
         "dots_op_qkv_rope_split": (i32, [vp, vp, vp, vp, vp, P(i32), i32, P(i32), i32, i32, i32, f32]),
         "dots_op_qkv_proj_rope": (i32, [vp, vp, vp, vp, vp, vp, vp, vp, P(i32), i32, P(i32), i32, i32, i32, i32, f32, i32]),
         "dots_op_dec_qkv": (i32, [vp, vp, vp, vp, vp, vp, vp, i32, vp, vp, i32, i32, i32, i32, f32, f32, i32]),
@@ -396,6 +399,7 @@
     "dots_set_speculation", "dots_set_speculation_rows", "dots_set_row_drafts", "dots_spec_stats", "dots_op_ngram_draft",
     "dots_slots_fork",
     "dots_stop_create", "dots_stop_destroy", "dots_set_row_stop", "dots_row_stop_hit",
+    "dots_set_vt_fuse", "dots_op_flash_attn_causal", "dots_plan_flash_causal_xcd",
 ]
 
 MAX_SPEC_DRAFTS = 15
@@ -483,6 +487,19 @@
     if n < 0:
         raise DotsEngineError(f"dots_plan_flash_xcd failed ({n})")
     return base, cnt, cost, int(n)
+
+
+def plan_flash_causal_xcd(lens: Sequence[int], heads: int):
+    lib = _lib.load()
+    _prototypes(lib)
+    L = np.ascontiguousarray(lens, dtype=np.int32)
+    base, cnt = np.zeros(8, np.int32), np.zeros(8, np.int32)
+    cap = int(sum((int(n) + 127) // 128 for n in L)) * int(heads)
+    cols = [np.zeros(max(cap, 1), np.int32) for _ in range(4)]
+    n = lib.dots_plan_flash_causal_xcd(_i32p(L), int(L.shape[0]), int(heads), _i32p(base), _i32p(cnt), *[_i32p(c) for c in cols])
+    if n < 0:
+        raise DotsEngineError(f"dots_plan_flash_causal_xcd failed ({n})")
+    return base, cnt, np.stack([c[:n] for c in cols], axis=1)
 
 
 def _i32p(a: np.ndarray):
@@ -925,6 +942,9 @@
     def set_gemm_plan(self, plan: int):
         self._ck(self.lib.dots_set_gemm_plan(self.h, int(plan)), "dots_set_gemm_plan")
 
+    def set_vt_fuse(self, on: bool):
+        self._ck(self.lib.dots_set_vt_fuse(self.h, int(bool(on))), "dots_set_vt_fuse")
+
     def tower_tail(self, set: int = -2) -> int:
         now = C.c_int32(0)
         self._ck(self.lib.dots_tower_tail(self.h, int(set), C.byref(now)), "dots_tower_tail")
@@ -1074,6 +1094,11 @@
         self._ck(self.lib.dots_op_flash_attn(self.h, q, k, vt, out, _i32p(cu), cu.shape[0] - 1, Hq, Hkv, int(causal), scale),
                  "dots_op_flash_attn")
 
+    def op_flash_attn_causal(self, q, k, vt, out, cu_seqlens, Hq, Hkv, scale, plan):
+        cu = np.ascontiguousarray(cu_seqlens, dtype=np.int32)
+        self._ck(self.lib.dots_op_flash_attn_causal(self.h, q, k, vt, out, _i32p(cu), cu.shape[0] - 1, Hq, Hkv, scale, int(bool(plan))),
+                 "dots_op_flash_attn_causal")
+
     def op_qkv_rope_split(self, qkv, q, k, vt, cu_seqlens, pos, Hq, Hkv, rope2d, theta):
         cu = np.ascontiguousarray(cu_seqlens, dtype=np.int32)
         pos = np.ascontiguousarray(pos, dtype=np.int32)
diff --git a/include/dots_ocr_hip.h b/include/dots_ocr_hip.h
--- a/include/dots_ocr_hip.h
+++ b/include/dots_ocr_hip.h
@@ -145,6 +145,7 @@
 int dots_set_decode_plan(DotsEngine* e, int plan);
 int dots_tower_tail(DotsEngine* e, int set, int* now);
 int dots_set_gemm_plan(DotsEngine* e, int plan);
+int dots_set_vt_fuse(DotsEngine* e, int on);
 
 int dots_slots_reset(DotsEngine* e);
 int dots_slots_fork(DotsEngine* e, int src_slot, const int32_t* dst_slots_host, int n);
@@ -184,6 +185,10 @@
 int dots_op_flash_attn(DotsEngine* e, const void* q_dev, const void* k_dev, const void* vt_dev, void* out_dev,
                        const int32_t* cu_seqlens_host, int n_seq, int Hq, int Hkv, int causal, float scale);
 int dots_plan_flash_xcd(const int32_t* lens, int n_seq, int Hq, int32_t* base8, int32_t* cnt8, int64_t* cost8);
+int dots_op_flash_attn_causal(DotsEngine* e, const void* q_dev, const void* k_dev, const void* vt_dev, void* out_dev,
+                              const int32_t* cu_seqlens_host, int n_seq, int Hq, int Hkv, float scale, int plan);
+int dots_plan_flash_causal_xcd(const int32_t* lens, int n_seq, int Hq, int32_t* base8, int32_t* cnt8, int32_t* item_seq, int32_t* item_head, int32_t* item_q0,
+                               int32_t* item_cost);
 int dots_op_qkv_rope_split(DotsEngine* e, const void* qkv_dev, void* q_dev, void* k_dev, void* vt_dev,
                            const int32_t* cu_seqlens_host, int n_seq, const int32_t* pos_host,
                            int Hq, int Hkv, int rope2d, float theta);
```
